# mitsuba-renderer/mitsuba2

Hardware: AMD Instinct MI355X
Metric: Msamples/sec (whole node), 1080p/512spp path integrator (higher is better)
Workload: dtype f32

## Files before the change

### mitsuba2_amd/csrc/device/resident_kernel.h

```cpp
#ifndef MIW_KERNEL
#define MIW_KERNEL __global__
#endif
MIW_KERNEL __launch_bounds__(MIW_BLOCK) void k_init_pixels(RenderParams P, U4 *st_out, uint32_t *pixel_out, InitArgs A) {
    uint32_t lane = blockIdx.x * blockDim.x + threadIdx.x;
    if (lane >= P.n_lanes) return;
    uint32_t tile = lane >> A.bs2_log2, i = lane & ((1u << A.bs2_log2) - 1u);
    uint32_t b = A.tile_list ? A.tile_list[tile] : tile;
    uint32_t bx = b % A.blocks_x, by = b / A.blocks_x;
    uint32_t x, y;
    morton_decode2(i, x, y);
    int32_t bw = P.film.crop_w - (int32_t) (bx * A.bs), bh = P.film.crop_h - (int32_t) (by * A.bs);
    if (bw > (int32_t) A.bs) bw = (int32_t) A.bs;
    if (bh > (int32_t) A.bs) bh = (int32_t) A.bs;
    if ((int32_t) x >= bw || (int32_t) y >= bh) {
        U4 st; st.x = st.y = 0; st.z = LF_DONE; st.w = 0;
        st_out[lane] = st; pixel_out[lane] = 0;
        return;
    }
    uint32_t px = (uint32_t) P.film.crop_x + bx * A.bs + x, py = (uint32_t) P.film.crop_y + by * A.bs + y;
    pixel_out[lane] = px | (py << 16);
    st_out[lane] = lane_seed_state(A.base_seed + (uint64_t) A.block_ids[b] * (uint64_t) (A.bs * A.bs) + i);
}

struct TileArgs {
// ... 21 lines not shown
            if (nq > 1u) { const uint32_t id = Q->simd_ids[1u + key]; q = id < nq ? id : key % nq; }
            else if ((threadIdx.x & 63u) == 0u) Q->simd_ids[1u + key] = 1u;
        }
    }
    uint32_t ticks, quarter, tail_prio, sample_end_; uint32_t *prog;
    __device__ __forceinline__ void tick(uint32_t sample_idx, bool has_pixel) {
        if (!tail_prio) { ++ticks; return; }
        if ((uint32_t) __builtin_amdgcn_readfirstlane((int) ++ticks) & 15u) return;
        if (has_pixel) atomicMin(prog, sample_idx);
        const uint32_t v = *prog;
        *prog = 0xffffffffu;
        const uint32_t v4 = 4u * v, se = sample_end_;
        uint32_t qtr = v == 0xffffffffu ? 3u : (v4 >= se ? 1u : 0u) + (v4 >= 2u * se ? 1u : 0u) + (v4 >= 3u * se ? 1u : 0u);
        qtr = (uint32_t) __builtin_amdgcn_readfirstlane((int) qtr);
        if (qtr == quarter) return;
        quarter = qtr;
        if (qtr == 0u) __builtin_amdgcn_s_setprio(3); else if (qtr == 1u) __builtin_amdgcn_s_setprio(2);
        else if (qtr == 2u) __builtin_amdgcn_s_setprio(1); else __builtin_amdgcn_s_setprio(0);
    }
    __device__ __forceinline__ void enable_tail_prio(uint32_t sample_end, uint32_t *wave_word) {
        tail_prio = 1u; sample_end_ = sample_end; quarter = 0; prog = wave_word; *prog = 0xffffffffu; __builtin_amdgcn_s_setprio(3);
    }
    typedef uint32_t U4v __attribute__((ext_vector_type(4)));
    __device__ __forceinline__ static uint32_t &job_pend() { __shared__ uint32_t s_job_pend[MIW_BLOCK]; return s_job_pend[threadIdx.x & (MIW_BLOCK - 1)]; }
    __device__ __forceinline__ bool exhausted() const { return !Jobs || !Q->job_chunk || job_pend() == 0xffffffffu; }
    __device__ __forceinline__ uint32_t job_end(uint32_t sample_idx, uint32_t sample_end) const {
        const uint32_t r = spp - sample_idx;
        return Jobs && (r & (r - 1u)) == 0u && r >= Q->job_min ? sample_idx : sample_end;
    }
    __device__ __forceinline__ bool fetch_job(uint32_t &pixel, U4 &st) {
        for (;;) {
            const uint32_t parked = job_pend();
            if (parked == 0xffffffffu) return false;
            uint32_t id = parked - 1u;
            const bool fresh = parked == 0u;
            const unsigned long long b = __ballot(fresh);
            if (fresh) {
                const uint32_t me = threadIdx.x & 63u, leader = (uint32_t) __ffsll((long long) b) - 1u;
                uint32_t base = 0;
                if (me == leader) base = atomicAdd(next_pixel, (uint32_t) __popcll(b));
                base = (uint32_t) __shfl((int) base, (int) leader, 64);
                id = base + __builtin_amdgcn_mbcnt_hi((uint32_t) (b >> 32), __builtin_amdgcn_mbcnt_lo((uint32_t) b, 0u));
                if (id >= Q->job_total) { job_pend() = 0xffffffffu; return false; }
            }
            const uint32_t j = id / n_lanes, slot = id - j * n_lanes;
            const uint32_t px = Q->pixel[slot];
            U4v w;
#if defined(__HIP_DEVICE_COMPILE__)
            asm volatile("global_load_dwordx4 %0, %1, off sc1\n\ts_waitcnt vmcnt(0)" : "=&v"(w) : "v"(Q->st + slot) : "memory");
#endif
            if (w.z & LF_DONE) { job_pend() = 0u; continue; }
            if (w.w != (j ? spp - (Q->job_pow >> (j - 1u)) : 0u)) { job_pend() = id + 1u; return false; }
            job_pend() = 0u;
            lane = slot; pixel = px;
            st.x = w.x; st.y = w.y; st.z = w.z; st.w = w.w;
            return true;
        }
    }
    __device__ __forceinline__ bool fetch(uint32_t &pixel, U4 &st) {
        if (Jobs && Q->job_chunk) return fetch_job(pixel, st);
        for (;;) {
            if (!Placed) {
                const unsigned long long b = __ballot(1);
                const uint32_t me = threadIdx.x & 63u, leader = (uint32_t) __ffsll((long long) b) - 1u;
                uint32_t base = 0;
                if (me == leader) base = atomicAdd(next_pixel, (uint32_t) __popcll(b));
                base = (uint32_t) __shfl((int) base, (int) leader, 64);
                const uint32_t l = base + __builtin_amdgcn_mbcnt_hi((uint32_t) (b >> 32), __builtin_amdgcn_mbcnt_lo((uint32_t) b, 0u));
                if (l >= n_lanes) return false;
                lane = l;
                st = Q->st[lane];
                if (st.z & LF_DONE) continue;
                pixel = Q->pixel[lane];
                return true;
            }
            if (dry >= nq) {
                if (nq > 1u) Q->simd_ids[0] = 1u;
                return false;
            }
            if (nq > 1u && __hip_atomic_load(Q->simd_ids, __ATOMIC_RELAXED, __HIP_MEMORY_SCOPE_AGENT)) { dry = nq; return false; }
            const unsigned long long all = __ballot(1);
            const uint32_t me = threadIdx.x & 63u, leader = (uint32_t) __ffsll((long long) all) - 1u;
            const uint32_t q_lead = (uint32_t) __shfl((int) q, (int) leader, 64);
            const bool mine = q == q_lead;
            const unsigned long long b = __ballot(mine);
            if (!mine) continue;
            uint32_t base = 0;
            if (me == leader) base = atomicAdd(next_pixel + q, (uint32_t) __popcll(b));
            base = (uint32_t) __shfl((int) base, (int) leader, 64);
            const uint32_t idx = base + __builtin_amdgcn_mbcnt_hi((uint32_t) (b >> 32), __builtin_amdgcn_mbcnt_lo((uint32_t) b, 0u));
            uint32_t l = idx;
            if (nq > 1u) {
                const uint32_t piece = idx < per ? Q->piece_list[q * MIW_PLACE_PIECES + (idx >> 6)] : 0xffffffffu;
                if (piece == 0xffffffffu) { q = q + 1u == nq ? 0u : q + 1u; ++dry; continue; }
                l = Q->lane_sorted[piece * Q->piece_a + (idx & 63u) * Q->piece_b];
                if (l >= n_lanes) continue;
            } else if (l >= n_lanes) { ++dry; continue; }
            lane = l;
            st = Q->st[lane];
            if (st.z & LF_DONE) continue;
            pixel = Q->pixel[lane];
            if (Placed) t_fetch = cost_clock();
            return true;
        }
    }
    __device__ __forceinline__ uint32_t cost_clock() const {
        return Clock ? (uint32_t) (__builtin_amdgcn_s_memtime() >> 8) : ticks;
    }
    __device__ __forceinline__ void store(U4 st) {
        if (Jobs && Q->job_chunk) {
            unsigned long long *words = reinterpret_cast<unsigned long long *>(Q->st + lane);
            __hip_atomic_store(words, (unsigned long long) st.x | ((unsigned long long) st.y << 32), __ATOMIC_RELAXED, __HIP_MEMORY_SCOPE_AGENT);
            asm volatile("s_waitcnt vmcnt(0)" ::: "memory");
            __hip_atomic_store(words + 1, (unsigned long long) st.z | ((unsigned long long) st.w << 32), __ATOMIC_RELAXED, __HIP_MEMORY_SCOPE_AGENT);
            return;
        }
        Q->st[lane] = st;
        if (Placed && Q->lane_cost) Q->lane_cost[lane] = cost_clock() - t_fetch + 1u;
        if (Groups && Q->group_done && (st.z & LF_DONE)) {
            __threadfence();
            const uint32_t g = lane >> Q->group_shift;
            if (atomicAdd(Q->group_done + g, 1u) + 1u == Q->group_expected[g]) {
                __threadfence_system();
                __hip_atomic_store(Q->group_flag + g, 1u, __ATOMIC_RELEASE, __HIP_MEMORY_SCOPE_SYSTEM);
            }
        }
    }
    __device__ __forceinline__ void put(uint32_t pixel, uint32_t sample_idx, V2 pos, const float *aovs) {
        if (Q->log_rec) {
            LogSink16<const float *> sink{ Q->log_rec, thr, film, lane, spp, Q->log_rej & 255u, Q->log_rej >> 8 };
            sink(pixel, sample_idx, pos, aovs);
        } else {
            LogSink sink; sink.log_pos = Q->log_pos; sink.log_val = Q->log_val; sink.lane = lane; sink.spp = spp; sink.warn_negative = warn_negative;
            sink(0u, sample_idx, pos, aovs);
        }
    }
};

#ifndef MIW_DIRECT_WAVES
#define MIW_DIRECT_WAVES 3
#endif
#ifndef MIW_PACKET_WAVES_ALL
#define MIW_PACKET_WAVES_ALL 4
#endif
#ifndef MIW_PACKET_WAVES
#define MIW_PACKET_WAVES 5
#endif
template <bool UseLog, int Tiny, int Mats = MATS_ALL, bool Analytic = (Tiny == 0), uint32_t Integ = INTEG_PATH, bool Groups = false, int Waves = 0>
__global__ __launch_bounds__(MIW_BLOCK, Waves ? Waves : Integ == INTEG_DIRECT ? MIW_DIRECT_WAVES : Tiny ? ((Mats == MATS_DIFFUSE && !MIW_SPECTRAL) ? (Tiny == 2 ? MIW_PACKET_WAVES : 4) : MIW_PACKET_WAVES_ALL) : MIW_TREE_WAVES) void k_path_resident(RenderParams P, SceneView sc, LaneQueues Q, double *accum, Counters *cnt,
                                                               TraceLds cfg, uint32_t sample_end, TileArgs T, uint32_t *next_pixel) {
    extern __shared__ uint4 smem[];
    stage_to_lds(sc, cfg, smem);
    const float *thr = stage_thresholds(smem, cfg, UseLog && Q.log_rec ? Q.log_thr : nullptr);
#if MIW_LDS_TABLES
    if constexpr (UseLog && Tiny != 0) stage_tables<true, mats_lights(Mats)>(sc, cfg, smem);
#endif
#if defined(MIW_SECTION_PROFILE) && defined(__HIP_DEVICE_COMPILE__)
    if ((threadIdx.x & 63u) == 0) { unsigned long long *b_ = miw_sec_buf(); for (int i = 0; i < 15; ++i) b_[i] = 0; b_[15] = __builtin_amdgcn_s_memtime(); }
#endif
    const uint32_t lane = blockIdx.x * blockDim.x + threadIdx.x;
    double *tile = reinterpret_cast<double *>(smem + T.geom16);
    int tile_x0 = 0, tile_y0 = 0;
    if (!UseLog && T.side) {
        const uint32_t lane0 = blockIdx.x * blockDim.x, t = lane0 >> T.bs2_log2, q0 = lane0 & ((1u << T.bs2_log2) - 1u);
        const uint32_t b = T.tile_list ? T.tile_list[t] : t;
        uint32_t qx, qy;
        morton_decode2(q0, qx, qy);
        const int margin = (int) (T.side - 16u) / 2;
        tile_x0 = (int) ((b % T.blocks_x) * T.bs + qx) - margin;
        tile_y0 = (int) ((b / T.blocks_x) * T.bs + qy) - margin;
        for (uint32_t i = threadIdx.x; i < T.side * T.side * MIW_FILM_CHANNELS; i += blockDim.x) tile[i] = 0.0;
        __syncthreads();
    }
    LaneCounters local; local.segments = local.samples = local.shadow_rays = 0;
    auto tr2 = [&](V3 o, float mint, V3 dE, float maxtE, bool hasE, V3 dS, float maxtS, bool hasS, F4 &hE, bool &occS) {
        trace2<Tiny, Analytic>(sc, cfg, smem, o, mint, dE, maxtE, hasE, dS, maxtS, hasS, hE, occS);
    };
    if (UseLog) {
        QueueWork<Tiny != 0, false, Groups> work; work.Q = &Q; work.next_pixel = next_pixel; work.n_lanes = P.n_lanes; work.spp = P.spp; work.lane = 0; work.warn_negative = P.film.warn_negative;
        work.film = &P.film; work.thr = thr; work.init_queues(cfg.queues ? cfg.queues : 1u);
        __shared__ uint32_t s_prog[MIW_BLOCK / 64];
        if (cfg.tail_prio) work.enable_tail_prio(sample_end, &s_prog[threadIdx.x >> 6]);
        if constexpr (Integ == INTEG_DIRECT) pixel_stream_render_direct<Mats, Analytic>(P, sc, sample_end, work, tr2, &local);
        else pixel_stream_render<Mats, Analytic>(P, sc, sample_end, work, tr2, &local);
    } else if (lane < P.n_lanes) {
        U4 st = Q.st[lane];
        if (!(st.z & LF_DONE)) {
            const uint32_t pixel = Q.pixel[lane];
            if (T.side) {
                TileAdd add; add.tile = tile; add.x0 = tile_x0; add.y0 = tile_y0; add.side = (int) T.side;
                SplatXYSink<TileAdd> sink; sink.film = &P.film; sink.add = add;
                st = pixel_render<Integ, mats_nested(Mats) ? Mats : MATS_ALL>(P, sc, pixel, st, sample_end, tr2, sink, &local);
            } else {
                FilmAdd add; add.accum = accum;
                SplatSink<FilmAdd> sink; sink.film = &P.film; sink.add = add;
                st = pixel_render<Integ, mats_nested(Mats) ? Mats : MATS_ALL>(P, sc, pixel, st, sample_end, tr2, sink, &local);
            }
            Q.st[lane] = st;
        }
    }
    if (!UseLog && T.side) {
        __syncthreads();
        const int n = (int) (T.side * T.side);
        for (int i = (int) threadIdx.x; i < n * MIW_FILM_CHANNELS; i += (int) blockDim.x) {
            const double v = tile[i];
            if (v == 0.0) continue;
            const int texel = i / MIW_FILM_CHANNELS, k = i - texel * MIW_FILM_CHANNELS;
            const int fx = tile_x0 + texel % (int) T.side, fy = tile_y0 + texel / (int) T.side;
            unsafeAtomicAdd(accum + ((size_t) fy * P.film.crop_w + fx) * MIW_FILM_CHANNELS + k, v);
        }
    }
    unsigned long long a = wave_sum(local.segments), b = wave_sum(local.samples), c = wave_sum(local.shadow_rays);
    if ((threadIdx.x & 63) == 0) {
        Counters *shard = cnt + ((blockIdx.x * (MIW_BLOCK / 64) + (threadIdx.x >> 6)) & (MIW_CNT_SHARDS - 1));
        if (a) atomicAdd(&shard->segments, a);
        if (b) atomicAdd(&shard->samples, b);
        if (c) atomicAdd(&shard->shadow_rays, c);
#if defined(MIW_SECTION_PROFILE) && defined(__HIP_DEVICE_COMPILE__)
        { unsigned long long *b_ = miw_sec_buf(); for (int i = 0; i < 15; ++i) if (b_[i]) atomicAdd(&g_sections[i], b_[i]); }
#endif
    }
}
```

### mitsuba2_amd/csrc/device/trace.h

```cpp

struct TraceLds {
    uint32_t nodes_staged;
    uint32_t tris_staged;
    uint32_t brute;
    uint32_t leaves;
    uint32_t stack;
    uint32_t stack16;
    uint32_t shade_num, shade_den;
    uint32_t node_exit, tri_exit;
    uint32_t queues;
    uint32_t tail_prio;
    uint32_t thr16;
    uint32_t tab16;
    uint32_t tab_words[10];
    uint32_t env_top_count, env_top_base, env_top_words;
    uint32_t pool_claim_min;
    uint32_t pool16, stat16;
    uint32_t light_words;
};

struct alignas(16) LeafBox { float p[6]; uint32_t mask_lo, mask_hi; };
static_assert(sizeof(LeafBox) == 32, "LeafBox must be 32 bytes");

struct alignas(16) TriPacket { float p0[3], e1[3], e2[3]; uint32_t prim; uint32_t pad[2]; };
static_assert(sizeof(TriPacket) == 48, "TriPacket must be 48 bytes");

#ifndef MIW_LDS_TABLES
#define MIW_LDS_TABLES 1
#endif
#ifndef MIW_OCTANT_BOXES
#define MIW_OCTANT_BOXES 1
#endif
#define MIW_LEAF_BOX_COPIES (MIW_OCTANT_BOXES ? 8u : 1u)
__device__ __forceinline__ void stage_to_lds(const SceneView &sc, TraceLds cfg, uint4 *smem) {
    if (cfg.brute) {
        TriPacket *dst = reinterpret_cast<TriPacket *>(smem);
        for (uint32_t i = threadIdx.x; i < sc.tri_count; i += blockDim.x) {
            const Tri &t = sc.tris[i];
            V3 p0 = ld3(t.p0), e1 = ld3(t.p1) - p0, e2 = ld3(t.p2) - p0;
            TriPacket k;
            k.p0[0] = p0.x; k.p0[1] = p0.y; k.p0[2] = p0.z; k.e1[0] = e1.x; k.e1[1] = e1.y; k.e1[2] = e1.z;
            k.e2[0] = e2.x; k.e2[1] = e2.y; k.e2[2] = e2.z; k.prim = t.prim; k.pad[0] = k.pad[1] = 0;
            dst[i] = k;
        }
        uint4 *dst_b = smem + sc.tri_count * (sizeof(TriPacket) / 16);
        const uint4 *src_b = reinterpret_cast<const uint4 *>(sc.leaf_boxes);
#if MIW_OCTANT_BOXES
        for (uint32_t i = threadIdx.x; i < cfg.leaves * 8u; i += blockDim.x) {
            const LeafBox b = reinterpret_cast<const LeafBox *>(sc.leaf_boxes)[i >> 3];
            const uint32_t o = i & 7u;
            LeafBox k;
            for (int a = 0; a < 3; ++a) { const bool neg = (o >> a) & 1u; k.p[2 * a] = b.p[2 * a + (neg ? 1 : 0)]; k.p[2 * a + 1] = b.p[2 * a + (neg ? 0 : 1)]; }
            k.mask_lo = b.mask_lo; k.mask_hi = b.mask_hi;
            reinterpret_cast<LeafBox *>(dst_b)[i] = k;
        }
        (void) src_b;
#else
        for (uint32_t i = threadIdx.x; i < cfg.leaves * (sizeof(LeafBox) / 16); i += blockDim.x) dst_b[i] = src_b[i];
#endif
        float *dst_t = reinterpret_cast<float *>(dst_b + cfg.leaves * MIW_LEAF_BOX_COPIES * (sizeof(LeafBox) / 16));
        const float *src_t = reinterpret_cast<const float *>(sc.tri_bounds);
        for (uint32_t i = threadIdx.x; i < sc.tri_count * 6u; i += blockDim.x) dst_t[i] = src_t[i];
        __syncthreads();
        return;
    }
    const uint4 *src_n = reinterpret_cast<const uint4 *>(sc.nodes);
    uint32_t n16 = cfg.nodes_staged * (sizeof(BvhNode) / 16);
    for (uint32_t i = threadIdx.x; i < n16; i += blockDim.x) smem[i] = src_n[i];
    const uint4 *src_t = reinterpret_cast<const uint4 *>(sc.tris);
    uint32_t t16 = cfg.tris_staged * (sizeof(Tri) / 16);
    uint4 *dst_t = smem + n16;
    for (uint32_t i = threadIdx.x; i < t16; i += blockDim.x) dst_t[i] = src_t[i];
    __syncthreads();
}

__device__ __forceinline__ const float *stage_thresholds(uint4 *smem, TraceLds cfg, const float *thr_global) {
    float *t = reinterpret_cast<float *>(smem + cfg.thr16);
    if (thr_global) {
        for (uint32_t i = threadIdx.x; i < MIW_FC_TABLE; i += blockDim.x) t[i] = thr_global[i];
        __syncthreads();
    }
    return t;
}

template <bool WithTris, bool Lights = false>
__device__ __forceinline__ void stage_tables(SceneView &sc, const TraceLds &cfg, uint4 *smem) {
    constexpr int N = WithTris ? 10 : 7;
    uint32_t *dst = reinterpret_cast<uint32_t *>(smem + cfg.tab16);
    const uint32_t *src[10] = { reinterpret_cast<const uint32_t *>(sc.shapes), reinterpret_cast<const uint32_t *>(sc.bsdfs), reinterpret_cast<const uint32_t *>(sc.emitters),
                                reinterpret_cast<const uint32_t *>(sc.emit_tri), reinterpret_cast<const uint32_t *>(sc.emit_vnorm),
                                reinterpret_cast<const uint32_t *>(sc.emit_pmf), reinterpret_cast<const uint32_t *>(sc.emit_cdf),
                                reinterpret_cast<const uint32_t *>(sc.tris), reinterpret_cast<const uint32_t *>(sc.tri_vn), reinterpret_cast<const uint32_t *>(sc.tri_uv) };
    uint32_t *at[10];
    uint32_t off = 0;
#pragma unroll
    for (int k = 0; k < N; ++k) {
        const uint32_t n = cfg.tab_words[k];
        at[k] = dst + off;
        for (uint32_t i = threadIdx.x; i < n; i += blockDim.x) dst[off + i] = src[k][i];
        off += (n + 3u) & ~3u;
    }
    uint32_t *lights_at = dst + off;
    if constexpr (Lights) {
        const uint32_t *lsrc = reinterpret_cast<const uint32_t *>(sc.lights);
        for (uint32_t i = threadIdx.x; i < cfg.light_words; i += blockDim.x) lights_at[i] = lsrc[i];
        off += (cfg.light_words + 3u) & ~3u;
    }
    uint32_t *env_at = dst + off;
    if (cfg.env_top_words) {
        const uint32_t *lv = reinterpret_cast<const uint32_t *>(sc.env->levels) + cfg.env_top_base;
        for (uint32_t i = threadIdx.x; i < cfg.env_top_words; i += blockDim.x) env_at[i] = lv[i];
    }
    sc.env_top = reinterpret_cast<const float *>(env_at); sc.env_top_count = cfg.env_top_count; sc.env_top_base = cfg.env_top_base;
    __syncthreads();
    sc.shapes = reinterpret_cast<const ShapeRec *>(at[0]); sc.bsdfs = reinterpret_cast<const BsdfRec *>(at[1]); sc.emitters = reinterpret_cast<const EmitterRec *>(at[2]);
    sc.emit_tri = reinterpret_cast<const float *>(at[3]);
    sc.emit_vnorm = reinterpret_cast<const float *>(at[4]);
    sc.emit_pmf = reinterpret_cast<const float *>(at[5]); sc.emit_cdf = reinterpret_cast<const float *>(at[6]);
    if constexpr (Lights) {
        if (cfg.light_words) {
            const LightRec *staged = reinterpret_cast<const LightRec *>(lights_at);
            if (sc.constant) sc.constant = staged + (sc.constant - sc.lights);
            sc.lights = staged;
        }
    }
    if (WithTris) {
        sc.tris = reinterpret_cast<const Tri *>(at[7]); sc.tri_vn = reinterpret_cast<const float *>(at[8]); sc.tri_uv = reinterpret_cast<const float *>(at[9]);
    }
}

struct FastRay { V3 inv_d, neg_o_inv_d; float mint; };
__device__ __forceinline__ FastRay fast_ray(V3 o, V3 d, float mint) {
    FastRay r;
    float dx = abs_(d.x) < 1e-30f ? mulsign(1e-30f, d.x) : d.x,
          dy = abs_(d.y) < 1e-30f ? mulsign(1e-30f, d.y) : d.y,
          dz = abs_(d.z) < 1e-30f ? mulsign(1e-30f, d.z) : d.z;
    r.inv_d = v3(__builtin_amdgcn_rcpf(dx), __builtin_amdgcn_rcpf(dy), __builtin_amdgcn_rcpf(dz));
    r.neg_o_inv_d = v3(-(o.x * r.inv_d.x), -(o.y * r.inv_d.y), -(o.z * r.inv_d.z));
    r.mint = mint;
    return r;
}
__device__ __forceinline__ bool box_test_fast(const float *lo, const float *hi, const FastRay &r, float tmax_wide, float &tn_out) {
    float t0x = __builtin_fmaf(lo[0], r.inv_d.x, r.neg_o_inv_d.x), t1x = __builtin_fmaf(hi[0], r.inv_d.x, r.neg_o_inv_d.x),
          t0y = __builtin_fmaf(lo[1], r.inv_d.y, r.neg_o_inv_d.y), t1y = __builtin_fmaf(hi[1], r.inv_d.y, r.neg_o_inv_d.y),
          t0z = __builtin_fmaf(lo[2], r.inv_d.z, r.neg_o_inv_d.z), t1z = __builtin_fmaf(hi[2], r.inv_d.z, r.neg_o_inv_d.z);
    float tn = __builtin_fmaxf(__builtin_fmaxf(__builtin_fminf(t0x, t1x), __builtin_fminf(t0y, t1y)),
                               __builtin_fmaxf(__builtin_fminf(t0z, t1z), r.mint));
    float tf = __builtin_fminf(__builtin_fminf(__builtin_fmaxf(t0x, t1x), __builtin_fmaxf(t0y, t1y)), __builtin_fmaxf(t0z, t1z));
    tf = __builtin_fmaf(abs_(tf), 2e-6f, tf);
    tn_out = tn;
    return tn <= tf && tn <= tmax_wide;
}
typedef float miw_f2 __attribute__((ext_vector_type(2)));
__device__ __forceinline__ bool leaf_box_test(const LeafBox &b, const FastRay &r, float tmax_wide) {
    const miw_f2 px = { b.p[0], b.p[1] }, py = { b.p[2], b.p[3] }, pz = { b.p[4], b.p[5] };
    const miw_f2 tx = __builtin_elementwise_fma(px, (miw_f2) { r.inv_d.x, r.inv_d.x }, (miw_f2) { r.neg_o_inv_d.x, r.neg_o_inv_d.x }),
                 ty = __builtin_elementwise_fma(py, (miw_f2) { r.inv_d.y, r.inv_d.y }, (miw_f2) { r.neg_o_inv_d.y, r.neg_o_inv_d.y }),
                 tz = __builtin_elementwise_fma(pz, (miw_f2) { r.inv_d.z, r.inv_d.z }, (miw_f2) { r.neg_o_inv_d.z, r.neg_o_inv_d.z });
    const float tn = __builtin_fmaxf(__builtin_fmaxf(__builtin_fminf(tx.x, tx.y), __builtin_fminf(ty.x, ty.y)),
                                     __builtin_fmaxf(__builtin_fminf(tz.x, tz.y), r.mint));
    float tf = __builtin_fminf(__builtin_fminf(__builtin_fmaxf(tx.x, tx.y), __builtin_fmaxf(ty.x, ty.y)), __builtin_fmaxf(tz.x, tz.y));
    tf = __builtin_fmaf(abs_(tf), 2e-6f, tf);
    return tn <= tf && tn <= tmax_wide;
}
__device__ __forceinline__ bool leaf_box_test_octant(const LeafBox &b, const FastRay &r, float tmax_wide) {
    const miw_f2 px = { b.p[0], b.p[1] }, py = { b.p[2], b.p[3] }, pz = { b.p[4], b.p[5] };
    const miw_f2 tx = __builtin_elementwise_fma(px, (miw_f2) { r.inv_d.x, r.inv_d.x }, (miw_f2) { r.neg_o_inv_d.x, r.neg_o_inv_d.x }),
                 ty = __builtin_elementwise_fma(py, (miw_f2) { r.inv_d.y, r.inv_d.y }, (miw_f2) { r.neg_o_inv_d.y, r.neg_o_inv_d.y }),
                 tz = __builtin_elementwise_fma(pz, (miw_f2) { r.inv_d.z, r.inv_d.z }, (miw_f2) { r.neg_o_inv_d.z, r.neg_o_inv_d.z });
    const float tn = __builtin_fmaxf(__builtin_fmaxf(tx.x, ty.x), __builtin_fmaxf(tz.x, r.mint));
    float tf = __builtin_fminf(__builtin_fminf(tx.y, ty.y), tz.y);
    tf = __builtin_fmaf(abs_(tf), 2e-6f, tf);
    return tn <= tf && tn <= tmax_wide;
}
__device__ __forceinline__ uint32_t ray_octant(const FastRay &r) {
    return (r.inv_d.x < 0.f ? 1u : 0u) | (r.inv_d.y < 0.f ? 2u : 0u) | (r.inv_d.z < 0.f ? 4u : 0u);
}
__device__ __forceinline__ float widen(float t) { return __builtin_fmaf(abs_(t), 2e-6f, t); }

#ifndef MIW_STACK_ENTRIES
#define MIW_STACK_ENTRIES 32
#endif
#ifndef MIW_WALK
#define MIW_WALK 1
#endif
#ifndef MIW_LDS_TOP
#define MIW_LDS_TOP 0
#endif
#ifndef MIW_TREE_WAVES
#define MIW_TREE_WAVES 3
#endif
template <bool AnyHit, bool Analytic, typename NodeAt, typename TriAt>
__device__ __forceinline__ bool bvh_intersect_stack(NodeAt node_at, TriAt tri_at, int32_t *stack ,
                                                    V3 o, V3 d, float mint, float maxt, Hit &best, PrimCtx ctx) {
    best.t = MIW_INFINITY; best.u = best.v = 0.f; best.tri = MIW_MISS; best.prim = 0xffffffffu;
    const FastRay r = fast_ray(o, d, mint);
    float tmax = maxt;
    int32_t cur = 0, sp = 0;
    for (;;) {
        if (cur >= 0) {
            const BvhNode &n = node_at(cur);
            float tn0, tn1;
            const float wide = widen(tmax);
            const bool h0 = box_test_fast(n.lo0, n.hi0, r, wide, tn0), h1 = box_test_fast(n.lo1, n.hi1, r, wide, tn1);
            const int32_t c0 = n.child0, c1 = n.child1;
            if (h0 && h1) {
                const bool second_first = tn1 < tn0;
                stack[sp * MIW_BLOCK] = second_first ? c0 : c1; ++sp;
                cur = second_first ? c1 : c0;
                continue;
            }
            if (h0 || h1) { cur = h0 ? c0 : c1; continue; }
        } else {
            const uint32_t code = (uint32_t) ~cur, first = code >> 4, count = (code & 15u) + 1u;
            for (uint32_t i = 0; i < count; ++i) {
                const Tri &tr = tri_at(first + i);
                float t, u, v;
                if (prim_intersect<Analytic>(tr, ctx, o, d, mint, maxt, t, u, v)) {
                    if (AnyHit) { best.t = 0.f; best.tri = first + i; best.prim = tr.prim; return true; }
                    if (t < best.t || (t == best.t && tr.prim < best.prim)) {
                        best.t = t; best.u = u; best.v = v; best.tri = first + i; best.prim = tr.prim;
                        tmax = t;
                    }
                }
            }
        }
        if (sp == 0) return best.tri != MIW_MISS;
        --sp; cur = stack[sp * MIW_BLOCK];
    }
}

#if defined(MIW_WALK_STATS)
#define MIW_WALK_STATS_DECL unsigned long long ws_lane_[2] = { 0, 0 }; float ws_wave_[2] = { 0.f, 0.f }
#define MIW_WALK_STATS_STEP(k) do { ws_lane_[k]++; ws_wave_[k] += 1.f / (float) __popcll(__ballot(1)); } while (0)
#define MIW_WALK_STATS_FLUSH(base) do { atomicAdd(&g_walk_stats[(base)], ws_lane_[0]); atomicAdd(&g_walk_stats[(base) + 1], ws_lane_[1]); \
        atomicAdd(&g_walk_statsf[(base)], ws_wave_[0]); atomicAdd(&g_walk_statsf[(base) + 1], ws_wave_[1]); \
        atomicAdd(&g_walk_stats[(base) + 2], 1ull); } while (0)
#else
#define MIW_WALK_STATS_DECL do { } while (0)
#define MIW_WALK_STATS_STEP(k) do { } while (0)
#define MIW_WALK_STATS_FLUSH(base) do { } while (0)
#endif
#define MIW_WALK_DONE ((int32_t) 0x80000000)
template <bool AnyHit, bool Analytic, int Postpone, typename NodeAt, typename TriAt>
__device__ __forceinline__ bool bvh_intersect_ww(NodeAt node_at, TriAt tri_at, int32_t *stack ,
                                                 V3 o, V3 d, float mint, float maxt, Hit &best, PrimCtx ctx) {
    best.t = MIW_INFINITY; best.u = best.v = 0.f; best.tri = MIW_MISS; best.prim = 0xffffffffu;
    const FastRay r = fast_ray(o, d, mint);
    float tmax = maxt;
    int32_t cur = 0, sp = 0, parked = MIW_WALK_DONE;
    MIW_WALK_STATS_DECL;
    for (;;) {
        if (Postpone && cur < 0 && cur != MIW_WALK_DONE && parked == MIW_WALK_DONE) {
            parked = cur;
            if (sp == 0) cur = MIW_WALK_DONE; else { --sp; cur = stack[sp * MIW_BLOCK]; }
        }
        while (cur >= 0) {
            MIW_WALK_STATS_STEP(0);
            const BvhNode &n = node_at(cur);
            float tn0, tn1;
            const float wide = widen(tmax);
            const bool h0 = box_test_fast(n.lo0, n.hi0, r, wide, tn0), h1 = box_test_fast(n.lo1, n.hi1, r, wide, tn1);
            const int32_t c0 = n.child0, c1 = n.child1;
            const bool second_first = tn1 < tn0;
            int32_t next = h0 ? c0 : c1;
            if (h0 && h1) {
                stack[sp * MIW_BLOCK] = second_first ? c0 : c1; ++sp;
                next = second_first ? c1 : c0;
            } else if (!(h0 || h1)) {
                if (sp == 0) next = MIW_WALK_DONE; else { --sp; next = stack[sp * MIW_BLOCK]; }
            }
            if (Postpone && next < 0 && next != MIW_WALK_DONE && parked == MIW_WALK_DONE) {
                parked = next;
                if (sp == 0) next = MIW_WALK_DONE; else { --sp; next = stack[sp * MIW_BLOCK]; }
            }
            cur = next;
        }
        int32_t leaf;
        if (Postpone) {
            if (parked == MIW_WALK_DONE) break;
// ... 180 lines not shown
```

### mitsuba2_amd/csrc/miw/path.h

```cpp
#pragma once
#include "base.h"
#include "rng.h"
#include "scene.h"
#include "film.h"

namespace miw {

enum : uint32_t {
    LF_DEPTH_MASK  = 0x0fffu,
    LF_VALID_RAY   = 1u << 12,
    LF_PREV_DELTA  = 1u << 13,
    LF_HAS_SHADOW  = 1u << 14,
    LF_RAY_ACTIVE  = 1u << 15,
    LF_DONE        = 1u << 16,
    LF_DEAD_PENDING= 1u << 17,
};

struct LaneQueues {
    F4 *tp;
    F4 *res;
    U4 *st;
    F2 *pos;
    const uint32_t *pixel;
    F4 *ray_o;
// ... 58 lines not shown

MIW_HD void lane_begin_sample(const RenderParams &P, uint32_t pixel, LaneRegs &L, uint32_t sample_end) {
    if (L.sample_idx >= sample_end) {
        L.flags = LF_DONE;
        L.ray.o = L.ray.d = v3(0.f); L.ray.mint = 0.f; L.ray.maxt = -1.f;
        return;
    }
    float px = (float) (pixel & 0xffffu), py = (float) (pixel >> 16);
    V2 j = next_2d(L.rng);
    L.pos = v2(px + j.x, py + j.y);
    const float wavelength_sample = next_1d(L.rng);
#if MIW_SPECTRAL
    sample_wavelengths(wavelength_sample, L.wl, L.ray_weight);
#else
    (void) wavelength_sample; L.ray_weight = spec(1.f);
#endif
    V2 adj = v2((L.pos.x - P.crop_f[0]) / P.crop_f[2],
                (L.pos.y - P.crop_f[1]) / P.crop_f[3]);
    L.ray = sensor_sample_ray(P.sensor, adj, v3(P.cam_o[0], P.cam_o[1], P.cam_o[2]));
    L.tp = spec(1.f); L.res = spec(0.f); L.eta = 1.f; L.prev_pdf = 0.f;
    L.flags = 1u | LF_RAY_ACTIVE;
}

template <typename Sink>
MIW_HD void lane_finish_sample(const RenderParams &P, uint32_t pixel, LaneRegs &L, Sink sink) {
#if MIW_SPECTRAL
    V3 xyz = spectrum_to_xyz(L.ray_weight * L.res, L.wl);
#else
    V3 xyz = srgb_to_xyz(L.res);
#endif
    float aovs[5] = { xyz.x, xyz.y, xyz.z, (L.flags & LF_VALID_RAY) ? 1.f : 0.f, 1.f };
    if (P.moment_pass) {
        const float sq[3] = { sqr(xyz.x), sqr(xyz.y), sqr(xyz.z) };
        bool ok = true;
        for (int k = 0; k < 3; ++k) ok = ok && isfinite_(aovs[k]) && isfinite_(sq[k]);
        if (P.moment_pass == 2u) { aovs[0] = sq[0]; aovs[1] = sq[1]; aovs[2] = sq[2]; }
        if (!ok) aovs[0] = __builtin_nanf("");
    }
    sink(pixel, L.sample_idx, L.pos, aovs);
    L.sample_idx++;
}

template <typename Add> struct SplatSink {
    const FilmRec *film; Add add;
    MIW_HD void operator()(uint32_t pixel, uint32_t, V2 pos, const float *aovs) const {
        film_splat(*film, (int) (pixel & 0xffffu), (int) (pixel >> 16), pos, aovs, add);
    }
};
template <typename AddXY> struct SplatXYSink {
    const FilmRec *film; AddXY add;
    MIW_HD void operator()(uint32_t pixel, uint32_t, V2 pos, const float *aovs) const {
        film_splat_xy(*film, (int) (pixel & 0xffffu), (int) (pixel >> 16), pos, aovs, add);
    }
};
struct LogSink {
    F2 *log_pos; F4 *log_val; uint32_t lane, spp;
    uint32_t warn_negative;
    MIW_HD void operator()(uint32_t, uint32_t sample_idx, V2 pos, const float *aovs) const {
        size_t i = (size_t) lane * spp + sample_idx;
        F2 p; p.x = sample_is_valid(aovs, warn_negative != 0) ? pos.x : __builtin_nanf(""); p.y = pos.y;
        F4 v; v.x = aovs[0]; v.y = aovs[1]; v.z = aovs[2]; v.w = aovs[3];
        log_pos[i] = p; log_val[i] = v;
    }
};

#ifndef MIW_LOG_NT
#define MIW_LOG_NT 1
#endif
template <typename Thr>
struct LogSink16 {
    U4 *log_rec; Thr thr; const FilmRec *film; uint32_t lane, spp, rej, il;
    MIW_HD void operator()(uint32_t pixel, uint32_t sample_idx, V2 pos, const float *aovs) const {
        const size_t i = log_index(il, lane, spp, sample_idx);
        U4 r; r.x = r.y = r.z = 0u; r.w = film_pack_meta(rej, rej, false);
        if (sample_is_valid(aovs, film->warn_negative != 0)) {
            const uint32_t cx = film_class_of(thr, film_phase(*film, pos.x, (int) (pixel & 0xffffu), film->crop_x)),
                           cy = film_class_of(thr, film_phase(*film, pos.y, (int) (pixel >> 16), film->crop_y));
            r.x = f2u(aovs[0]); r.y = f2u(aovs[1]); r.z = f2u(aovs[2]); r.w = film_pack_meta(cx, cy, aovs[3] != 0.f);
        }
#if defined(__HIP_DEVICE_COMPILE__) && MIW_LOG_NT
        typedef uint32_t u4v_ __attribute__((ext_vector_type(4)));
        u4v_ v_; v_.x = r.x; v_.y = r.y; v_.z = r.z; v_.w = r.w;
        __builtin_nontemporal_store(v_, reinterpret_cast<u4v_ *>(log_rec + i));
#else
        log_rec[i] = r;
#endif
    }
};

MIW_HD void lane_load(const LaneQueues &Q, uint32_t lane, LaneRegs &L) {
    U4 st = Q.st[lane];
    L.rng.state = (uint64_t) st.x | ((uint64_t) st.y << 32);
    L.rng.inc = MIW_PCG32_SCALAR_INC;
    L.flags = st.z; L.sample_idx = st.w;
}
#if !MIW_SPECTRAL
MIW_HD void lane_load_path(const LaneQueues &Q, uint32_t lane, LaneRegs &L) {
    F4 a = Q.tp[lane], b = Q.res[lane];
    L.tp = v3(a.x, a.y, a.z); L.eta = a.w;
    L.res = v3(b.x, b.y, b.z); L.prev_pdf = b.w;
    L.pos = v2(0.f, 0.f);
}
MIW_HD void lane_store(const LaneQueues &Q, uint32_t lane, const LaneRegs &L, bool store_pos) {
    U4 st; st.x = (uint32_t) L.rng.state; st.y = (uint32_t) (L.rng.state >> 32);
    st.z = L.flags; st.w = L.sample_idx;
    Q.st[lane] = st;
    F4 a; a.x = L.tp.x; a.y = L.tp.y; a.z = L.tp.z; a.w = L.eta; Q.tp[lane] = a;
    F4 b; b.x = L.res.x; b.y = L.res.y; b.z = L.res.z; b.w = L.prev_pdf; Q.res[lane] = b;
    if (store_pos) { F2 p; p.x = L.pos.x; p.y = L.pos.y; Q.pos[lane] = p; }
    F4 o; o.x = L.ray.o.x; o.y = L.ray.o.y; o.z = L.ray.o.z; o.w = L.ray.mint; Q.ray_o[lane] = o;
    F4 d; d.x = L.ray.d.x; d.y = L.ray.d.y; d.z = L.ray.d.z; d.w = L.ray.maxt; Q.ray_d[lane] = d;
}
MIW_HD void lane_clear_shadow(const LaneQueues &Q, uint32_t lane) {
    F4 dead; dead.x = dead.y = dead.z = 0.f; dead.w = -1.f;
    Q.sh_d[lane] = dead;
}

MIW_HD void lane_init(const RenderParams &P, const LaneQueues &Q, uint32_t lane, uint32_t pixel, uint64_t seed) {
    LaneRegs L;
    pcg32_seed(L.rng, seed, MIW_PCG32_DEFAULT_STREAM);
    L.sample_idx = 0; L.flags = 0;
    L.tp = v3(1.f); L.res = v3(0.f); L.eta = 1.f; L.prev_pdf = 0.f; L.pos = v2(0.f, 0.f);
    L.ray.o = L.ray.d = v3(0.f); L.ray.mint = 0.f; L.ray.maxt = -1.f;
    lane_begin_sample(P, pixel, L, P.spp);
    lane_store(Q, lane, L, true);
    lane_clear_shadow(Q, lane);
    Q.sh_vis[lane] = 0;
}
MIW_HD void lane_init_unused(const LaneQueues &Q, uint32_t lane) {
    LaneRegs L;
    L.rng.state = 0; L.rng.inc = MIW_PCG32_SCALAR_INC; L.sample_idx = 0; L.flags = LF_DONE;
    L.tp = v3(0.f); L.res = v3(0.f); L.eta = 0.f; L.prev_pdf = 0.f; L.pos = v2(0.f, 0.f);
    L.ray.o = L.ray.d = v3(0.f); L.ray.mint = 0.f; L.ray.maxt = -1.f;
    lane_store(Q, lane, L, true);
    lane_clear_shadow(Q, lane);
    Q.sh_vis[lane] = 0;
}
#endif

#ifndef MIW_SECTION
#define MIW_SECTION(i) do { } while (0)
#endif

struct ShadowOut { bool has; V3 d; float maxt; Spec c; };

enum { STEP_CONTINUE = 0,
       STEP_FINISHED = 1,
       STEP_DEAD_PENDING = 2 };

enum { MATS_ALL = 0, MATS_DIFFUSE = 1, MATS_PLAIN = 2, MATS_TRIO = 3, MATS_NESTED = 4, MATS_LIGHTS = 5 };
MIW_HD constexpr bool mats_full(int mats) { return mats == MATS_ALL || mats == MATS_NESTED || mats == MATS_LIGHTS; }
MIW_HD constexpr bool mats_nested(int mats) { return mats == MATS_NESTED || mats == MATS_LIGHTS; }
MIW_HD constexpr bool mats_lights(int mats) { return mats == MATS_LIGHTS; }
template <int Mats = MATS_ALL, bool Analytic = true, typename PrevO, typename Cnt>
MIW_HD int path_step(const RenderParams &P, const SceneView &sc, LaneRegs &L, F4 h, PrevO prev_o,
                     ShadowOut &sh, Cnt *cnt_local) {
    sh.has = false;
    const uint32_t depth = L.flags & LF_DEPTH_MASK;
    const uint32_t tri_idx = f2u(h.w);
    const bool valid = tri_idx != MIW_MISS;
    const V3 ray_d = L.ray.d;

    SurfaceInteraction si;
    uint32_t bsdf_index = 0;
    int32_t emitter = -1;
    if (valid) hit_surface_interaction<Analytic, mats_full(Mats)>(sc, tri_idx, h.x, h.y, h.z, prev_o, ray_d, si, bsdf_index, emitter);
    else emitter = miss_emitter<mats_lights(Mats)>(sc);
    if (depth == 1 && valid) L.flags |= LF_VALID_RAY;
    MIW_SECTION(7);

    if (emitter >= 0) {
        float emission_weight = 1.f;
        if (depth > 1) {
            float emitter_pdf = 0.f;
            if (!(L.flags & LF_PREV_DELTA)) {
                V3 d = ray_d; float dist = 0.f; V3 n = v3(0.f), ref_p = v3(0.f);
                if (valid) {
                    ref_p = prev_o();
                    d = si.p - ref_p;
                    dist = norm(d);
                    d = d / dist;
                    n = si.sh.n;
                }
                emitter_pdf = pdf_emitter_direction<Analytic, mats_lights(Mats)>(sc, (uint32_t) emitter, d, dist, n, ref_p);
            }
            emission_weight = mis_weight(L.prev_pdf, emitter_pdf);
        }
        Spec radiance = valid ? emitter_eval(sc.emitters[emitter], si.wi, L.wl) : miss_eval<mats_lights(Mats)>(sc, ray_d, L.wl);
        L.res = L.res + emission_weight * L.tp * radiance;
    }

    MIW_SECTION(8);
    bool active = valid;

    if ((int32_t) depth > P.rr_depth) {
        float q = min_(hmax(L.tp) * sqr(L.eta), .95f);
        active = (next_1d(L.rng) < q) && active;
        L.tp = L.tp * rcp(q);
    }

    if (depth >= (uint32_t) P.max_depth || !active) return STEP_FINISHED;

    if (cnt_local) cnt_local->segments++;
    BsdfSide bsdf;
    if (Mats == MATS_DIFFUSE) { bsdf.b = sc.bsdfs + bsdf_index; bsdf.flip = bsdf.none = false; bsdf.flags = BSDF_DiffuseReflection; }
    else bsdf = bsdf_side<mats_nested(Mats)>(sc.bsdfs, bsdf_index, si.wi);
    const uint32_t bflags = bsdf.flags;
    L.ray.o = si.p; L.ray.mint = spawn_mint(si.p);
    L.ray.d = v3(0.f); L.ray.maxt = -1.f;

    const TexCtx tc(L.wl, si.uv, mats_full(Mats) ? sc.bitmaps : nullptr, mats_full(Mats) ? sc.bsdf_tables : nullptr);
    constexpr bool Ext = mats_full(Mats);
    constexpr bool Trio = Mats == MATS_TRIO;
    constexpr bool Nested = mats_nested(Mats);

    if (bflags & BSDF_Smooth) {
        DirectionSample ds;
        Spec emitter_val = sample_emitter_direction<Analytic, mats_lights(Mats)>(sc, si.p, next_2d(L.rng), ds, L.wl);
        if (ds.pdf != 0.f) {
            V3 wo = to_local(si.sh, ds.d);
            Spec bsdf_val = Mats == MATS_DIFFUSE ? diffuse_eval(*bsdf.b, si.wi, wo, tc) : bsdf_side_eval<Ext, Trio, Nested>(bsdf, si.wi, wo, tc);
            float bpdf = Mats == MATS_DIFFUSE ? diffuse_pdf(si.wi, wo) : bsdf_side_pdf<Ext, Trio, Nested>(bsdf, si.wi, wo, tc);
            float mis = (mats_lights(Mats) && ds.delta) ? 1.f : mis_weight(ds.pdf, bpdf);
            Spec c = mis * L.tp * bsdf_val * emitter_val;
            if (!all_zero(c)) {
                sh.has = true; sh.d = ds.d; sh.maxt = ds.dist * (1.f - MIW_SHADOW_EPSILON); sh.c = c;
                if (cnt_local) cnt_local->shadow_rays++;
            }
        }
    }

    MIW_SECTION(9);
    float s1 = next_1d(L.rng);
    V2 s2 = next_2d(L.rng);
    BSDFSample bs;
    Spec bsdf_val = Mats == MATS_DIFFUSE ? diffuse_sample(*bsdf.b, si.wi, s2, bs, tc) : bsdf_side_sample<Ext, Trio, Nested>(bsdf, si.wi, s1, s2, bs, tc);
    L.tp = L.tp * bsdf_val;
    if (all_zero(L.tp))
        return sh.has ? STEP_DEAD_PENDING : STEP_FINISHED;
    L.eta *= bs.eta;
    L.ray.d = to_world(si.sh, bs.wo);
    L.ray.maxt = MIW_INFINITY;
    L.prev_pdf = bs.pdf;
    L.flags = (L.flags & ~(LF_DEPTH_MASK | LF_PREV_DELTA)) | ((depth + 1) & LF_DEPTH_MASK)
            | ((bs.sampled_type & BSDF_Delta) ? LF_PREV_DELTA : 0u) | LF_RAY_ACTIVE;
    MIW_SECTION(10);
    return STEP_CONTINUE;
}

#if !MIW_SPECTRAL
template <int Mats = MATS_NESTED, typename Sink, typename Cnt>
MIW_HD uint32_t lane_shade(const RenderParams &P, const SceneView &sc, const LaneQueues &Q,
                           uint32_t lane, Cnt *cnt_local, Sink sink) {
    LaneRegs L;
    lane_load(Q, lane, L);
    if (L.flags & LF_DONE) return LF_DONE;
    lane_load_path(Q, lane, L);
    const bool had_shadow = (L.flags & LF_HAS_SHADOW) != 0;

    if (had_shadow) {
        if (Q.sh_vis[lane]) { F4 c = Q.sh_c[lane]; L.res = L.res + v3(c.x, c.y, c.z); }
        L.flags &= ~LF_HAS_SHADOW;
    }

    bool finished = false;

    if (L.flags & LF_DEAD_PENDING) {
        finished = true;
    } else {
        F4 rd = Q.ray_d[lane];
        L.ray.d = v3(rd.x, rd.y, rd.z);
        ShadowOut sh;
        const int r = path_step<Mats>(P, sc, L, Q.hit[lane],
                                [&]() { F4 ro = Q.ray_o[lane]; return v3(ro.x, ro.y, ro.z); }, sh, cnt_local);
        if (sh.has) {
            F4 sd; sd.x = sh.d.x; sd.y = sh.d.y; sd.z = sh.d.z; sd.w = sh.maxt;
            Q.sh_d[lane] = sd;
            F4 sc4; sc4.x = sh.c.x; sc4.y = sh.c.y; sc4.z = sh.c.z; sc4.w = 0.f;
            Q.sh_c[lane] = sc4;
            L.flags |= LF_HAS_SHADOW;
        }
        if (r == STEP_FINISHED) finished = true;
        else if (r == STEP_DEAD_PENDING)
            L.flags = (L.flags & ~LF_RAY_ACTIVE) | LF_DEAD_PENDING;
    }

    bool store_pos = false;
    if (finished) {
        const uint32_t pixel = Q.pixel[lane];
        F2 ps = Q.pos[lane]; L.pos = v2(ps.x, ps.y);
        lane_finish_sample(P, pixel, L, sink);
        if (cnt_local) cnt_local->samples++;
        L.flags = 0;
        lane_begin_sample(P, pixel, L, P.spp);
        store_pos = true;
    }
    lane_store(Q, lane, L, store_pos);
    if (had_shadow && !(L.flags & LF_HAS_SHADOW)) lane_clear_shadow(Q, lane);
    return L.flags;
}
#endif

template <int Mats = MATS_ALL, bool Analytic = true, typename Work, typename Trace2, typename Cnt>
MIW_HD void pixel_stream_render(const RenderParams &P, const SceneView &sc, uint32_t sample_end, Work &work,
                                Trace2 trace2, Cnt *cnt_local) {
    LaneRegs L;
    L.flags = LF_DONE; L.sample_idx = 0; L.rng.state = 0; L.rng.inc = MIW_PCG32_SCALAR_INC;
    uint32_t pixel = 0;
    bool have = false, dead_pending = false;
    ShadowOut sh; sh.has = false; sh.d = v3(0.f); sh.maxt = -1.f; sh.c = spec(0.f);
    auto sink = [&work](uint32_t px, uint32_t sample_idx, V2 pos, const float *aovs) { work.put(px, sample_idx, pos, aovs); };
    for (;;) {
        if (L.flags & LF_DONE) {
            if (have) {
                U4 st; st.x = (uint32_t) L.rng.state; st.y = (uint32_t) (L.rng.state >> 32);
                st.z = L.sample_idx >= P.spp ? (uint32_t) LF_DONE : 0u; st.w = L.sample_idx;
                work.store(st);
            }
            U4 st;
            have = work.fetch(pixel, st);
            if (!have) { if (work.exhausted()) break; continue; }
            L.rng.state = (uint64_t) st.x | ((uint64_t) st.y << 32);
            L.sample_idx = st.w; L.flags = 0;
            lane_begin_sample(P, pixel, L, sample_end);
            MIW_SECTION(0);
            continue;
        }
        work.tick(L.sample_idx, true);
        MIW_SECTION(0);
        const V3 o = L.ray.o;
        F4 h; bool occluded = false;
        trace2(o, L.ray.mint, L.ray.d, L.ray.maxt, !dead_pending, sh.d, sh.maxt, sh.has, h, occluded);
        if (sh.has && !occluded) L.res = L.res + sh.c;
        sh.has = false;
        int r = STEP_FINISHED;
        if (!dead_pending) {
            r = path_step<Mats, Analytic>(P, sc, L, h, [o]() { return o; }, sh, cnt_local);
            MIW_SECTION(4);
            if (r == STEP_DEAD_PENDING) { dead_pending = true; continue; }
            if (r == STEP_CONTINUE) continue;
        }
        dead_pending = false;
        lane_finish_sample(P, pixel, L, sink);
        if (cnt_local) cnt_local->samples++;
        L.flags = 0;
        lane_begin_sample(P, pixel, L, work.job_end(L.sample_idx, sample_end));
        MIW_SECTION(5);
    }
}

MIW_HD void lane_begin_path(LaneRegs &L) {
    L.tp = spec(1.f); L.res = spec(0.f); L.eta = 1.f; L.prev_pdf = 0.f;
    L.flags = 1u | LF_RAY_ACTIVE;
    L.sample_idx = 0; L.pos = v2(0.f, 0.f); L.ray_weight = spec(1.f);
}
template <int Mats = MATS_ALL, bool Analytic = true, typename Feed, typename Trace2, typename Cnt>
MIW_HD void ray_stream_sample(const RenderParams &P, const SceneView &sc, Feed &feed, Trace2 trace2, Cnt *cnt_local) {
    LaneRegs L;
    L.flags = LF_DONE; L.rng.state = 0; L.rng.inc = MIW_PCG32_SCALAR_INC;
    bool dead_pending = false;
    ShadowOut sh; sh.has = false; sh.d = v3(0.f); sh.maxt = -1.f; sh.c = spec(0.f);
    for (;;) {
        if (L.flags & LF_DONE) {
            if (!feed.fetch(L)) break;
            lane_begin_path(L);
            continue;
        }
        const V3 o = L.ray.o;
        F4 h; bool occluded = false;
        trace2(o, L.ray.mint, L.ray.d, L.ray.maxt, !dead_pending, sh.d, sh.maxt, sh.has, h, occluded);
        if (sh.has && !occluded) L.res = L.res + sh.c;
        sh.has = false;
        if (!dead_pending) {
            const int r = path_step<Mats, Analytic>(P, sc, L, h, [o]() { return o; }, sh, cnt_local);
            if (r == STEP_DEAD_PENDING) { dead_pending = true; continue; }
            if (r == STEP_CONTINUE) continue;
        }
        dead_pending = false;
        feed.store(L);
        if (cnt_local) cnt_local->samples++;
        L.flags = LF_DONE;
    }
}

template <int Mats, bool Analytic, typename Feed, typename Trace2, typename Cnt>
MIW_HD void ray_stream_sample_direct(const RenderParams &P, const SceneView &sc, Feed &feed, Trace2 trace2, Cnt *cnt_local);

template <int Mats, bool Analytic, typename Work, typename Trace2, typename Cnt>
MIW_HD void pixel_stream_render_direct(const RenderParams &P, const SceneView &sc, uint32_t sample_end, Work &work,
                                       Trace2 trace2, Cnt *cnt_local);

template <uint32_t Integ = INTEG_PATH, int Mats = MATS_NESTED, typename Trace2, typename Sink, typename Cnt>
MIW_HD U4 pixel_render(const RenderParams &P, const SceneView &sc, uint32_t pixel, U4 st, uint32_t sample_end,
                       Trace2 trace2, Sink sink, Cnt *cnt_local) {
    struct OnePixel {
        uint32_t pixel; U4 st; bool taken; Sink sink;
        MIW_HD bool fetch(uint32_t &px, U4 &s) { if (taken) return false; taken = true; px = pixel; s = st; return true; }
        MIW_HD void store(U4 s) { st = s; }
        MIW_HD bool exhausted() const { return true; }
        MIW_HD uint32_t job_end(uint32_t, uint32_t sample_end) const { return sample_end; }
        MIW_HD void tick(uint32_t, bool) { }
        MIW_HD void put(uint32_t px, uint32_t sample_idx, V2 pos, const float *aovs) { sink(px, sample_idx, pos, aovs); }
    } work{ pixel, st, false, sink };
    if constexpr (Integ == INTEG_DIRECT) pixel_stream_render_direct<Mats, true>(P, sc, sample_end, work, trace2, cnt_local);
    else pixel_stream_render<Mats>(P, sc, sample_end, work, trace2, cnt_local);
    return work.st;
}

MIW_HD U4 lane_seed_state(uint64_t seed) {
    PCG32 r; pcg32_seed(r, seed, MIW_PCG32_DEFAULT_STREAM);
    U4 st; st.x = (uint32_t) r.state; st.y = (uint32_t) (r.state >> 32); st.z = 0; st.w = 0;
    return st;
}

}
```

### mitsuba2_amd/csrc/miw/scene.h

```cpp
#pragma once
#include "base.h"
#include "shape.h"
#include "bsdf.h"
#include "envmap.h"
#include "light.h"

namespace miw {

#define MIW_MISS 0xffffffffu

struct BvhNode {
    float lo0[3], hi0[3];
    float lo1[3], hi1[3];
    int32_t child0, child1;
    int32_t parent;
    int32_t pad;
};

struct ShapeRec {
    uint32_t bsdf;
    int32_t  emitter;
    uint32_t flags;
    uint32_t pad;
};

struct EmitterRec {
    TexRec radiance;
    uint32_t shape;
    uint32_t tri_first;
    uint32_t tri_count;
    uint32_t valid_lo, valid_hi;
    float sum, normalization;
    uint32_t flags;
    uint32_t type;
};
enum : uint32_t { SHAPE_HAS_NORMALS = 1u, SHAPE_HAS_TEXCOORDS = 8u };

struct SceneView {
    const BvhNode *nodes;   uint32_t node_count;
    const Tri     *tris;    uint32_t tri_count;
    const float   *tri_vn;
    const float   *tri_uv;
    const ShapeRec *shapes; uint32_t shape_count;
    const BsdfRec  *bsdfs;  uint32_t bsdf_count;
    const EmitterRec *emitters; uint32_t emitter_count;
    float emitter_count_f, emitter_count_inv;
    const float *emit_tri;
    const float *emit_vnorm;
    const float *emit_pmf, *emit_cdf;
    const EnvmapRec *env;
    const AnalyticRec *rects;   uint32_t rect_count;
    const BitmapRec *bitmaps;
    const float *bsdf_tables;
    float accept_pad;
    const void *tri_bounds;
    const void *leaf_boxes;
    const struct Bvh4Node *nodes4;
    const struct Bvh8Node *nodes8;
    const float *env_top; uint32_t env_top_count, env_top_base;
    const LightRec *lights;
    const LightRec *constant;
};
MIW_HD EnvTop env_top(const SceneView &sc) { EnvTop t; t.p = sc.env_top; t.count = sc.env_top_count; t.base = sc.env_top_base; return t; }
MIW_HD void scene_view_prepare(SceneView &v) {
    v.emitter_count_f = (float) v.emitter_count;
    v.emitter_count_inv = v.emitter_count ? 1.f / (float) v.emitter_count : 0.f;
}

MIW_HD PrimCtx prim_ctx(const SceneView &sc) { PrimCtx c; c.rects = sc.rects; c.accept_pad = sc.accept_pad; return c; }

template <bool Analytic, bool Texcoords, typename RayO>
MIW_HD void hit_surface_interaction(const SceneView &sc, uint32_t tri_idx, float t, float u, float v, RayO ray_o, V3 ray_d,
                                    SurfaceInteraction &si, uint32_t &bsdf_index, int32_t &emitter) {
    const Tri &tr = sc.tris[tri_idx];
    const ShapeRec &shape = sc.shapes[tr.shape];
    if (Analytic && tr.pad) {
        const AnalyticRec &a = sc.rects[tr.pad - 1u];
        if (a.kind == ANALYTIC_SPHERE) compute_surface_interaction_sphere(a, t, ray_o(), ray_d, si);
        else compute_surface_interaction_rect(a, t, u, v, ray_o(), ray_d, si);
    } else {
        const float *vn = (shape.flags & 1u) ? sc.tri_vn + 9 * (size_t) tri_idx : nullptr;
        const float *tc = (Texcoords && (shape.flags & SHAPE_HAS_TEXCOORDS)) ? sc.tri_uv + 6 * (size_t) tr.prim : nullptr;
        compute_surface_interaction(ld3(tr.p0), ld3(tr.p1), ld3(tr.p2), vn, tc, t, u, v, ray_d, si);
    }
    si.shape = tr.shape; si.prim = tr.prim;
    emitter = shape.emitter; bsdf_index = shape.bsdf;
}

struct DirectionSample { V3 p, n, d; float dist, pdf; uint32_t emitter; bool delta; };

template <bool Lights = false>
MIW_HD int32_t miss_emitter(const SceneView &sc) {
    if (sc.env) return (int32_t) sc.env->emitter_index;
    if (Lights && sc.constant) return (int32_t) sc.constant->emitter_index;
    return -1;
}

MIW_HD MeshSampler emitter_mesh(const SceneView &sc, const EmitterRec &e) {
    MeshSampler m;
    m.tri = sc.emit_tri + 9 * (size_t) e.tri_first;
    m.vnorm = (e.flags & 1u) ? sc.emit_vnorm + 9 * (size_t) e.tri_first : nullptr;
    m.pmf = sc.emit_pmf + e.tri_first;
    m.cdf = sc.emit_cdf + e.tri_first;
    m.count = e.tri_count;
    m.valid_lo = e.valid_lo; m.valid_hi = e.valid_hi;
    m.sum = e.sum; m.normalization = e.normalization;
    return m;
}

MIW_HD void sphere_sample_direction(const AnalyticRec &r, V3 ref_p, V2 sample, DirectionSample &ds) {
    const V3 center = ld3(r.n);
    const float radius = r.radius;
    V3 dc_v = center - ref_p;
    float dc_2 = squared_norm(dc_v);
    float radius_adj = radius * (r.flip ? (1.f + MIW_RAY_EPSILON) : (1.f - MIW_RAY_EPSILON));
    if (dc_2 > sqr(radius_adj)) {
        float inv_dc = rsqrt(dc_2),
              sin_theta_max = radius * inv_dc,
              sin_theta_max_2 = sqr(sin_theta_max),
              inv_sin_theta_max = rcp(sin_theta_max),
              cos_theta_max = safe_sqrt(1.f - sin_theta_max_2);
        float sin_theta_2 = sin_theta_max_2 > 0.00068523f ? 1.f - sqr(fmadd(cos_theta_max - 1.f, sample.x, 1.f))
                                                          : sin_theta_max_2 * sample.x,
              cos_theta = safe_sqrt(1.f - sin_theta_2);
        float cos_alpha = sin_theta_2 * inv_sin_theta_max + cos_theta * safe_sqrt(fnmadd(sin_theta_2, sqr(inv_sin_theta_max), 1.f)),
              sin_alpha = safe_sqrt(fnmadd(cos_alpha, cos_alpha, 1.f));
        float sin_phi, cos_phi;
        sincos_(sample.y * (2.f * MIW_PI), sin_phi, cos_phi);
        Frame f; f.n = dc_v * -inv_dc;
        coordinate_system(f.n, f.s, f.t);
        V3 d = to_world(f, v3(cos_phi * sin_alpha, sin_phi * sin_alpha, cos_alpha));
        ds.p = v3(fmadd(d.x, radius, center.x), fmadd(d.y, radius, center.y), fmadd(d.z, radius, center.z));
        ds.n = d;
        ds.d = ds.p - ref_p;
        float dist2 = squared_norm(ds.d);
        ds.dist = __builtin_sqrtf(dist2);
        ds.d = ds.d / ds.dist;
        ds.pdf = (.5f * MIW_INV_PI) / (1.f - cos_theta_max);
        if (ds.dist == 0.f) ds.pdf = 0.f;
    } else {
        V3 d = square_to_uniform_sphere(sample);
        ds.p = v3(fmadd(d.x, radius, center.x), fmadd(d.y, radius, center.y), fmadd(d.z, radius, center.z));
        ds.n = d;
        ds.d = ds.p - ref_p;
        float dist2 = squared_norm(ds.d);
        ds.dist = __builtin_sqrtf(dist2);
        ds.d = ds.d / ds.dist;
        ds.pdf = r.inv_area * dist2 / abs_dot(ds.d, ds.n);
    }
    if (r.flip) ds.n = -ds.n;
}
MIW_HD float sphere_pdf_direction(const AnalyticRec &r, V3 ref_p, V3 ds_d, float ds_dist, V3 ds_n) {
    float sin_alpha = r.radius * rcp(norm(ld3(r.n) - ref_p)),
          cos_alpha = safe_sqrt(1.f - sin_alpha * sin_alpha);
    return sin_alpha < (1.f - MIW_EPSILON) ? (.5f * MIW_INV_PI) / (1.f - cos_alpha)
                                           : r.inv_area * sqr(ds_dist) / abs_dot(ds_d, ds_n);
}

#if MIW_SPECTRAL
MIW_HD Spec env_eval_uv_spec(const EnvmapRec &e, V2 uv, const Wavelengths &wl) {
    uv.x *= (float) (e.width - 1u); uv.y *= (float) (e.height - 1u);
    uint32_t px = (uint32_t) uv.x, py = (uint32_t) uv.y;
    if (px > e.width - 2u) px = e.width - 2u;
    if (py > e.height - 2u) py = e.height - 2u;
    const float w1x = uv.x - (float) px, w1y = uv.y - (float) py, w0x = 1.f - w1x, w0y = 1.f - w1y;
    const float *p = e.data + 4 * ((size_t) px + (size_t) py * e.width);
    const float *q = p + 4 * (size_t) e.width;
    const float f0 = fmadd(w0x, p[3], w1x * p[7]), f1 = fmadd(w0x, q[3], w1x * q[7]);
    const float f = fmadd(w0y, f0, w1y * f1);
    Spec r;
    for (int i = 0; i < MIW_SPEC_N; ++i) {
        const float l = wl.l[i];
        const float s00 = srgb_model_eval(p, l), s10 = srgb_model_eval(p + 4, l),
                    s01 = srgb_model_eval(q, l), s11 = srgb_model_eval(q + 4, l);
        const float s0 = fmadd(w0x, s00, w1x * s10), s1 = fmadd(w0x, s01, w1x * s11);
        const float sv = fmadd(w0y, s0, w1y * s1);
        const float wp = d65_eval(1.f * (1.f / 10568.f), l);
        r.c[i] = sv * wp * f * e.scale;
    }
    return r;
}
MIW_HD Spec env_eval_spec(const EnvmapRec &e, V3 d_world, const Wavelengths &wl) {
    return env_eval_uv_spec(e, env_dir_to_uv(xf_vector(e.to_local, d_world)), wl);
}
MIW_HD Spec env_sample_direction_spec(const EnvmapRec &e, V3 ref_p, V2 sample, V3 &d_out, float &dist_out, float &pdf_out,
                                      V3 &p_out, V3 &n_out, const Wavelengths &wl, EnvTop top = env_top_none()) {
    float pdf;
    V2 uv = hier2d_sample(e, sample, pdf, top);
    float theta = uv.y * MIW_PI, phi = uv.x * (2.f * MIW_PI);
    float st, ct, sp, cp;
    sincos_(theta, st, ct); sincos_(phi, sp, cp);
    V3 d = v3(cp * st, sp * st, ct);
    d = v3(d.y, d.z, -d.x);
    float dist = 2.f * e.radius;
    float inv_sin_theta = env_inv_sin_theta(d);
    d = xf_vector(e.to_world, d);
    p_out = ref_p + d * dist;
    n_out = -d;
    float ds_pdf = pdf > 0.f ? pdf * inv_sin_theta * (1.f / (2.f * sqr(MIW_PI))) : 0.f;
    d_out = d; dist_out = dist; pdf_out = ds_pdf;
    return env_eval_uv_spec(e, uv, wl) / ds_pdf;
}
#else
MIW_HD Spec env_sample_direction_spec(const EnvmapRec &e, V3 ref_p, V2 sample, V3 &d, float &dist, float &pdf, V3 &p, V3 &n, const Wavelengths &,
                                      EnvTop top = env_top_none()) {
    return env_sample_direction(e, ref_p, sample, d, dist, pdf, p, n, top);
}
MIW_HD Spec env_eval_spec(const EnvmapRec &e, V3 d, const Wavelengths &) { return env_eval(e, d); }
#endif

template <bool Analytic = true, bool Lights = false>
MIW_HD Spec emitter_sample_direction(const SceneView &sc, uint32_t index, V3 ref_p, V2 sample, DirectionSample &ds, const Wavelengths &wl) {
    const EmitterRec &e = sc.emitters[index];
    Spec value;
    ds.emitter = index;
    if (Lights) ds.delta = false;
    if (Lights && e.type >= EMITTER_POINT) {
        LightSample ls;
        value = light_sample_direction(sc.lights[e.tri_first], ref_p, sample, ls, wl);
        ds.p = ls.p; ds.n = ls.n; ds.d = ls.d; ds.dist = ls.dist; ds.pdf = ls.pdf; ds.delta = ls.delta;
    } else if (e.type == EMITTER_ENVMAP) {
        value = env_sample_direction_spec(*sc.env, ref_p, sample, ds.d, ds.dist, ds.pdf, ds.p, ds.n, wl, env_top(sc));
    } else {
        if (Analytic && (e.flags & 2u) && sc.rects[e.tri_first].kind == ANALYTIC_SPHERE) {
            sphere_sample_direction(sc.rects[e.tri_first], ref_p, sample, ds);
        } else {
            PositionSample ps = (Analytic && (e.flags & 2u)) ? rect_sample_position(sc.rects[e.tri_first], sample)
                                                             : mesh_sample_position(emitter_mesh(sc, e), sample);
            ds.p = ps.p; ds.n = ps.n; ds.pdf = ps.pdf;
            ds.d = ds.p - ref_p;
            float dist_squared = squared_norm(ds.d);
            ds.dist = __builtin_sqrtf(dist_squared);
            ds.d = ds.d / ds.dist;
            float dp = abs_dot(ds.d, ds.n);
            ds.pdf *= (dp != 0.f) ? dist_squared / dp : 0.f;
        }
        bool active = dot(ds.d, ds.n) < 0.f && ds.pdf != 0.f;
        value = tex_eval(e.radiance, wl) / ds.pdf;
        if (!active) value = spec(0.f);
    }
    return value;
}

template <bool Analytic = true, bool Lights = false>
MIW_HD Spec sample_emitter_direction(const SceneView &sc, V3 ref_p, V2 sample, DirectionSample &ds, const Wavelengths &wl) {
    if (sc.emitter_count == 0) {
        ds.p = ds.n = ds.d = v3(0.f); ds.dist = 0.f; ds.pdf = 0.f; ds.emitter = 0;
        if (Lights) ds.delta = false;
        return spec(0.f);
    }
    uint32_t index = 0;
    float emitter_pdf = 1.f;
    if (sc.emitter_count > 1) {
        float n = sc.emitter_count_f;
        emitter_pdf = sc.emitter_count_inv;
        uint32_t i = (uint32_t) (sample.x * n);
        index = i < sc.emitter_count - 1 ? i : sc.emitter_count - 1;
        sample.x = (sample.x - (float) index * emitter_pdf) * n;
    }
    Spec value = emitter_sample_direction<Analytic, Lights>(sc, index, ref_p, sample, ds, wl);
    if (sc.emitter_count > 1) {
        ds.pdf *= emitter_pdf;
        value = value * rcp(emitter_pdf);
    }
    return value;
}

template <bool Analytic = true, bool Lights = false>
MIW_HD float emitter_pdf_direction(const SceneView &sc, uint32_t emitter, V3 ds_d, float ds_dist, V3 ds_n, V3 ref_p) {
    const EmitterRec &e = sc.emitters[emitter];
    if (Lights && e.type >= EMITTER_POINT) return light_pdf_direction(sc.lights[e.tri_first]);
    if (e.type == EMITTER_ENVMAP) return env_pdf_direction(*sc.env, ds_d);
    float dp = dot(ds_d, ds_n);
    bool active = dp < 0.f;
    float pdf;
    if (Analytic && (e.flags & 2u) && sc.rects[e.tri_first].kind == ANALYTIC_SPHERE) {
        pdf = sphere_pdf_direction(sc.rects[e.tri_first], ref_p, ds_d, ds_dist, ds_n);
    } else {
        pdf = e.normalization;
        float adp = abs_dot(ds_d, ds_n);
        pdf *= (adp != 0.f) ? (ds_dist * ds_dist) / adp : 0.f;
    }
    return active ? pdf : 0.f;
}
template <bool Analytic = true, bool Lights = false>
MIW_HD float pdf_emitter_direction(const SceneView &sc, uint32_t emitter, V3 ds_d, float ds_dist, V3 ds_n, V3 ref_p) {
    float value = emitter_pdf_direction<Analytic, Lights>(sc, emitter, ds_d, ds_dist, ds_n, ref_p);
    if (sc.emitter_count > 1) value = value * sc.emitter_count_inv;
    return value;
}

MIW_HD Spec emitter_eval(const EmitterRec &e, V3 wi, const Wavelengths &wl) {
    return wi.z > 0.f ? tex_eval(e.radiance, wl) : spec(0.f);
}
template <bool Lights = false>
MIW_HD Spec miss_eval(const SceneView &sc, V3 ray_d, const Wavelengths &wl) {
    if (Lights && !sc.env) return light_eval(*sc.constant, wl);
    return env_eval_spec(*sc.env, ray_d, wl);
}


MIW_HD float mis_weight(float pdf_a, float pdf_b) {
    pdf_a *= pdf_a; pdf_b *= pdf_b;
    return pdf_a > 0.f ? pdf_a / (pdf_a + pdf_b) : 0.f;
}

struct SensorRec {
    float sample_to_camera[16];
    float to_world[16];
    float near_clip, far_clip;
    float pp_offset[2];
};

MIW_HD V3 sensor_origin(const SensorRec &s) { return xf_point_affine(s.to_world, v3(0.f)); }
MIW_HD Ray sensor_sample_ray(const SensorRec &s, V2 position_sample, V3 origin) {
    V3 near_p = xf_point_persp(s.sample_to_camera,
                               v3(position_sample.x + s.pp_offset[0],
                                  position_sample.y + s.pp_offset[1], 0.f));
    V3 d = normalize(near_p);
    float inv_z = rcp(d.z);
    Ray r;
    r.mint = s.near_clip * inv_z;
    r.maxt = s.far_clip * inv_z;
    r.o = origin;
    r.d = xf_vector(s.to_world, d);
    return r;
}
MIW_HD Ray sensor_sample_ray(const SensorRec &s, V2 position_sample) { return sensor_sample_ray(s, position_sample, sensor_origin(s)); }

}
```

### mitsuba2_amd/csrc/miw/shape.h

```cpp
#pragma once
#include "base.h"
#include "warp.h"
#include "special.h"

namespace miw {

struct Ray { V3 o, d; float mint, maxt; };

struct Tri {
    float p0[3], p1[3], p2[3];
    uint32_t shape;
    uint32_t prim;
    uint32_t pad;
};

enum : uint32_t { ANALYTIC_RECTANGLE = 0, ANALYTIC_SPHERE = 1 };
struct AnalyticRec {
    float to_world[16], to_object[16];
    float n[3], inv_area;
    float dp_du[3]; uint32_t shape;
    float dp_dv[3]; uint32_t prim;
    uint32_t kind; float radius;
    uint32_t flip;
    uint32_t pad_;
};

MIW_HD V3 ld3(const float *p) { return v3(p[0], p[1], p[2]); }

MIW_HD bool ray_intersect_triangle_edges(V3 p0, V3 e1, V3 e2, V3 o, V3 d, float mint, float maxt,
                                         float &t_out, float &u_out, float &v_out) {
    V3 pvec = cross(d, e2);
    float inv_det = rcp_loop(dot(e1, pvec));
    V3 tvec = o - p0;
    float u = dot(tvec, pvec) * inv_det;
    bool active = u >= 0.f && u <= 1.f;
    V3 qvec = cross(tvec, e1);
    float v = dot(d, qvec) * inv_det;
    active = active && v >= 0.f && u + v <= 1.f;
    float t = dot(e2, qvec) * inv_det;
    active = active && t >= mint && t <= maxt;
    t_out = t; u_out = u; v_out = v;
    return active;
}

MIW_HD bool ray_intersect_triangle(V3 p0, V3 p1, V3 p2, V3 o, V3 d, float mint, float maxt,
                                   float &t_out, float &u_out, float &v_out) {
    V3 e1 = p1 - p0, e2 = p2 - p0;
    V3 pvec = cross(d, e2);
    float inv_det = rcp(dot(e1, pvec));
    V3 tvec = o - p0;
    float u = dot(tvec, pvec) * inv_det;
    bool active = u >= 0.f && u <= 1.f;
    V3 qvec = cross(tvec, e1);
    float v = dot(d, qvec) * inv_det;
    active = active && v >= 0.f && u + v <= 1.f;
    float t = dot(e2, qvec) * inv_det;
    active = active && t >= mint && t <= maxt;
    t_out = t; u_out = u; v_out = v;
    return active;
}

MIW_HD bool ray_intersect_rectangle(const AnalyticRec &r, V3 o, V3 d, float mint, float maxt,
                                    float &t_out, float &u_out, float &v_out) {
    V3 ol = xf_point_affine(r.to_object, o), dl = xf_vector(r.to_object, d);
    float t = -ol.z * rcp(dl.z);
    V3 local = v3(fmadd(dl.x, t, ol.x), fmadd(dl.y, t, ol.y), fmadd(dl.z, t, ol.z));
    t_out = t; u_out = local.x; v_out = local.y;
    return t >= mint && t <= maxt && abs_(local.x) <= 1.f && abs_(local.y) <= 1.f;
}
struct PrimCtx { const AnalyticRec *rects; float accept_pad; };
struct TriBounds { float lo[3], hi[3]; };
MIW_HD TriBounds tri_bounds(V3 p0, V3 p1, V3 p2, float pad) {
    TriBounds b;
    b.lo[0] = min_(p0.x, min_(p1.x, p2.x)) - pad; b.hi[0] = max_(p0.x, max_(p1.x, p2.x)) + pad;
    b.lo[1] = min_(p0.y, min_(p1.y, p2.y)) - pad; b.hi[1] = max_(p0.y, max_(p1.y, p2.y)) + pad;
    b.lo[2] = min_(p0.z, min_(p1.z, p2.z)) - pad; b.hi[2] = max_(p0.z, max_(p1.z, p2.z)) + pad;
    return b;
}
#ifndef MIW_ACCEPT_RULE
#define MIW_ACCEPT_RULE 1
#endif
MIW_HD bool hit_in_bounds(const TriBounds &b, V3 o, V3 d, float t) {
#if !MIW_ACCEPT_RULE
    (void) b; (void) o; (void) d; (void) t;
    return true;
#endif
    const float px = fmadd(d.x, t, o.x), py = fmadd(d.y, t, o.y), pz = fmadd(d.z, t, o.z);
    return px >= b.lo[0] && px <= b.hi[0] && py >= b.lo[1] && py <= b.hi[1] && pz >= b.lo[2] && pz <= b.hi[2];
}
MIW_HD bool solve_quadratic_d(double a, double b, double c, double &x0, double &x1) {
    const bool linear_case = a == 0.0, valid_linear = linear_case && b != 0.0;
    x0 = x1 = -c / b;
    const double discrim = __builtin_fma(b, b, -(4.0 * a * c));
    const bool valid_quadratic = !linear_case && discrim >= 0.0;
    if (valid_quadratic) {
        const double sqrt_discrim = __builtin_sqrt(discrim);
        const double temp = -0.5 * (b + __builtin_copysign(sqrt_discrim, b));
        const double x0p = temp / a, x1p = c / temp;
        x0 = x1p < x0p ? x1p : x0p;
        x1 = x0p < x1p ? x1p : x0p;
    }
    return valid_linear || valid_quadratic;
}
MIW_HD bool ray_intersect_sphere(const AnalyticRec &r, V3 o_, V3 d_, float mint_, float maxt_,
                                 float &t_out, float &u_out, float &v_out) {
    const double mint = (double) mint_, maxt = (double) maxt_;
    const double ox = (double) o_.x - (double) r.n[0], oy = (double) o_.y - (double) r.n[1], oz = (double) o_.z - (double) r.n[2];
    const double dx = d_.x, dy = d_.y, dz = d_.z;
    const double A = __builtin_fma(dz, dz, __builtin_fma(dy, dy, dx * dx));
    const double B = 2.0 * __builtin_fma(oz, dz, __builtin_fma(oy, dy, ox * dx));
    const double rad = (double) r.radius;
    const double C = __builtin_fma(oz, oz, __builtin_fma(oy, oy, ox * ox)) - rad * rad;
    double near_t, far_t;
    const bool found = solve_quadratic_d(A, B, C, near_t, far_t);
    const bool out_bounds = !(near_t <= maxt && far_t >= mint);
    const bool in_bounds = near_t < mint && far_t > maxt;
    t_out = near_t < mint ? (float) far_t : (float) near_t;
    u_out = v_out = 0.f;
    return found && !out_bounds && !in_bounds;
}

template <bool Analytic = true>
MIW_HD bool prim_intersect(const Tri &tr, PrimCtx ctx, V3 o, V3 d, float mint, float maxt,
                           float &t, float &u, float &v) {
    if (Analytic && tr.pad) {
        const AnalyticRec &a = ctx.rects[tr.pad - 1u];
        return a.kind == ANALYTIC_SPHERE ? ray_intersect_sphere(a, o, d, mint, maxt, t, u, v)
                                         : ray_intersect_rectangle(a, o, d, mint, maxt, t, u, v);
    }
    const V3 p0 = ld3(tr.p0), p1 = ld3(tr.p1), p2 = ld3(tr.p2);
    return ray_intersect_triangle(p0, p1, p2, o, d, mint, maxt, t, u, v) &&
           hit_in_bounds(tri_bounds(p0, p1, p2, ctx.accept_pad), o, d, t);
}

struct SurfaceInteraction {
    float t;
    V3 p, n;
    Frame sh;
    V3 wi;
    V2 uv;
    uint32_t shape, prim;
};

MIW_HD void compute_surface_interaction(V3 p0, V3 p1, V3 p2, const float *vn, const float *tc,
                                        float t, float b1, float b2, V3 ray_d,
                                        SurfaceInteraction &si) {
    float b0 = 1.f - b1 - b2;
    V3 dp0 = p1 - p0, dp1 = p2 - p0;
    si.t = t;
    si.p = p0 * b0 + p1 * b1 + p2 * b2;
    si.n = normalize(cross(dp0, dp1));
    si.uv = v2(b1, b2);
    V3 dp_du, dp_dv;
    coordinate_system(si.n, dp_du, dp_dv);
    if (tc) {
        const V2 uv0 = v2(tc[0], tc[1]), uv1 = v2(tc[2], tc[3]), uv2 = v2(tc[4], tc[5]);
        si.uv = v2(uv0.x * b0 + uv1.x * b1 + uv2.x * b2, uv0.y * b0 + uv1.y * b1 + uv2.y * b2);
        const V2 duv0 = v2(uv1.x - uv0.x, uv1.y - uv0.y), duv1 = v2(uv2.x - uv0.x, uv2.y - uv0.y);
        const float det = fmsub(duv0.x, duv1.y, duv0.y * duv1.x), inv_det = rcp(det);
        if (det != 0.f) {
            dp_du = fmsub3(dp0, duv1.y, dp1 * duv0.y) * inv_det;
            dp_dv = fnmadd3(dp0, duv1.x, dp1 * duv0.x) * inv_det;
        }
    }
    if (vn) {
        V3 n0 = ld3(vn), n1 = ld3(vn + 3), n2 = ld3(vn + 6);
        si.sh.n = normalize(n0 * b0 + n1 * b1 + n2 * b2);
    } else {
        si.sh.n = si.n;
    }
    si.sh.s = normalize(fnmadd3(si.sh.n, dot(si.sh.n, dp_du), dp_du));
    si.sh.t = cross(si.sh.n, si.sh.s);
    si.wi = to_local(si.sh, -ray_d);
}
MIW_HD void compute_surface_interaction(V3 p0, V3 p1, V3 p2, const float *vn, float t, float b1, float b2, V3 ray_d,
                                        SurfaceInteraction &si) {
    compute_surface_interaction(p0, p1, p2, vn, nullptr, t, b1, b2, ray_d, si);
}

MIW_HD void compute_surface_interaction_rect(const AnalyticRec &r, float t, float u, float v, V3 ray_o, V3 ray_d,
                                             SurfaceInteraction &si) {
    si.t = t;
    si.p = v3(fmadd(ray_d.x, t, ray_o.x), fmadd(ray_d.y, t, ray_o.y), fmadd(ray_d.z, t, ray_o.z));
    si.n = ld3(r.n); si.sh.n = si.n;
    V3 dp_du = ld3(r.dp_du);
    si.uv = v2(fmadd(u, .5f, .5f), fmadd(v, .5f, .5f));
    si.sh.s = normalize(fnmadd3(si.sh.n, dot(si.sh.n, dp_du), dp_du));
    si.sh.t = cross(si.sh.n, si.sh.s);
    si.wi = to_local(si.sh, -ray_d);
}

MIW_HD float unit_angle_z(V3 v) {
    float temp = 2.f * asin_(.5f * __builtin_sqrtf(sqr(v.x) + sqr(v.y) + sqr(v.z - mulsign(1.f, v.z))));
    return v.z >= 0.f ? temp : MIW_PI - temp;
}
MIW_HD void compute_surface_interaction_sphere(const AnalyticRec &r, float t, V3 ray_o, V3 ray_d, SurfaceInteraction &si) {
    const V3 center = ld3(r.n);
    si.t = t;
    V3 n = normalize(v3(fmadd(ray_d.x, t, ray_o.x), fmadd(ray_d.y, t, ray_o.y), fmadd(ray_d.z, t, ray_o.z)) - center);
    si.p = v3(fmadd(n.x, r.radius, center.x), fmadd(n.y, r.radius, center.y), fmadd(n.z, r.radius, center.z));
    V3 local = xf_point_affine(r.to_object, si.p);
    float phi = atan2_(local.y, local.x);
    if (phi < 0.f) phi += 2.f * MIW_PI;
    si.uv = v2(phi * (.5f * MIW_INV_PI), unit_angle_z(local) * MIW_INV_PI);
    V3 dp_du = xf_vector(r.to_world, v3(-local.y, local.x, 0.f)) * (2.f * MIW_PI);
    if (r.flip) n = -n;
    si.sh.n = n; si.n = n;
    si.sh.s = normalize(fnmadd3(si.sh.n, dot(si.sh.n, dp_du), dp_du));
    si.sh.t = cross(si.sh.n, si.sh.s);
    si.wi = to_local(si.sh, -ray_d);
}

MIW_HD float spawn_mint(V3 p) { return (1.f + hmax(abs3(p))) * MIW_RAY_EPSILON; }

struct MeshSampler {
    const float *tri;
    const float *vnorm;
    const float *pmf;
    const float *cdf;
    uint32_t count;
    uint32_t valid_lo, valid_hi;
    float sum, normalization;
};

MIW_HD uint32_t distr_sample(const MeshSampler &m, float value) {
    value *= m.sum;
    uint32_t lo = m.valid_lo, hi = m.valid_hi;
    while (lo < hi) {
        uint32_t mid = (lo + hi) >> 1;
        if (m.cdf[mid] < value) lo = mid + 1; else hi = mid;
    }
    return lo;
}

struct PositionSample { V3 p, n; V2 uv; float pdf; };

MIW_HD PositionSample rect_sample_position(const AnalyticRec &r, V2 sample) {
    PositionSample ps;
    ps.p = xf_point_affine(r.to_world, v3(sample.x * 2.f - 1.f, sample.y * 2.f - 1.f, 0.f));
    ps.n = ld3(r.n); ps.pdf = r.inv_area; ps.uv = sample;
    return ps;
}

MIW_HD PositionSample mesh_sample_position(const MeshSampler &m, V2 sample) {
    uint32_t idx = distr_sample(m, sample.y);
    float pmf = m.pmf[idx] * m.normalization,
          cdf = idx > 0 ? m.cdf[idx - 1] * m.normalization : 0.f;
    sample.y = (sample.y - cdf) / pmf;

    const float *f = m.tri + 9 * (size_t) idx;
    V3 p0 = ld3(f), p1 = ld3(f + 3), p2 = ld3(f + 6);
    V3 e0 = p1 - p0, e1 = p2 - p0;
    V2 b = square_to_uniform_triangle(sample);

    PositionSample ps;
    ps.p = p0 + e0 * b.x + e1 * b.y;
    ps.pdf = m.normalization;
    ps.uv = b;
    if (m.vnorm) {
        const float *vn = m.vnorm + 9 * (size_t) idx;
        V3 n0 = ld3(vn), n1 = ld3(vn + 3), n2 = ld3(vn + 6);
        ps.n = normalize(n0 * (1.f - b.x - b.y) + n1 * b.x + n2 * b.y);
    } else {
        ps.n = normalize(cross(e0, e1));
    }
    return ps;
}

MIW_HD float face_area(V3 p0, V3 p1, V3 p2) { return 0.5f * norm(cross(p1 - p0, p2 - p0)); }

}
```

### mitsuba2_amd/csrc/miwave.hip

```cpp
#include <hip/hip_runtime.h>
#include <stdio.h>
#include <stdlib.h>
#include <string.h>
#include <stdarg.h>
#include <string>
#include <vector>
#include <chrono>
#include <atomic>
#include <cmath>
#include <map>
#include <string>
#include <algorithm>

#include "../../include/miwave.h"
#if defined(MIW_NESTED_PART) || defined(MIW_LIGHTS_PART)
#define MIW_KERNELS_ONLY 1
#endif
#if defined(MIW_SECTION_PROFILE)
__device__ unsigned long long g_sections[16];
#endif
#if defined(MIW_PHASE_STATS)
__device__ unsigned long long g_phase_stats[15];
#endif
#if defined(MIW_WALK_STATS)
// ... 488 lines not shown
            uint32_t vi = s->faces[3 * f + k];
            if (vi >= s->vertex_count) return fail(c, MI_ERR_INVALID, "face %u: vertex index out of range", f);
            float *dst = k == 0 ? t.p0 : (k == 1 ? t.p1 : t.p2);
            memcpy(dst, s->vertex_positions + 3 * (size_t) vi, 12);
            if (any_normals && (c->shapes[face_shape[f]].flags & 1u))
                memcpy(&c->tri_vn_in[(size_t) f * 9 + 3 * k], s->vertex_normals + 3 * (size_t) vi, 12);
        }
        t.shape = face_shape[f]; t.prim = f; t.pad = 0;
    }
    c->bsdfs.resize(s->bsdf_count);
    for (uint32_t i = 0; i < s->bsdf_count; ++i) {
        const mi_bsdf &b = s->bsdfs[i];
        BsdfRec r; int slot = 0;
        if (s->bsdf_table_floats && !s->bsdf_tables) return fail(c, MI_ERR_INVALID, "scene: bsdf_table_floats without bsdf_tables");
        if (const char *why = bsdf_record_from_abi(b, s->bitmap_count, s->bsdf_table_floats, r, &slot))
            return slot < 0 ? fail(c, MI_ERR_INVALID, "bsdf %u: %s", i, why) : fail(c, MI_ERR_INVALID, "bsdf %u: texture %d: %s", i, slot, why);
        if (!(b.flags & MI_BSDF_FLAG_TWOSIDED) && b.type != BSDF_TYPE_MASK && b.type != BSDF_TYPE_BLEND) r.back = 0;
        c->bsdfs[i] = r;
    }
    for (uint32_t i = 0; i < s->bsdf_count; ++i)
        if (const char *why = bsdf_chain_check(c->bsdfs, i, s->bitmaps)) return fail(c, MI_ERR_INVALID, "bsdf %u: %s", i, why);
    c->diffuse_only = true;
    for (const BsdfRec &r : c->bsdfs) if (r.type != BSDF_TYPE_DIFFUSE || (r.flags & BSDF_REC_TWOSIDED)) c->diffuse_only = false;
    if (!c->tri_uv_in.empty()) c->diffuse_only = false;
    for (const BsdfRec &r : c->bsdfs) if (bsdf_uses_bitmap(r)) c->diffuse_only = false;
    {
        std::vector<BitmapRec> recs; uint32_t bad = 0;
        if (const char *why = build_bitmap_table(s, recs, &bad)) return fail(c, MI_ERR_INVALID, "bitmap %u: %s", bad, why);
        std::vector<size_t> first(recs.size() + 1, 0);
        for (size_t i = 0; i < recs.size(); ++i) first[i + 1] = first[i] + (size_t) recs[i].width * recs[i].height * recs[i].channels;
        HIP_TRY(c, c->d_bitmap_data.resize(std::max<size_t>(first.back(), 1)));
        for (size_t i = 0; i < recs.size(); ++i) {
            HIP_TRY(c, hipMemcpyAsync(c->d_bitmap_data.p + first[i], recs[i].data, (first[i + 1] - first[i]) * sizeof(float), hipMemcpyHostToDevice, c->stream));
            recs[i].data = c->d_bitmap_data.p + first[i];
        }
        HIP_TRY(c, hipStreamSynchronize(c->stream));
        HIP_TRY(c, c->d_bitmaps.upload(recs, c->stream));
        c->bitmap_count = (uint32_t) recs.size();
    }
    c->trio = true;
    for (const BsdfRec &r : c->bsdfs) if (r.type != BSDF_TYPE_DIFFUSE && r.type != BSDF_TYPE_DIELECTRIC && r.type != BSDF_TYPE_ROUGHCONDUCTOR) c->trio = false;
    c->textured = !c->tri_uv_in.empty();
    for (const BsdfRec &r : c->bsdfs) if (bsdf_uses_bitmap(r) || bsdf_is_extended(r)) c->textured = true;
    c->nested = false;
    for (const BsdfRec &r : c->bsdfs) if (bsdf_is_nested(r)) c->nested = c->textured = true;
    c->bsdf_tables.assign(s->bsdf_tables, s->bsdf_tables + s->bsdf_table_floats);
    HIP_TRY(c, c->d_bsdf_tables.upload(c->bsdf_tables, c->stream));
    HIP_TRY(c, hipStreamSynchronize(c->stream));
    c->emitters.clear(); c->emit_tri.clear(); c->emit_vnorm.clear(); c->emit_pmf.clear(); c->emit_cdf.clear();
    bool any_emit_normals = false;
    auto push_env = [&]() { EmitterRec r; memset(&r, 0, sizeof r); r.type = EMITTER_ENVMAP; r.shape = 0xffffffffu; c->emitters.push_back(r); };
    c->lights.clear(); c->constant_light = -1; c->lights_on = s->light_count != 0;
    auto push_light = [&](uint32_t k) {
        const mi_light &l = s->lights[k];
        LightRec q; memset(&q, 0, sizeof q);
#if MIW_SPECTRAL
        memcpy(&q.value, &l.value_tex, sizeof(TexRec));
#else
        q.value.type = TEX_RGB; memcpy(q.value.v, l.value, 12);
#endif
        q.type = EMITTER_POINT + l.type; q.emitter_index = (uint32_t) c->emitters.size();
        memcpy(q.position, l.position, 12); memcpy(q.direction, l.direction, 12); memcpy(q.to_object, l.to_object, 64);
        q.cutoff_angle = l.cutoff_angle; q.cos_cutoff_angle = l.cos_cutoff_angle; q.cos_beam_width = l.cos_beam_width; q.inv_transition_width = l.inv_transition_width;
        q.dist = 2.f * light_bsphere_radius(l.bsphere_radius);
        EmitterRec r; memset(&r, 0, sizeof r); r.type = q.type; r.shape = 0xffffffffu; r.tri_first = (uint32_t) c->lights.size();
        if (l.type == MI_LIGHT_CONSTANT) c->constant_light = (int32_t) c->lights.size();
        c->lights.push_back(q); c->emitters.push_back(r);
    };
    auto push_specials = [&]() { while (c->emitters.size() < emitter_total && slot_light[c->emitters.size()] != -1) { const int32_t k = slot_light[c->emitters.size()]; if (k == -2) push_env(); else push_light((uint32_t) k); } };
    for (uint32_t i = 0; i < s->emitter_count; ++i) {
        if (s->light_count) push_specials();
        else if (s->envmap && s->envmap->emitter_index == i) push_env();
        const mi_emitter &e = s->emitters[i];
        if (e.shape >= s->shape_count) return fail(c, MI_ERR_INVALID, "emitter %u: shape index out of range", i);
        const mi_shape &sh = s->shapes[e.shape];
        if (sh.emitter != (int32_t) i) return fail(c, MI_ERR_INVALID, "emitter %u: shape %u does not point back to it", i, e.shape);
        if (sh.face_count == 0) return fail(c, MI_ERR_INVALID, "emitter %u: cannot create sampling table for an empty mesh", i);
        EmitterRec r; memset(&r, 0, sizeof r);
#if MIW_SPECTRAL
        if (e.radiance_tex.type != MI_TEX_D65 && e.radiance_tex.type != MI_TEX_SRGB_D65 && e.radiance_tex.type != MI_TEX_UNIFORM)
            return fail(c, MI_ERR_INVALID, "emitter %u: the scalar_spectral library needs a spectral radiance record", i);
        memcpy(&r.radiance, &e.radiance_tex, sizeof(TexRec));
#else
        r.radiance.type = TEX_RGB; memcpy(r.radiance.v, e.radiance, 12);
#endif
        if (shape_rect[e.shape] >= 0) {
            const AnalyticRec &q = c->rects[shape_rect[e.shape]];
            r.shape = e.shape; r.tri_first = (uint32_t) shape_rect[e.shape]; r.tri_count = 0; r.flags = 2u;
            r.valid_lo = r.valid_hi = 0; r.normalization = q.inv_area; r.sum = rcp(q.inv_area);
            c->emitters.push_back(r);
            continue;
        }
        r.shape = e.shape; r.tri_first = (uint32_t) c->emit_pmf.size(); r.tri_count = sh.face_count;
        r.flags = (sh.flags & MI_SHAPE_HAS_NORMALS) ? 1u : 0u;
        any_emit_normals = any_emit_normals || r.flags;
        double sum = 0.0; uint32_t vlo = 0xffffffffu, vhi = 0;
        for (uint32_t k = 0; k < sh.face_count; ++k) {
            const Tri &t = c->tris_in[sh.first_face + k];
            float area = face_area(ld3(t.p0), ld3(t.p1), ld3(t.p2));
            if (area < 0.f) return fail(c, MI_ERR_INVALID, "emitter %u: negative face area", i);
            c->emit_pmf.push_back(area);
            sum += (double) area;
            c->emit_cdf.push_back((float) sum);
            if (area > 0.f) { if (vlo == 0xffffffffu) vlo = k; vhi = k; }
            for (int q = 0; q < 3; ++q) c->emit_tri.push_back(t.p0[q]);
            for (int q = 0; q < 3; ++q) c->emit_tri.push_back(t.p1[q]);
            for (int q = 0; q < 3; ++q) c->emit_tri.push_back(t.p2[q]);
            for (int q = 0; q < 9; ++q)
                c->emit_vnorm.push_back(r.flags ? c->tri_vn_in[(size_t) (sh.first_face + k) * 9 + q] : 0.f);
        }
        if (vlo == 0xffffffffu) return fail(c, MI_ERR_INVALID, "emitter %u: no probability mass found", i);
        r.valid_lo = vlo; r.valid_hi = vhi;
        r.sum = (float) sum; r.normalization = (float) (1.0 / sum);
        c->emitters.push_back(r);
    }
    if (!any_emit_normals) c->emit_vnorm.clear();
    if (s->light_count) push_specials();
    else if (s->envmap && s->envmap->emitter_index >= s->emitter_count) push_env();
    if (c->lights_on) { c->nested = c->textured = true; c->diffuse_only = c->trio = false; }

    HIP_TRY(c, hipSetDevice(c->device));
    c->have_env = false;
#if MIW_SPECTRAL
    if (s->envmap && !s->envmap->density)
        return fail(c, MI_ERR_INVALID, "envmap: the scalar_spectral library needs mi_envmap::density (its texels are model coefficients, include/miwave.h)");
#endif
    if (s->envmap) {
        EnvmapTables t = envmap_build(*s->envmap);
        if (!t.ok) return fail(c, MI_ERR_INVALID, "envmap: needs >= 2x2 texels, a non-zero luminance sum and an invertible to_world");
        HIP_TRY(c, c->d_env_data.upload(t.data, c->stream));
        HIP_TRY(c, c->d_env_levels.upload(t.levels, c->stream));
        t.rec.data = c->d_env_data.p; t.rec.levels = c->d_env_levels.p;
        c->env_host = t.rec; c->env_levels_total = t.levels.size();
        std::vector<EnvmapRec> one(1, t.rec);
        HIP_TRY(c, c->d_env.upload(one, c->stream));
        HIP_TRY(c, hipStreamSynchronize(c->stream));
        c->have_env = true;
    }
    HIP_TRY(c, c->d_shapes.upload(c->shapes, c->stream));
    HIP_TRY(c, c->d_tri_uv.upload(c->tri_uv_in, c->stream));
    HIP_TRY(c, c->d_rects.upload(c->rects, c->stream));
    HIP_TRY(c, c->d_bsdfs.upload(c->bsdfs, c->stream));
    HIP_TRY(c, c->d_emitters.upload(c->emitters, c->stream));
    HIP_TRY(c, c->d_lights.upload(c->lights, c->stream));
    HIP_TRY(c, c->d_emit_tri.upload(c->emit_tri, c->stream));
    HIP_TRY(c, c->d_emit_vnorm.upload(c->emit_vnorm, c->stream));
    HIP_TRY(c, c->d_emit_pmf.upload(c->emit_pmf, c->stream));
    HIP_TRY(c, c->d_emit_cdf.upload(c->emit_cdf, c->stream));
    HIP_TRY(c, hipStreamSynchronize(c->stream));
    c->have_scene = true;
    return MI_OK;
}

#define MIW_LDS_PER_WORKGROUP (40u * 1024u)
#define MIW_LDS_STATIC 1024u
#define MIW_LDS_GRANULE 512u
static size_t lds_table_bytes(const mi_ctx *c, uint32_t words[10], bool with_tris) {
    words[0] = (uint32_t) (c->shapes.size() * sizeof(ShapeRec) / 4); words[1] = (uint32_t) (c->bsdfs.size() * sizeof(BsdfRec) / 4);
    words[2] = (uint32_t) (c->emitters.size() * sizeof(EmitterRec) / 4);
    words[3] = (uint32_t) c->emit_tri.size(); words[4] = (uint32_t) c->emit_vnorm.size(); words[5] = (uint32_t) c->emit_pmf.size(); words[6] = (uint32_t) c->emit_cdf.size();
    words[7] = with_tris ? (uint32_t) (c->tris_in.size() * sizeof(Tri) / 4) : 0u;
    words[8] = with_tris ? (uint32_t) c->tri_vn_in.size() : 0u; words[9] = with_tris ? (uint32_t) c->tri_uv_in.size() : 0u;
    size_t total = 0;
    for (int k = 0; k < 10; ++k) total += ((size_t) words[k] + 3u) / 4u * 16u;
    total += c->lights.size() * sizeof(LightRec);
    return total;
}

mi_status mi_bvh_build(mi_ctx *c, int32_t quality) {
    if (!c) return MI_ERR_INVALID;
    if (!c->have_scene) return fail(c, MI_ERR_STATE, "mi_bvh_build: no scene uploaded");
    const bool force_tree = (quality & MI_BVH_FORCE_TREE) != 0;
    const int32_t quality_flags = quality;
    quality &= ~(MI_BVH_FORCE_TREE | MI_BVH_NO_LEAF_FILTER | MI_BVH_RADIX_TREE);
    if (quality != 1 && quality != 0) return fail(c, MI_ERR_INVALID, "mi_bvh_build: quality must be 0 or 1");
    auto t0 = std::chrono::steady_clock::now();
    HIP_TRY(c, hipSetDevice(c->device));
    const float pad_unit = scene_pad_unit(c->tris_in);
    BvhBuildResult r;
    uint32_t node_count = 0, tri_count = (uint32_t) c->tris_in.size(), depth = 0;
    bool built_on_device = false;
    bool wide_on_device = false; uint32_t dev4_nodes = 0, dev4_stack = 0;
    const bool wide_on = !(c->opt.get("MIW_BVH4") && atoi(c->opt.get("MIW_BVH4")) == 0);
    const bool wide8_on = wide_on && !(c->opt.get("MIW_BVH8") && atoi(c->opt.get("MIW_BVH8")) == 0) && !c->opt.get("MIW_BVH4_FAN");
    uint32_t dev8_nodes = 0, dev8_depth = 0; double ms_bvh8 = 0.0;
    std::vector<uint32_t> sah_level_start;
    int max_fan = 4;
    if (const char *e = c->opt.get("MIW_BVH4_FAN")) max_fan = std::min(4, std::max(2, atoi(e)));
    double ms_bvh4 = 0.0;
    uint32_t tab_words_[10];
    const bool tiny = c->tris_in.size() <= MIW_BRUTE_MAX_TRIS && !force_tree && c->rects.empty() &&
                      (!MIW_LDS_TABLES || lds_table_bytes(c, tab_words_, true) <= 24u * 1024u);
    if (quality == 0 && !tiny && tri_count >= 2) {
        hipStream_t s = c->stream;
        const int n = (int) tri_count;
        TmpBuf<Tri> d_in; TmpBuf<float> d_vn_in; TmpBuf<uint64_t> d_keys, d_keys_sorted; TmpBuf<uint32_t> d_bounds, d_arrivals, d_height, d_span, d_first;
        uint32_t lbvh_leaf = 2u;
        if (const char *e = c->opt.get("MIW_LBVH_LEAF")) lbvh_leaf = (uint32_t) std::min(16, std::max(1, atoi(e)));
        if ((uint32_t) n <= lbvh_leaf) lbvh_leaf = 1u;
        TmpBuf<LbvhBox> d_boxes; TmpBuf<LbvhLinks> d_inner; TmpBuf<int32_t> d_leaf_parent; TmpBuf<unsigned char> d_tmp;
        auto free_tmp = [&]() { d_in.release(); d_vn_in.release(); d_keys.release(); d_keys_sorted.release(); d_bounds.release();
                                d_arrivals.release(); d_height.release(); d_boxes.release(); d_inner.release(); d_leaf_parent.release(); d_tmp.release();
                                d_span.release(); d_first.release(); };
        auto lap_t = std::chrono::steady_clock::now();
        auto lap = [&](const char *what) {
            if (!c->opt.get("MIW_DEBUG_ALLOC")) return;
            (void) hipStreamSynchronize(s);
            const auto now = std::chrono::steady_clock::now();
            fprintf(stderr, "[miwave]   build set-up: %-28s %8.2f ms\n", what, std::chrono::duration<double, std::milli>(now - lap_t).count());
            lap_t = now;
        };
        HIP_TRY(c, d_in.upload(c->tris_in, s));
        lap("triangle upload");
        if (!c->tri_vn_in.empty()) HIP_TRY(c, d_vn_in.upload(c->tri_vn_in, s));
        lap("vertex-normal upload");
        HIP_TRY(c, c->d_nodes.resize(n)); HIP_TRY(c, c->d_tris.resize(n)); HIP_TRY(c, d_height.resize(n));
        if (!c->tri_vn_in.empty()) HIP_TRY(c, c->d_tri_vn.resize((size_t) n * 9));
        lap("node / triangle buffers");
        const dim3 blk(256), grd((unsigned) ((n + 255) / 256));
        enum { DEV_SAH = 0, DEV_LBVH = 1 } dev_builder = (quality_flags & MI_BVH_RADIX_TREE) ? DEV_LBVH : DEV_SAH;
        if (const char *e = c->opt.get("MIW_DEVICE_BUILDER")) {
            if (!strcmp(e, "lbvh")) dev_builder = DEV_LBVH; else if (!strcmp(e, "sah")) dev_builder = DEV_SAH;
        }
        bool sah_need_host = false;
        if (dev_builder == DEV_SAH) {
            uint32_t max_leaf = 4u;
            if (const char *e = c->opt.get("MIW_MAX_LEAF")) max_leaf = (uint32_t) std::min(16, std::max(1, atoi(e)));
            const uint32_t un = (uint32_t) n;
            const float pad = 2.f * pad_unit;
            TmpBuf<SahPrim> d_prim; TmpBuf<uint32_t> d_ia, d_ib, d_flags, d_rank; TmpBuf<SahCand> d_ca, d_cb; TmpBuf<SahDecision> d_dec; TmpBuf<SahState> d_state;
            TmpBuf<unsigned char> d_scan_tmp; TmpBuf<SahHuge> d_huge;
            HIP_TRY(c, d_huge.resize(MIW_SAH_HUGE_CANDS));
            HIP_TRY(c, d_prim.resize(un)); HIP_TRY(c, d_ia.resize(un)); HIP_TRY(c, d_ib.resize(un)); HIP_TRY(c, d_flags.resize(un)); HIP_TRY(c, d_rank.resize(un));
            HIP_TRY(c, d_ca.resize(un)); HIP_TRY(c, d_cb.resize(un)); HIP_TRY(c, d_dec.resize(un)); HIP_TRY(c, d_state.resize(1));
            size_t scan_bytes = 0;
            HIP_TRY(c, rocprim::exclusive_scan(nullptr, scan_bytes, d_flags.p, d_rank.p, 0u, (size_t) n, rocprim::plus<uint32_t>(), s));
            HIP_TRY(c, d_scan_tmp.resize(scan_bytes + 16));
            lap("builder temporaries");
            HIP_TRY(c, hipStreamSynchronize(s));
            const auto t_setup = std::chrono::steady_clock::now();
            hipLaunchKernelGGL(k_sah_prims, grd, blk, 0, s, d_in.p, un, pad, d_prim.p, d_ia.p);
            const SahCand root = { 0u, un, -1, 0u };
            HIP_TRY(c, hipMemcpyAsync(d_ca.p, &root, sizeof root, hipMemcpyHostToDevice, s));
            HIP_TRY(c, hipMemsetAsync(d_state.p, 0, sizeof(SahState), s));
            std::vector<uint32_t> level_start{ 0u };
            uint32_t n_cand = 1u, base = 0u, level = 0u;
            bool big_left = true;
            uint32_t level_max = un;
            const bool huge_on = !(c->opt.get("MIW_SAH_HUGE") && atoi(c->opt.get("MIW_SAH_HUGE")) == 0);
            while (n_cand > 0u && !sah_need_host) {
                const SahCand *cur = (level & 1u) ? d_cb.p : d_ca.p; SahCand *nxt = (level & 1u) ? d_ca.p : d_cb.p;
                const uint32_t *ic = (level & 1u) ? d_ib.p : d_ia.p; uint32_t *in = (level & 1u) ? d_ia.p : d_ib.p;
                const bool all_big = n_cand <= 512u;
                const uint32_t none = 0u, all = 0xffffffffu;
                const bool huge = huge_on && level_max > MIW_SAH_HUGE && n_cand <= MIW_SAH_HUGE_CANDS;
                if (huge) {
                    const dim3 hgrid(n_cand, (level_max + MIW_SAH_SLICE - 1u) / MIW_SAH_SLICE);
                    const uint32_t words = n_cand * (uint32_t) (sizeof(SahHuge) / 4u);
                    hipLaunchKernelGGL(k_sah_huge_init, dim3((words + 255u) / 256u), dim3(256), 0, s, d_huge.p, n_cand);
                    hipLaunchKernelGGL(k_sah_huge_box, hgrid, dim3(1024), 0, s, cur, n_cand, ic, d_prim.p, d_huge.p);
                    hipLaunchKernelGGL(k_sah_huge_bins, hgrid, dim3(1024), 0, s, cur, n_cand, ic, d_prim.p, level, d_huge.p);
                    hipLaunchKernelGGL(k_sah_huge_finish, dim3(n_cand), dim3(64), 0, s, cur, n_cand, level, max_leaf, d_huge.p, d_dec.p, d_flags.p, d_state.p);
                }
                if (all_big || big_left) hipLaunchKernelGGL(k_sah_decide<1024>, dim3(n_cand), dim3(1024), 0, s, cur, n_cand, ic, d_prim.p, level, max_leaf, d_dec.p, d_flags.p, d_state.p, all_big ? none : MIW_SAH_BIG, huge ? MIW_SAH_HUGE : all);
                if (!all_big) hipLaunchKernelGGL(k_sah_decide<64>, dim3(n_cand), dim3(64), 0, s, cur, n_cand, ic, d_prim.p, level, max_leaf, d_dec.p, d_flags.p, d_state.p, none, big_left ? MIW_SAH_BIG : all);
                HIP_TRY(c, rocprim::exclusive_scan(d_scan_tmp.p, scan_bytes, d_flags.p, d_rank.p, 0u, (size_t) n_cand, rocprim::plus<uint32_t>(), s));
                hipLaunchKernelGGL(k_sah_totals, dim3(1), dim3(1), 0, s, d_flags.p, d_rank.p, n_cand, d_state.p);
                if (all_big || big_left) hipLaunchKernelGGL(k_sah_apply<1024>, dim3(n_cand), dim3(1024), 0, s, cur, n_cand, ic, in, d_prim.p, d_dec.p, d_rank.p, base, c->d_nodes.p, nxt, d_state.p, all_big ? none : MIW_SAH_BIG, all, un);
                if (!all_big) hipLaunchKernelGGL(k_sah_apply<64>, dim3(n_cand), dim3(64), 0, s, cur, n_cand, ic, in, d_prim.p, d_dec.p, d_rank.p, base, c->d_nodes.p, nxt, d_state.p, none, big_left ? MIW_SAH_BIG : all, un);
                SahState h;
                HIP_TRY(c, hipMemcpyAsync(&h, d_state.p, sizeof h, hipMemcpyDeviceToHost, s));
                HIP_TRY(c, hipStreamSynchronize(s));
                HIP_TRY(c, hipGetLastError());
                sah_need_host = h.need_host != 0u || level >= 62u || (uint64_t) base + h.n_inner > (uint64_t) un - 1u;
                big_left = h.max_count > MIW_SAH_BIG; level_max = h.max_count;
                if (big_left) HIP_TRY(c, hipMemsetAsync(&d_state.p->max_count, 0, sizeof(uint32_t), s));
                depth = level;
                base += h.n_inner; level_start.push_back(base);
                n_cand = 2u * h.n_inner; ++level;
            }
            const auto t_levels = std::chrono::steady_clock::now();
            if (!sah_need_host) {
                for (size_t L = level_start.size() - 1; L-- > 0;) {
                    const uint32_t cnt = level_start[L + 1] - level_start[L];
                    if (cnt) hipLaunchKernelGGL(k_sah_heights, dim3((cnt + 255u) / 256u), blk, 0, s, c->d_nodes.p, level_start[L], level_start[L + 1], d_height.p);
                }
                const uint32_t *idx_final = (level & 1u) ? d_ib.p : d_ia.p;
                hipLaunchKernelGGL(k_sah_gather, grd, blk, 0, s, d_in.p, c->tri_vn_in.empty() ? (const float *) nullptr : d_vn_in.p, idx_final, un,
                                   c->d_tris.p, c->tri_vn_in.empty() ? (float *) nullptr : c->d_tri_vn.p);
                HIP_TRY(c, hipGetLastError());
                HIP_TRY(c, hipStreamSynchronize(s));
                node_count = base;
                built_on_device = true;
                sah_level_start = level_start;
                c->counters.bvh_builder = 3u;
                if (c->opt.get("MIW_DEBUG")) {
                    auto ms = [](std::chrono::steady_clock::time_point a, std::chrono::steady_clock::time_point b) { return std::chrono::duration<double, std::milli>(b - a).count(); };
                    fprintf(stderr, "[miwave] device builder: binned SAH by levels, %u triangles, %u inner nodes, depth %u; upload + allocations %.2f ms, %u levels %.2f ms, heights + gather %.2f ms\n",
                            un, node_count, depth, ms(t0, t_setup), level, ms(t_setup, t_levels), ms(t_levels, std::chrono::steady_clock::now()));
                }
            }
        } else {
            HIP_TRY(c, d_keys.resize(n)); HIP_TRY(c, d_keys_sorted.resize(n)); HIP_TRY(c, d_bounds.resize(6));
            HIP_TRY(c, d_arrivals.resize(n)); HIP_TRY(c, d_boxes.resize((size_t) 2 * n));
            HIP_TRY(c, d_inner.resize(n)); HIP_TRY(c, d_leaf_parent.resize(n)); HIP_TRY(c, d_span.resize(n)); HIP_TRY(c, d_first.resize(n));
            const uint32_t init_bounds[6] = { 0xffffffffu, 0xffffffffu, 0xffffffffu, 0u, 0u, 0u };
            HIP_TRY(c, hipMemcpyAsync(d_bounds.p, init_bounds, sizeof init_bounds, hipMemcpyHostToDevice, s));
            HIP_TRY(c, hipMemsetAsync(d_arrivals.p, 0, (size_t) n * sizeof(uint32_t), s));
            HIP_TRY(c, hipMemsetAsync(d_height.p, 0, (size_t) n * sizeof(uint32_t), s));
            hipLaunchKernelGGL(k_lbvh_bounds, dim3(std::min<unsigned>(grd.x, 1024u)), blk, 0, s, d_in.p, (uint32_t) n, d_bounds.p);
            hipLaunchKernelGGL(k_lbvh_morton, grd, blk, 0, s, d_in.p, (uint32_t) n, d_bounds.p, d_keys.p);
            size_t tmp_bytes = 0;
            HIP_TRY(c, rocprim::radix_sort_keys(nullptr, tmp_bytes, d_keys.p, d_keys_sorted.p, (size_t) n, 0u, 64u, s));
            HIP_TRY(c, d_tmp.resize(tmp_bytes + 16));
            HIP_TRY(c, rocprim::radix_sort_keys(d_tmp.p, tmp_bytes, d_keys.p, d_keys_sorted.p, (size_t) n, 0u, 64u, s));
            uint32_t hb[6];
            HIP_TRY(c, hipMemcpyAsync(hb, d_bounds.p, sizeof hb, hipMemcpyDeviceToHost, s));
            HIP_TRY(c, hipStreamSynchronize(s));
            float m = 0.f;
            for (int k = 0; k < 6; ++k) { uint32_t o = hb[k]; float f = u2f((o & 0x80000000u) ? (o & 0x7fffffffu) : ~o); m = std::max(m, std::fabs(f)); }
            const float pad = 2.f * std::max(1e-5f * m, 1e-30f);
            HIP_TRY(c, hipMemsetAsync(d_height.p, 0, (size_t) n * sizeof(uint32_t), s));
            hipLaunchKernelGGL(k_lbvh_leaves, grd, blk, 0, s, d_in.p, c->tri_vn_in.empty() ? (const float *) nullptr : d_vn_in.p, d_keys_sorted.p,
                               (uint32_t) n, pad, c->d_tris.p, c->tri_vn_in.empty() ? (float *) nullptr : c->d_tri_vn.p, d_boxes.p);
            hipLaunchKernelGGL(k_lbvh_tree, grd, blk, 0, s, d_keys_sorted.p, n, d_inner.p, d_leaf_parent.p, d_span.p, d_first.p);
            hipLaunchKernelGGL(k_lbvh_fit, grd, blk, 0, s, d_inner.p, d_leaf_parent.p, n, d_boxes.p, d_arrivals.p, d_height.p, d_span.p, lbvh_leaf);
            hipLaunchKernelGGL(k_lbvh_emit, grd, blk, 0, s, d_inner.p, d_boxes.p, n, c->d_nodes.p, d_span.p, d_first.p, lbvh_leaf);
            HIP_TRY(c, hipGetLastError());
            HIP_TRY(c, hipMemcpyAsync(&depth, d_height.p, sizeof depth, hipMemcpyDeviceToHost, s));
            HIP_TRY(c, hipStreamSynchronize(s));
            c->counters.bvh_builder = 1u;
            if (c->opt.get("MIW_DEBUG")) fprintf(stderr, "[miwave] device builder: LBVH, %u triangles, height %u\n", (uint32_t) n, depth);
        node_count = (uint32_t) (n - 1);
        built_on_device = depth <= MIW_BVH_MAX_DEPTH;
        }
        const uint32_t budget4 = MIW_STACK_ENTRIES - 1;
        if (built_on_device && wide_on && depth <= budget4 && !c->opt.get("MIW_NO_STACK") && !c->opt.get("MIW_BVH4_HOST")) {
            auto t4 = std::chrono::steady_clock::now();
            TmpBuf<Bvh4Item> fa, fb; TmpBuf<Bvh4Levels> lv;
            HIP_TRY(c, fa.resize(n)); HIP_TRY(c, fb.resize(n)); HIP_TRY(c, lv.resize(1)); HIP_TRY(c, c->d_nodes4.resize(n));
            Bvh4Levels h; memset(&h, 0, sizeof h); h.count[0] = 1;
            const Bvh4Item root = { 0, budget4 };
            HIP_TRY(c, hipMemcpyAsync(lv.p, &h, sizeof h, hipMemcpyHostToDevice, s));
            HIP_TRY(c, hipMemcpyAsync(fa.p, &root, sizeof root, hipMemcpyHostToDevice, s));
            const uint32_t levels = std::min<uint32_t>(depth + 1u, 62u);
            for (uint32_t L = 0; L < levels; ++L)
                hipLaunchKernelGGL(k_bvh4_level, grd, blk, 0, s, c->d_nodes.p, d_height.p, (L & 1u) ? fb.p : fa.p, (L & 1u) ? fa.p : fb.p, lv.p,
                                   c->d_nodes4.p, L, budget4, max_fan);
            HIP_TRY(c, hipGetLastError());
            HIP_TRY(c, hipMemcpyAsync(&h, lv.p, sizeof h, hipMemcpyDeviceToHost, s));
            HIP_TRY(c, hipStreamSynchronize(s));
            for (uint32_t L = 0; L < levels; ++L) dev4_nodes += h.count[L];
            dev4_stack = h.stack_bound;
            wide_on_device = !h.failed && h.count[levels] == 0 && dev4_stack <= budget4 && dev4_nodes <= (uint32_t) n;
            ms_bvh4 = std::chrono::duration<double, std::milli>(std::chrono::steady_clock::now() - t4).count();
        }
        if (built_on_device && dev_builder == DEV_SAH && wide8_on && !c->opt.get("MIW_NO_STACK")) {
            auto t8 = std::chrono::steady_clock::now();
            TmpBuf<Bvh8Dp> d_dp; TmpBuf<int32_t> ga, gb; TmpBuf<Bvh8Levels> lv8; TmpBuf<uint32_t> d_perm;
            HIP_TRY(c, d_dp.resize(node_count)); HIP_TRY(c, ga.resize(n)); HIP_TRY(c, gb.resize(n)); HIP_TRY(c, lv8.resize(1)); HIP_TRY(c, d_perm.resize(n));
            HIP_TRY(c, c->d_nodes8.resize(n)); HIP_TRY(c, c->d_tris8.resize(n));
            if (!c->tri_vn_in.empty()) HIP_TRY(c, c->d_tri_vn8.resize((size_t) n * 9));
            for (size_t L = sah_level_start.size() - 1; L-- > 0;) {
                const uint32_t cnt = sah_level_start[L + 1] - sah_level_start[L];
                if (cnt) hipLaunchKernelGGL(k_bvh8_dp, dim3((cnt + 255u) / 256u), blk, 0, s, c->d_nodes.p, d_dp.p, sah_level_start[L], sah_level_start[L + 1]);
            }
            Bvh8Levels h8; memset(&h8, 0, sizeof h8); h8.count[0] = 1;
            const int32_t root8 = 0;
            HIP_TRY(c, hipMemcpyAsync(lv8.p, &h8, sizeof h8, hipMemcpyHostToDevice, s));
            HIP_TRY(c, hipMemcpyAsync(ga.p, &root8, sizeof root8, hipMemcpyHostToDevice, s));
            const uint32_t levels8 = std::min<uint32_t>(depth + 1u, 62u);
            for (uint32_t L = 0; L < levels8; ++L)
                hipLaunchKernelGGL(k_bvh8_level, grd, blk, 0, s, c->d_nodes.p, d_dp.p, (L & 1u) ? gb.p : ga.p, (L & 1u) ? ga.p : gb.p, lv8.p,
                                   c->d_nodes8.p, d_perm.p, L, (uint32_t) n, (uint32_t) n);
            hipLaunchKernelGGL(k_bvh8_gather, grd, blk, 0, s, c->d_tris.p, c->tri_vn_in.empty() ? (const float *) nullptr : c->d_tri_vn.p, d_perm.p, (uint32_t) n,
                               c->d_tris8.p, c->tri_vn_in.empty() ? (float *) nullptr : c->d_tri_vn8.p);
            HIP_TRY(c, hipGetLastError());
            HIP_TRY(c, hipMemcpyAsync(&h8, lv8.p, sizeof h8, hipMemcpyDeviceToHost, s));
            HIP_TRY(c, hipStreamSynchronize(s));
            uint32_t nn = 0, dd = 0;
            for (uint32_t L = 0; L < levels8; ++L) { nn += h8.count[L]; dd += h8.count[L] ? 1u : 0u; }
            if (!h8.failed && h8.count[levels8] == 0 && h8.tri_next == (uint32_t) n && dd <= MIW_BVH8_STACK && nn <= (uint32_t) n) { dev8_nodes = nn; dev8_depth = dd; }
            ms_bvh8 = std::chrono::duration<double, std::milli>(std::chrono::steady_clock::now() - t8).count();
        }
        free_tmp();
    }
    std::vector<float> vn;
    if (!built_on_device) {
        uint32_t max_leaf = tiny ? MIW_BRUTE_MAX_LEAF : 4u;
        if (const char *e = c->opt.get("MIW_MAX_LEAF")) max_leaf = (uint32_t) atoi(e);
        r = bvh_build_sah(c->tris_in, -1.f, max_leaf);
        if (r.depth > MIW_BVH_MAX_DEPTH) return fail(c, MI_ERR_INVALID, "BVH depth %u exceeds the traversal trail", r.depth);
        if (!c->tri_vn_in.empty()) {
            vn.resize(c->tri_vn_in.size());
            for (size_t i = 0; i < r.order.size(); ++i)
                memcpy(&vn[i * 9], &c->tri_vn_in[(size_t) r.order[i] * 9], 36);
        }
        HIP_TRY(c, c->d_nodes.upload(r.nodes, c->stream));
        HIP_TRY(c, c->d_tris.upload(r.tris, c->stream));
        HIP_TRY(c, c->d_tri_vn.upload(vn, c->stream));
        HIP_TRY(c, hipStreamSynchronize(c->stream));
        node_count = (uint32_t) r.nodes.size(); tri_count = (uint32_t) r.tris.size(); depth = r.depth;
    }
    c->counters.bvh_on_device = built_on_device ? 1u : 0u;
    if (!built_on_device) c->counters.bvh_builder = 0u;

    SceneView &v = c->view;
    v.accept_pad = pad_unit;
    v.tri_bounds = nullptr;
    v.nodes = c->d_nodes.p; v.node_count = node_count;
    v.tris = c->d_tris.p; v.tri_count = tri_count;
    v.tri_vn = c->tri_vn_in.empty() ? nullptr : c->d_tri_vn.p;
    v.tri_uv = c->tri_uv_in.empty() ? nullptr : c->d_tri_uv.p;
    v.bitmaps = c->bitmap_count ? c->d_bitmaps.p : nullptr;
    v.bsdf_tables = c->bsdf_tables.empty() ? nullptr : c->d_bsdf_tables.p;
    v.shapes = c->d_shapes.p; v.shape_count = (uint32_t) c->shapes.size();
    v.bsdfs = c->d_bsdfs.p; v.bsdf_count = (uint32_t) c->bsdfs.size();
    v.emitters = c->d_emitters.p; v.emitter_count = (uint32_t) c->emitters.size();
    scene_view_prepare(v);
    v.emit_tri = c->d_emit_tri.p; v.emit_vnorm = c->emit_vnorm.empty() ? nullptr : c->d_emit_vnorm.p;
    v.emit_pmf = c->d_emit_pmf.p; v.emit_cdf = c->d_emit_cdf.p;
    v.env = c->have_env ? c->d_env.p : nullptr;
    v.lights = c->lights.empty() ? nullptr : c->d_lights.p;
    v.constant = c->constant_light >= 0 ? c->d_lights.p + c->constant_light : nullptr;
    v.env_top = nullptr; v.env_top_count = v.env_top_base = 0;
    v.rects = c->rects.empty() ? nullptr : c->d_rects.p; v.rect_count = (uint32_t) c->rects.size();

    size_t all = (size_t) node_count * sizeof(BvhNode) + (size_t) tri_count * sizeof(Tri);
    c->lds_cfg.brute = 0; c->lds_cfg.leaves = 0; c->lds_cfg.stack = 0; c->lds_cfg.stack16 = 0; v.leaf_boxes = nullptr; v.nodes4 = nullptr; c->nodes4_count = c->nodes4_stack = 0;
    v.nodes8 = nullptr; c->nodes8_count = c->nodes8_depth = 0; bool wide8_on_device = false;
    if (tiny && v.tri_count > 0) {
        c->lds_cfg.brute = 1; c->lds_cfg.nodes_staged = 0; c->lds_cfg.tris_staged = v.tri_count;
        std::vector<LeafBox> leaves;
        auto add_leaf = [&](const float *lo, const float *hi, int32_t child) {
            if (child >= 0 || !(lo[0] <= hi[0])) return;
            const uint32_t code = (uint32_t) ~child;
            const uint32_t first = code >> 4, count = (code & 15u) + 1u;
            const unsigned long long bits = (count >= 64u ? ~0ull : ((1ull << count) - 1ull)) << first;
            LeafBox b; for (int a = 0; a < 3; ++a) { b.p[2 * a] = lo[a]; b.p[2 * a + 1] = hi[a]; } b.mask_lo = (uint32_t) bits; b.mask_hi = (uint32_t) (bits >> 32);
            leaves.push_back(b);
        };
        for (const BvhNode &n : r.nodes) { add_leaf(n.lo0, n.hi0, n.child0); add_leaf(n.lo1, n.hi1, n.child1); }
        HIP_TRY(c, c->d_leaf_boxes.upload(leaves, c->stream));
        HIP_TRY(c, hipStreamSynchronize(c->stream));
        v.leaf_boxes = c->d_leaf_boxes.p;
        c->lds_cfg.leaves = (quality_flags & MI_BVH_NO_LEAF_FILTER) ? 0u : (uint32_t) leaves.size();
        std::vector<TriBounds> bounds(v.tri_count);
        for (uint32_t i = 0; i < v.tri_count; ++i)
            bounds[i] = tri_bounds(ld3(r.tris[i].p0), ld3(r.tris[i].p1), ld3(r.tris[i].p2), v.accept_pad);
        HIP_TRY(c, c->d_tri_bounds.upload(bounds, c->stream));
        HIP_TRY(c, hipStreamSynchronize(c->stream));
        v.tri_bounds = c->d_tri_bounds.p;
        c->lds_bytes = v.tri_count * sizeof(TriPacket) + leaves.size() * MIW_LEAF_BOX_COPIES * sizeof(LeafBox) + v.tri_count * sizeof(TriBounds);
    } else {
        const bool stack_ok = depth <= MIW_STACK_ENTRIES && !c->opt.get("MIW_NO_STACK");
        const bool resident_tree = all <= 16 * 1024 && (!stack_ok || v.tri_count <= MIW_BRUTE_MAX_TRIS);
        if (resident_tree) { c->lds_cfg.nodes_staged = v.node_count; c->lds_cfg.tris_staged = v.tri_count; }
        else { c->lds_cfg.nodes_staged = MIW_LDS_TOP ? std::min<uint32_t>(v.node_count, 255) : 0u; c->lds_cfg.tris_staged = 0; }
        c->lds_bytes = c->lds_cfg.nodes_staged * sizeof(BvhNode) + c->lds_cfg.tris_staged * sizeof(Tri);
        c->lds_cfg.stack = 0; c->lds_cfg.stack16 = 0;
        if (!resident_tree && stack_ok) {
            c->lds_cfg.stack = 1; c->lds_cfg.stack16 = (uint32_t) (c->lds_bytes / 16);
            c->lds_bytes += (size_t) MIW_STACK_ENTRIES * MIW_BLOCK * sizeof(int32_t);
        }
        if (c->lds_cfg.stack && wide_on && wide_on_device) {
            v.nodes4 = c->d_nodes4.p; c->nodes4_count = dev4_nodes; c->nodes4_stack = dev4_stack;
            if (c->opt.get("MIW_DEBUG")) fprintf(stderr, "[miwave] bvh4 (device): %u nodes (bvh2 %u), stack bound %u, %.2f ms\n", dev4_nodes, node_count, dev4_stack, ms_bvh4);
        } else if (c->lds_cfg.stack && wide_on) {
            auto t4 = std::chrono::steady_clock::now();
            if (built_on_device) {
                r.nodes.resize(node_count);
                HIP_TRY(c, hipMemcpy(r.nodes.data(), c->d_nodes.p, (size_t) node_count * sizeof(BvhNode), hipMemcpyDeviceToHost));
            }
            const Bvh4BuildResult b4 = bvh4_collapse(r.nodes, MIW_STACK_ENTRIES - 1, max_fan);
            if (b4.ok) {
                HIP_TRY(c, c->d_nodes4.upload(b4.nodes, c->stream));
                HIP_TRY(c, hipStreamSynchronize(c->stream));
                v.nodes4 = c->d_nodes4.p; c->nodes4_count = (uint32_t) b4.nodes.size(); c->nodes4_stack = b4.stack_bound;
            }
            ms_bvh4 = std::chrono::duration<double, std::milli>(std::chrono::steady_clock::now() - t4).count();
            if (c->opt.get("MIW_DEBUG")) fprintf(stderr, "[miwave] bvh4: %zu nodes (bvh2 %u), depth %u, stack bound %u, ok %d\n", b4.nodes.size(), node_count, b4.depth, b4.stack_bound, (int) b4.ok);
        }
        if (c->lds_cfg.stack && v.nodes4 && dev8_nodes) {
            c->nodes8_count = dev8_nodes; c->nodes8_depth = dev8_depth; wide8_on_device = true;
            if (c->opt.get("MIW_DEBUG")) fprintf(stderr, "[miwave] bvh8 (device): %u nodes (bvh2 %u, bvh4 %u), depth %u, %.2f ms\n", dev8_nodes, node_count, c->nodes4_count, dev8_depth, ms_bvh8);
        } else if (c->lds_cfg.stack && v.nodes4 && wide8_on && !built_on_device) {
            auto t8 = std::chrono::steady_clock::now();
            const Bvh8BuildResult b8 = bvh8_collapse(r.nodes, tri_count);
            if (b8.ok) {
                std::vector<Tri> t8v(b8.perm.size()); std::vector<float> vn8;
                for (size_t i = 0; i < t8v.size(); ++i) t8v[i] = r.tris[b8.perm[i]];
                if (!vn.empty()) { vn8.resize(vn.size()); for (size_t i = 0; i < t8v.size(); ++i) memcpy(&vn8[i * 9], &vn[(size_t) b8.perm[i] * 9], 36); }
                HIP_TRY(c, c->d_nodes8.upload(b8.nodes, c->stream)); HIP_TRY(c, c->d_tris8.upload(t8v, c->stream)); HIP_TRY(c, c->d_tri_vn8.upload(vn8, c->stream));
                HIP_TRY(c, hipStreamSynchronize(c->stream));
                c->nodes8_count = (uint32_t) b8.nodes.size(); c->nodes8_depth = b8.depth;
            }
            ms_bvh8 = std::chrono::duration<double, std::milli>(std::chrono::steady_clock::now() - t8).count();
            if (c->opt.get("MIW_DEBUG")) fprintf(stderr, "[miwave] bvh8: %zu nodes (bvh2 %u), depth %u, ok %d, %.2f ms\n", b8.nodes.size(), node_count, b8.depth, (int) b8.ok, ms_bvh8);
        }
    }

    if (c->nodes8_count == 0) { c->d_nodes8.release(); c->d_tris8.release(); c->d_tri_vn8.release(); }
    else if (c->d_nodes8.n > 2 * (size_t) c->nodes8_count) {
        DevBuf<Bvh8Node> fit;
        HIP_TRY(c, fit.resize(c->nodes8_count));
        HIP_TRY(c, hipMemcpyAsync(fit.p, c->d_nodes8.p, (size_t) c->nodes8_count * sizeof(Bvh8Node), hipMemcpyDeviceToDevice, c->stream));
        HIP_TRY(c, hipStreamSynchronize(c->stream));
        c->d_nodes8.release(); c->d_nodes8 = fit;
    }

    c->counters.ms_bvh_build = std::chrono::duration<double, std::milli>(std::chrono::steady_clock::now() - t0).count();
    c->counters.bvh_nodes = v.node_count; c->counters.bvh_tris = v.tri_count; c->counters.bvh_depth = depth;
    c->counters.bvh4_on_device = (v.nodes4 && wide_on_device) ? 1u : 0u; c->counters.ms_bvh4 = ms_bvh4;
    c->counters.bvh8_nodes = c->nodes8_count; c->counters.bvh8_depth = c->nodes8_depth; c->counters.bvh8_on_device = wide8_on_device ? 1u : 0u; c->counters.ms_bvh8 = ms_bvh8;
    c->have_bvh = true;
    return MI_OK;
}

mi_status mi_trace(mi_ctx *c, const mi_rays_soa *rays, const mi_hits_soa *hits, uint64_t n, int32_t any_hit) {
    if (!c || !rays || !hits) return MI_ERR_INVALID;
    if (!c->have_bvh) return fail(c, MI_ERR_STATE, "mi_trace: call mi_scene_upload and mi_bvh_build first");
    if (n == 0) return MI_OK;
    if (!hits->t) return fail(c, MI_ERR_INVALID, "mi_trace: hits->t is required");
    HIP_TRY(c, hipSetDevice(c->device));
    TmpBuf<float> in, out; TmpBuf<uint32_t> outu;
    HIP_TRY(c, in.resize(8 * n)); HIP_TRY(c, out.resize(3 * n)); HIP_TRY(c, outu.resize(2 * n));
    const float *src[8] = { rays->ox, rays->oy, rays->oz, rays->dx, rays->dy, rays->dz, rays->mint, rays->maxt };
    for (int k = 0; k < 8; ++k) {
        if (!src[k]) return fail(c, MI_ERR_INVALID, "mi_trace: null ray array");
        HIP_TRY(c, hipMemcpyAsync(in.p + k * n, src[k], n * sizeof(float), hipMemcpyHostToDevice, c->stream));
    }
    SoaRays R = { in.p, in.p + n, in.p + 2 * n, in.p + 3 * n, in.p + 4 * n, in.p + 5 * n, in.p + 6 * n, in.p + 7 * n };
    SoaHits H = { out.p, out.p + n, out.p + 2 * n, outu.p, outu.p + n };
    dim3 grid((unsigned) ((n + MIW_BLOCK - 1) / MIW_BLOCK)), block(MIW_BLOCK);
    if (any_hit) hipLaunchKernelGGL(k_trace_soa<true>, grid, block, c->lds_bytes, c->stream, c->view, R, H, n, c->lds_cfg);
    else         hipLaunchKernelGGL(k_trace_soa<false>, grid, block, c->lds_bytes, c->stream, c->view, R, H, n, c->lds_cfg);
    HIP_TRY(c, hipGetLastError());
    HIP_TRY(c, hipMemcpyAsync(hits->t, out.p, n * sizeof(float), hipMemcpyDeviceToHost, c->stream));
    if (hits->u) HIP_TRY(c, hipMemcpyAsync(hits->u, out.p + n, n * sizeof(float), hipMemcpyDeviceToHost, c->stream));
    if (hits->v) HIP_TRY(c, hipMemcpyAsync(hits->v, out.p + 2 * n, n * sizeof(float), hipMemcpyDeviceToHost, c->stream));
    if (hits->prim) HIP_TRY(c, hipMemcpyAsync(hits->prim, outu.p, n * sizeof(uint32_t), hipMemcpyDeviceToHost, c->stream));
    if (hits->shape) HIP_TRY(c, hipMemcpyAsync(hits->shape, outu.p + n, n * sizeof(uint32_t), hipMemcpyDeviceToHost, c->stream));
    HIP_TRY(c, hipStreamSynchronize(c->stream));
    return MI_OK;
}

mi_status mi_ray_intersect(mi_ctx *c, const mi_rays_soa *rays, mi_surface_interaction *si, uint64_t n) {
    if (!c || !rays || !si) return MI_ERR_INVALID;
    if (!c->have_bvh) return fail(c, MI_ERR_STATE, "mi_ray_intersect: call mi_scene_upload and mi_bvh_build first");
    if (n == 0) return MI_OK;
    HIP_TRY(c, hipSetDevice(c->device));
    TmpBuf<float> in; TmpBuf<mi_surface_interaction> out;
    HIP_TRY(c, in.resize(8 * n)); HIP_TRY(c, out.resize(n));
    const float *src[8] = { rays->ox, rays->oy, rays->oz, rays->dx, rays->dy, rays->dz, rays->mint, rays->maxt };
    for (int k = 0; k < 8; ++k) {
        if (!src[k]) return fail(c, MI_ERR_INVALID, "mi_ray_intersect: null ray array");
        HIP_TRY(c, hipMemcpyAsync(in.p + k * n, src[k], n * sizeof(float), hipMemcpyHostToDevice, c->stream));
    }
    SoaRays R = { in.p, in.p + n, in.p + 2 * n, in.p + 3 * n, in.p + 4 * n, in.p + 5 * n, in.p + 6 * n, in.p + 7 * n };
    hipLaunchKernelGGL(k_ray_intersect, dim3((unsigned) ((n + MIW_BLOCK - 1) / MIW_BLOCK)), dim3(MIW_BLOCK), c->lds_bytes, c->stream, c->view, R, out.p, n, c->lds_cfg);
    HIP_TRY(c, hipGetLastError());
    HIP_TRY(c, hipMemcpyAsync(si, out.p, n * sizeof(mi_surface_interaction), hipMemcpyDeviceToHost, c->stream));
    HIP_TRY(c, hipStreamSynchronize(c->stream));
    return MI_OK;
}

mi_status mi_sample_emitter_direction(mi_ctx *c, int32_t emitter, const float *ref_p, const float *sample, const float *wavelengths,
                                      int32_t test_visibility, mi_direction_sample *ds, float *spec_out, uint64_t n) {
    if (!c || !ref_p || !sample || !ds || !spec_out) return MI_ERR_INVALID;
    if (!c->have_bvh) return fail(c, MI_ERR_STATE, "mi_sample_emitter_direction: call mi_scene_upload and mi_bvh_build first");
    if (emitter >= (int32_t) c->emitters.size()) return fail(c, MI_ERR_INVALID, "mi_sample_emitter_direction: emitter index out of range");
    if (MIW_SPECTRAL && !wavelengths) return fail(c, MI_ERR_INVALID, "mi_sample_emitter_direction: the scalar_spectral library needs wavelengths");
    if (n == 0) return MI_OK;
    HIP_TRY(c, hipSetDevice(c->device));
    TmpBuf<float> d_ref, d_smp, d_wl, d_spec; TmpBuf<mi_direction_sample> d_ds;
    HIP_TRY(c, d_ref.resize(3 * n)); HIP_TRY(c, d_smp.resize(2 * n)); HIP_TRY(c, d_spec.resize(MIW_SPEC_N * n)); HIP_TRY(c, d_ds.resize(n));
    HIP_TRY(c, hipMemcpyAsync(d_ref.p, ref_p, 3 * n * sizeof(float), hipMemcpyHostToDevice, c->stream));
    HIP_TRY(c, hipMemcpyAsync(d_smp.p, sample, 2 * n * sizeof(float), hipMemcpyHostToDevice, c->stream));
// ... 556 lines not shown
                        const uint32_t first = queued ? queued->beside : 0u, groups_all = ((uint32_t) n_tiles + 63u) / 64u;
                        const uint32_t waves_rest = (groups_all - first) * PC.patches_x * PC.patches_y;
                        if (waves_rest == 0u) { }
                        else if (fl_nt) MIW_TIMED(4, hipLaunchKernelGGL((k_film_lanes<4, 1>), dim3(waves_rest), dim3(64), lbytes, s, P.film, A, PC, (uint32_t) n_tiles, c->d_tiles.p, first, 0u));
                        else MIW_TIMED(4, hipLaunchKernelGGL((k_film_lanes<4, 0>), dim3(waves_rest), dim3(64), lbytes, s, P.film, A, PC, (uint32_t) n_tiles, c->d_tiles.p, first, 0u));
                        if (queued) { for (int i = 0; i < 3; ++i) HIP_TRY(c, hipStreamWaitEvent(s, c->ev_join[i], 0)); }
                    } else if (quads) {
                        PatchArgs PC = PA; PC.patches_x = (side + qw - 1) / qw; PC.patches_y = (side + qh - 1) / qh;
                        const uint32_t per_wave = 64u / qw, waves = (uint32_t) (((size_t) n_tiles * PC.patches_x * PC.patches_y + per_wave - 1u) / per_wave);
                        const size_t qbytes = (size_t) (c->classes.count + 1u) * (size_t) (5u + 2u * qh) * sizeof(float);
#define MIW_FQ_LAUNCH(GW, GH, U) MIW_TIMED(4, hipLaunchKernelGGL((k_film_quads<GW, GH, U>), dim3(waves), dim3(64), qbytes, s, P.film, A, PC, (uint32_t) n_tiles, c->d_tiles.p))
                        int fq_u = 4;
                        if (const char *e = ropt.get("MIW_FQ_U")) fq_u = atoi(e);
                        if (quads == 24) { if (fq_u == 8) MIW_FQ_LAUNCH(2, 4, 8); else if (fq_u == 2) MIW_FQ_LAUNCH(2, 4, 2); else MIW_FQ_LAUNCH(2, 4, 4); }
                        else if (quads == 42) { if (fq_u == 8) MIW_FQ_LAUNCH(4, 2, 8); else MIW_FQ_LAUNCH(4, 2, 4); }
                        else if (quads == 28) MIW_FQ_LAUNCH(2, 8, 4); else MIW_FQ_LAUNCH(4, 4, 4);
#undef MIW_FQ_LAUNCH
                    } else if (columns == 42) MIW_FC_LAUNCH(4, 2); else if (columns == 44) MIW_FC_LAUNCH(4, 4); else if (columns == 82) MIW_FC_LAUNCH(8, 2);
                    else if (group == 4) MIW_FG_LAUNCH(4, 4); else if (group == 2) MIW_FG_LAUNCH(2, 2); else MIW_FG_LAUNCH(4, 2);
#undef MIW_FC_LAUNCH
#undef MIW_FG_LAUNCH
                } else if (wide)
                    MIW_TIMED(4, hipLaunchKernelGGL(k_film_blocks<true>, fgrid, dim3(64), 0, s, P.film, A, PA, c->d_tiles.p));
                else
                    MIW_TIMED(4, hipLaunchKernelGGL(k_film_blocks<false>, fgrid, dim3(64), 0, s, P.film, A, PA, c->d_tiles.p));
            }
            MIW_TIMED(5, hipLaunchKernelGGL(k_film_merge, dim3(((uint32_t) cfg->crop_w + 255u) / 256u, (uint32_t) cfg->crop_h), dim3(256), 0, s,
                                            P.film, A, c->d_tiles.p, dst32, dst64, cfg->accumulate));
            HIP_TRY(c, hipGetLastError());
            HIP_TRY(c, hipStreamSynchronize(s));
        } else {
            dim3 block(256), grid((unsigned) ((film_n + 255) / 256));
            MIW_TIMED(4, hipLaunchKernelGGL(k_film_resolve, grid, block, 0, s, c->d_accum.p, dst32, dst64, film_n, cfg->accumulate));
        }
        if (staged) HIP_TRY(c, hipMemcpyAsync(film, c->d_out.p, film_n * elem, hipMemcpyDeviceToHost, s));
        HIP_TRY(c, hipGetLastError());
        HIP_TRY(c, hipStreamSynchronize(s));
        T.drain();
#if defined(MIW_DEBUG_POISON)
        if (result == MI_OK) {
            std::vector<unsigned char> host(film_n * elem);
            HIP_TRY(c, hipMemcpy(host.data(), dst, film_n * elem, hipMemcpyDeviceToHost));
            size_t bad = 0;
            for (size_t i = 0; i < film_n; ++i) bad += cfg->film_f64 ? std::isnan(((const double *) host.data())[i]) : std::isnan(((const float *) host.data())[i]);
            if (bad) return fail(c, MI_ERR_STATE, "render (poisoned build): %zu film values are NaN - a log / queue / tile slot was read before it was written", bad);
        }
#endif
    }
#undef MIW_TIMED
    return MI_OK;
}

mi_status mi_render(mi_ctx *c, const mi_render_cfg *cfg, void *film) {
    if (!c || !cfg || !film) return MI_ERR_INVALID;
    if (!c->have_bvh) return fail(c, MI_ERR_STATE, "mi_render: call mi_scene_upload and mi_bvh_build first");
    Options ropt = c->opt;
    switch (cfg->debug_film_replay) {
        case MI_FILM_REPLAY_AUTO: break;
        case MI_FILM_REPLAY_BLOCKS: ropt.v["MIW_FILM_LEGACY"] = "1"; break;
        case MI_FILM_REPLAY_GROUPS: ropt.v.erase("MIW_FILM_LEGACY"); ropt.v["MIW_FILM_LANES"] = "0"; ropt.v["MIW_FILM_QUADS"] = "0"; ropt.v["MIW_FILM_COLUMNS"] = "0"; break;
        case MI_FILM_REPLAY_COLUMNS: ropt.v.erase("MIW_FILM_LEGACY"); ropt.v["MIW_FILM_LANES"] = "0"; ropt.v["MIW_FILM_QUADS"] = "0"; ropt.v.erase("MIW_FILM_COLUMNS"); ropt.v.erase("MIW_FILM_GROUP"); break;
        case MI_FILM_REPLAY_QUADS: ropt.v.erase("MIW_FILM_LEGACY"); ropt.v["MIW_FILM_LANES"] = "0"; ropt.v.erase("MIW_FILM_COLUMNS"); ropt.v.erase("MIW_FILM_GROUP"); if (ropt.get("MIW_FILM_QUADS") && atoi(ropt.get("MIW_FILM_QUADS")) == 0) ropt.v.erase("MIW_FILM_QUADS"); break;
        case MI_FILM_REPLAY_LANES: ropt.v.erase("MIW_FILM_LEGACY"); ropt.v["MIW_FILM_LANES"] = "1"; break;
        case MI_FILM_REPLAY_LANES_PLAIN_LOG: ropt.v.erase("MIW_FILM_LEGACY"); ropt.v["MIW_FILM_LANES"] = "2"; break;
        default: return fail(c, MI_ERR_INVALID, "render: debug_film_replay must be one of MI_FILM_REPLAY_*");
    }
    if (cfg->debug_tree_width == 4) ropt.v["MIW_BVH8"] = "0";
    else if (cfg->debug_tree_width == 8) ropt.v.erase("MIW_BVH8");
    else if (cfg->debug_tree_width != 0) return fail(c, MI_ERR_INVALID, "render: debug_tree_width must be 0, 4 or 8");
    switch (cfg->debug_path_kernel) {
        case MI_PATH_KERNEL_AUTO: break;
        case MI_PATH_KERNEL_LOCKSTEP: ropt.v["MIW_PHASED"] = "0"; break;
        case MI_PATH_KERNEL_PHASED: ropt.v.erase("MIW_PHASED"); ropt.v["MIW_POOLED"] = "0"; break;
        case MI_PATH_KERNEL_POOLED: ropt.v.erase("MIW_PHASED"); ropt.v["MIW_POOLED"] = "1"; break;
        default: return fail(c, MI_ERR_INVALID, "render: debug_path_kernel must be one of MI_PATH_KERNEL_*");
    }
    RenderParams P;
    mi_status st = fill_params(c, cfg, P);
    if (st != MI_OK) return st;
    const uint32_t bs = (uint32_t) cfg->block_size, bs2 = bs * bs;
    uint32_t bs2_log2 = 0; while ((1u << bs2_log2) < bs2) ++bs2_log2;
    const uint32_t blocks_x = (cfg->crop_w + bs - 1) / bs, blocks_y = (cfg->crop_h + bs - 1) / bs;
    if (!cfg->block_ids || cfg->block_count != blocks_x * blocks_y)
        return fail(c, MI_ERR_INVALID, "render: block_ids must hold %u entries", blocks_x * blocks_y);
    uint32_t n_tiles = cfg->tile_list ? cfg->tile_count : cfg->block_count;
    if (cfg->tile_list)
        for (uint32_t i = 0; i < n_tiles; ++i)
            if (cfg->tile_list[i] >= cfg->block_count) return fail(c, MI_ERR_INVALID, "render: tile_list entry out of range");
    uint64_t n_lanes64 = (uint64_t) n_tiles * bs2;
    if (n_lanes64 >= (1ull << 31)) return fail(c, MI_ERR_INVALID, "render: too many lanes");
    const uint32_t n_lanes = (uint32_t) n_lanes64;
    P.n_lanes = n_lanes;
    const size_t film_n = (size_t) cfg->crop_w * cfg->crop_h * MIW_FILM_CHANNELS;

    HIP_TRY(c, hipSetDevice(c->device));
    hipStream_t s = c->stream;
    auto wall0 = std::chrono::steady_clock::now();
    c->cancel.store(0);

    int plan = cfg->plan;
    if (plan < 0 || plan > 2) return fail(c, MI_ERR_INVALID, "render: plan must be 0, 1 or 2");
    const bool lds_resident = c->lds_cfg.brute || (c->lds_cfg.nodes_staged >= c->view.node_count && c->lds_cfg.tris_staged >= c->view.tri_count);
    if (plan == 0) plan = (lds_resident || c->lds_cfg.stack || c->nested) ? 2 : 1;
    if (plan == 1 && c->lights_on) return fail(c, MI_ERR_INVALID, "render: scenes with point / spot / directional / constant emitters run the resident plan only (plan 0 or 2)");
    if (plan == 1 && c->nested) return fail(c, MI_ERR_INVALID, "render: scenes with mask / blendbsdf / null / thindielectric records run the resident plan only (plan 0 or 2)");
#if MIW_SPECTRAL
    if (cfg->plan == 1) return fail(c, MI_ERR_INVALID, "render: the scalar_spectral library runs the resident plan only (plan 0 or 2)");
    plan = 2;
#endif
    const bool direct = P.integrator == INTEG_DIRECT;
    if (direct) {
        if (cfg->plan == 1) return fail(c, MI_ERR_INVALID, "render: the direct integrator runs the resident plan only (plan 0 or 2)");
        plan = 2;
    }
    c->counters.plan = (uint32_t) plan;

    size_t nl = std::max<uint32_t>(n_lanes, 1);
    HIP_TRY(c, c->q_st.resize(nl)); HIP_TRY(c, c->q_pixel.resize(nl));
    if (plan == 1) {
        HIP_TRY(c, c->q_tp.resize(nl)); HIP_TRY(c, c->q_res.resize(nl)); HIP_TRY(c, c->q_ray_o.resize(nl));
        HIP_TRY(c, c->q_ray_d.resize(nl)); HIP_TRY(c, c->q_hit.resize(nl)); HIP_TRY(c, c->q_sh_d.resize(nl));
        HIP_TRY(c, c->q_sh_c.resize(nl)); HIP_TRY(c, c->q_pos.resize(nl)); HIP_TRY(c, c->q_sh_vis.resize(nl));
    }
    HIP_TRY(c, c->d_cnt.resize(MIW_CNT_SHARDS));
    HIP_TRY(c, hipMemsetAsync(c->d_cnt.p, 0, sizeof(Counters) * MIW_CNT_SHARDS, s));

    FilmPlan FP;
    FilmReplay replay;
    { const mi_status fs = plan_film_log(c, cfg, ropt, P, s, plan, n_tiles, n_lanes, bs2, bs2_log2, film_n, FP); if (fs != MI_OK) return fs; }
    const int film_mode = FP.film_mode; const bool rec16 = FP.rec16; const int film_lanes = FP.film_lanes; const uint32_t log_il = FP.log_il;
    HIP_TRY(c, c->d_block_ids.resize(cfg->block_count));
    HIP_TRY(c, hipMemcpyAsync(c->d_block_ids.p, cfg->block_ids, cfg->block_count * sizeof(uint32_t), hipMemcpyHostToDevice, s));
    if (cfg->tile_list && n_tiles) {
        HIP_TRY(c, c->d_tile_list.resize(n_tiles));
        HIP_TRY(c, hipMemcpyAsync(c->d_tile_list.p, cfg->tile_list, n_tiles * sizeof(uint32_t), hipMemcpyHostToDevice, s));
    }

    LaneQueues Q;
    Q.tp = c->q_tp.p; Q.res = c->q_res.p; Q.st = c->q_st.p; Q.pos = c->q_pos.p; Q.pixel = c->q_pixel.p;
    Q.ray_o = c->q_ray_o.p; Q.ray_d = c->q_ray_d.p; Q.hit = c->q_hit.p;
    Q.sh_d = c->q_sh_d.p; Q.sh_c = c->q_sh_c.p; Q.sh_vis = c->q_sh_vis.p;
    Q.log_pos = film_mode == 1 && !rec16 ? c->q_log_pos.p : nullptr; Q.log_val = film_mode == 1 && !rec16 ? c->q_log_val.p : nullptr;
    Q.lane_cost = nullptr; Q.lane_sorted = nullptr; Q.piece_list = nullptr; Q.simd_ids = nullptr; Q.piece_a = 64u; Q.piece_b = 1u;
    Q.log_rec = film_mode == 1 && rec16 ? c->q_log_rec.p : nullptr; Q.log_thr = rec16 ? c->d_fc_thr.p : nullptr; Q.log_rej = rec16 ? c->classes.count | ((film_mode == 1 ? log_il : 0u) << 8) : 0u;
    struct LdsLayout { TraceLds cfg; size_t rlds, rlds_plain, table_bytes; bool tables_fit; };
    const size_t lds_budget4 = MIW_LDS_PER_WORKGROUP - MIW_LDS_STATIC - MIW_LDS_GRANULE;
    auto lay_out = [&](size_t base, size_t env_cap, size_t lds_budget) {
        LdsLayout L; L.cfg = c->lds_cfg; L.rlds = base;
        L.cfg.thr16 = (uint32_t) ((L.rlds + 15) / 16);
        if (rec16) L.rlds = (size_t) L.cfg.thr16 * 16 + (MIW_FC_TABLE + 3) / 4 * 16;
        L.cfg.tab16 = (uint32_t) ((L.rlds + 15) / 16);
        L.table_bytes = lds_table_bytes(c, L.cfg.tab_words, c->lds_cfg.brute != 0);
        L.cfg.light_words = (uint32_t) (c->lights.size() * sizeof(LightRec) / 4);
        L.tables_fit = (size_t) L.cfg.tab16 * 16 + L.table_bytes <= (c->lds_cfg.brute ? 64u * 1024u : lds_budget);
        L.cfg.env_top_count = L.cfg.env_top_base = L.cfg.env_top_words = 0;
        if (L.tables_fit && c->have_env && !(ropt.get("MIW_ENV_TOP") && atoi(ropt.get("MIW_ENV_TOP")) == 0)) {
            const EnvmapRec &e = c->env_host;
            const size_t used = (size_t) L.cfg.tab16 * 16 + L.table_bytes;
            const size_t room = used < lds_budget ? std::min<size_t>(env_cap, lds_budget - used) : 0;
            uint32_t count = 0;
            while (count + 1 < e.n_levels && ((size_t) c->env_levels_total - e.level_offset[e.n_levels - 1 - count]) * 4 <= room) ++count;
            if (count) {
                L.cfg.env_top_count = count; L.cfg.env_top_base = e.level_offset[e.n_levels - count];
                L.cfg.env_top_words = (uint32_t) (c->env_levels_total - L.cfg.env_top_base);
                L.table_bytes += ((size_t) L.cfg.env_top_words + 3) / 4 * 16;
            }
        }
        L.rlds_plain = L.rlds;
        if (L.tables_fit) L.rlds = (size_t) L.cfg.tab16 * 16 + L.table_bytes;
        return L;
    };
    LdsLayout lay = lay_out(c->lds_bytes, 4096, lds_budget4);
    const bool pre8 = plan == 2 && cfg->integrator != MI_INTEGRATOR_DIRECT && !c->lds_cfg.brute && c->lds_cfg.stack && c->view.nodes4 && c->nodes8_count != 0u &&
                      !(ropt.get("MIW_BVH8") && atoi(ropt.get("MIW_BVH8")) == 0) && !(ropt.get("MIW_PHASED") && atoi(ropt.get("MIW_PHASED")) == 0) &&
                      !(ropt.get("MIW_PHASED_WAVES") && atoi(ropt.get("MIW_PHASED_WAVES")) != 4) && film_mode == 1;
    bool stack8_sized = false;
    if (pre8 && !(ropt.get("MIW_STACK8_FULL") && atoi(ropt.get("MIW_STACK8_FULL")) != 0)) {
        const size_t base8 = (size_t) c->lds_cfg.stack16 * 16 + (size_t) std::max<uint32_t>(c->nodes8_depth, 2u) * MIW_BLOCK * sizeof(U2);
        const LdsLayout lay8 = lay_out(base8, 12288, lds_budget4);
        if (lay8.tables_fit && base8 <= c->lds_bytes) { lay = lay8; stack8_sized = true; }
    }
    LdsLayout layp{}; bool pooled_fits = false;
    int pool_nw = 12, pool_pp = 1;
    if (const char *e = ropt.get("MIW_POOL_SHAPE")) { int a = 0, b = 0; if (sscanf(e, "%dx%d", &a, &b) == 2 && ((a == 12 && b == 1) || (a == 8 && b == 2))) { pool_nw = a; pool_pp = b; } }
    if (!(c->trio && !(ropt.get("MIW_TRIO") && atoi(ropt.get("MIW_TRIO")) == 0) && c->rects.empty() && !c->textured)) { pool_nw = 12; pool_pp = 1; }
    if (pre8 && ropt.get("MIW_POOLED") && atoi(ropt.get("MIW_POOLED")) != 0) {
        const size_t NJ = (size_t) pool_nw * pool_pp * 64u;
        size_t base = (size_t) std::max<uint32_t>(c->nodes8_depth, 2u) * NJ * sizeof(U2);
        const uint32_t pool16 = (uint32_t) (base / 16); base += 5u * NJ * 16u;
        const uint32_t stat16 = (uint32_t) (base / 16); base += NJ;
        layp = lay_out(base, 32768, (size_t) 160u * 1024u - 1024u);
        layp.cfg.stack16 = 0u; layp.cfg.pool16 = pool16; layp.cfg.stat16 = stat16; layp.cfg.nodes_staged = layp.cfg.tris_staged = 0u;
        pooled_fits = layp.tables_fit;
        if (ropt.get("MIW_DEBUG")) fprintf(stderr, "[miwave] pooled phase machine: %d wavefronts per workgroup x %d pixels per lane, LDS %zu bytes (stacks %zu, job records %zu, tables %zu of which environment warp levels %u), fits %d\n",
                                         pool_nw, pool_pp, layp.rlds, (size_t) pool16 * 16, 5u * NJ * 16u, layp.table_bytes, layp.cfg.env_top_words * 4u, (int) pooled_fits);
    }
    TraceLds rcfg = lay.cfg; size_t rlds = lay.rlds; const size_t rlds_plain = lay.rlds_plain, table_bytes = lay.table_bytes; const bool tables_fit = lay.tables_fit;
    if (ropt.get("MIW_DEBUG")) fprintf(stderr, "[miwave] LDS per workgroup: %zu bytes dynamic with the scene tables (%zu without), tables %zu B of which environment warp levels %u B, budget %zu%s\n",
                                     rlds, rlds_plain, table_bytes, rcfg.env_top_words * 4u, lds_budget4, stack8_sized ? "; stack sized for the 8-wide tree's depth" : "");

    mi_counters &K = c->counters;
    K.samples = K.segments = K.shadow_rays = K.iterations = 0; K.lanes = n_lanes;
    K.ms_trace_closest = K.ms_trace_any = K.ms_shade = K.ms_init = K.ms_resolve = K.ms_path = K.ms_film_blocks = K.ms_film_merge = K.ms_film_pack = 0;
    K.n_trace_closest = K.n_trace_any = K.n_shade = K.n_path = 0; K.path_kernel = 0; K.placed = 0; K.tree_width = 0; K.pooled = 0; K.pool_waves = 0; K.film_overlapped = 0; K.film_groups = 0; K.job_chunk = 0; K.job_chunks = 0; c->replay_enqueued = false; K.place_cost_max = K.place_cost_unit = K.place_max_pixel = K.place_measure_spp = 0; K.place_cost_mean = 0.0;

    LaunchTimer T{ c, K, cfg->profile != 0 };
#define MIW_TIMED(cls_, launch) do {                                                   \
        size_t e0_ = 0, e1_ = 0;                                                       \
        if (T.on) { HIP_TRY(c, T.get_event(e0_)); HIP_TRY(c, hipEventRecord(c->ev_pool[e0_], s)); } \
        launch;                                                                        \
        if (T.on) { HIP_TRY(c, T.get_event(e1_)); HIP_TRY(c, hipEventRecord(c->ev_pool[e1_], s)); \
                    T.stamps.push_back({ cls_, e0_, e1_ }); }                          \
    } while (0)

    mi_status result = MI_OK;
    auto read_counters = [&](Counters &sum) -> mi_status {
        HIP_TRY(c, hipMemcpyAsync(c->h_cnt, c->d_cnt.p, sizeof(Counters) * MIW_CNT_SHARDS, hipMemcpyDeviceToHost, s));
        HIP_TRY(c, hipStreamSynchronize(s));
        sum.segments = sum.samples = sum.shadow_rays = sum.active_lanes = 0;
        for (int i = 0; i < MIW_CNT_SHARDS; ++i) {
            sum.segments += c->h_cnt[i].segments; sum.samples += c->h_cnt[i].samples;
            sum.shadow_rays += c->h_cnt[i].shadow_rays; sum.active_lanes += c->h_cnt[i].active_lanes;
        }
        K.samples = sum.samples; K.segments = sum.segments; K.shadow_rays = sum.shadow_rays;
        return MI_OK;
    };
    auto out_of_time = [&]() {
        return cfg->timeout_s > 0.f &&
               std::chrono::duration<double>(std::chrono::steady_clock::now() - wall0).count() > cfg->timeout_s;
    };
    if (n_lanes > 0 && plan == 2) {
        dim3 grid((n_lanes + MIW_BLOCK - 1) / MIW_BLOCK), block(MIW_BLOCK);
        InitArgs A; A.block_ids = c->d_block_ids.p; A.tile_list = cfg->tile_list ? c->d_tile_list.p : nullptr;
        A.blocks_x = blocks_x; A.blocks_y = blocks_y; A.bs = bs; A.bs2_log2 = bs2_log2; A.base_seed = cfg->base_seed;
        MIW_TIMED(3, hipLaunchKernelGGL(k_init_pixels, grid, block, 0, s, P, c->q_st.p, c->q_pixel.p, A));
        HIP_TRY(c, hipGetLastError());
        const uint32_t n_simd = (uint32_t) c->cu_count * 4u;
        HIP_TRY(c, c->d_next_pixel.resize(std::max<uint32_t>(8u, n_simd)));
        const uint32_t per_launch = cfg->samples_per_launch > 0 ? (uint32_t) cfg->samples_per_launch : 128u;
        const bool tiny = c->lds_cfg.brute != 0;
        const bool phased_on = !(ropt.get("MIW_PHASED") && atoi(ropt.get("MIW_PHASED")) == 0);
        const bool trio_on = !(ropt.get("MIW_TRIO") && atoi(ropt.get("MIW_TRIO")) == 0);
        const bool trio_kernel = c->trio && trio_on && c->rects.empty() && !c->textured;
        const bool phased = phased_on && !direct && !tiny && c->lds_cfg.stack && (c->view.nodes4 != nullptr || trio_kernel) && (tables_fit || !MIW_LDS_TABLES);
        int ph_waves = 4;
        if (const char *e = ropt.get("MIW_PHASED_WAVES")) ph_waves = atoi(e) == 4 ? 4 : 3;
        const bool phased_placeable = phased && c->view.nodes4 != nullptr && ph_waves == 4;
        const bool phased8 = phased_placeable && c->nodes8_count != 0u && !(ropt.get("MIW_BVH8") && atoi(ropt.get("MIW_BVH8")) == 0);
        if (stack8_sized && !phased8) return fail(c, MI_ERR_STATE, "render: the LDS stack was sized for the 8-wide walk, which this launch does not run");
        SceneView view8 = c->view;
        if (phased8) { view8.nodes8 = c->d_nodes8.p; view8.tris = c->d_tris8.p; if (view8.tri_vn) view8.tri_vn = c->d_tri_vn8.p; }
        bool packet_shard4 = !phased && tiny && c->diffuse_only && !MIW_SPECTRAL && !direct && c->view.tri_count <= 32u && MIW_PACKET_WAVES > 4 && film_mode == 1 && n_lanes <= 64u * 4u * n_simd;
        if (const char *e = ropt.get("MIW_PACKET_SHARD4")) packet_shard4 = packet_shard4 && atoi(e) != 0;
        const uint32_t res_waves = phased ? (uint32_t) ph_waves : !tiny ? (uint32_t) MIW_TREE_WAVES : (c->diffuse_only && !MIW_SPECTRAL ? (c->view.tri_count <= 32u && !packet_shard4 ? (uint32_t) MIW_PACKET_WAVES : 4u) : (uint32_t) MIW_PACKET_WAVES_ALL);
        bool place = film_mode == 1 && !direct && (tiny || phased_placeable) && n_lanes >= 64u * n_simd / 2u && n_lanes <= 64u * res_waves * n_simd &&
                     cfg->spp >= 128u && per_launch >= cfg->spp && cfg->timeout_s <= 0.f;
        if (const char *e = ropt.get("MIW_PLACE")) place = place && atoi(e) != 0;
        uint32_t measure_div = 8u;
        if (const char *e = ropt.get("MIW_PLACE_MEASURE")) measure_div = (uint32_t) std::max(2, atoi(e));
        const uint32_t measure_end = place ? std::max<uint32_t>(16u, cfg->spp / measure_div) : 0u;
        const uint32_t n_pieces = (n_lanes + 63u) / 64u;
        size_t place_tmp_bytes = 0;
        if (place) {
            HIP_TRY(c, c->d_lane_cost.resize(n_lanes)); HIP_TRY(c, c->d_cost_sorted.resize(n_lanes)); HIP_TRY(c, c->d_lane_iota.resize(n_lanes));
            HIP_TRY(c, c->d_lane_sorted.resize((size_t) n_pieces * 64u));
            HIP_TRY(c, c->d_piece_list.resize((size_t) n_simd * MIW_PLACE_PIECES)); HIP_TRY(c, c->d_simd_ids.resize(1u + (1u << 14)));
            HIP_TRY(c, hipMemsetAsync(c->d_lane_cost.p, 0, n_lanes * sizeof(uint32_t), s));
            HIP_TRY(c, hipMemsetAsync(c->d_lane_sorted.p, 0xff, (size_t) n_pieces * 64u * sizeof(uint32_t), s));
            HIP_TRY(c, hipMemsetAsync(c->d_simd_ids.p, 0, c->d_simd_ids.n * sizeof(uint32_t), s));
            hipLaunchKernelGGL(k_iota, dim3((n_lanes + 255u) / 256u), dim3(256), 0, s, c->d_lane_iota.p, n_lanes);
            HIP_TRY(c, rocprim::radix_sort_pairs_desc(nullptr, place_tmp_bytes, c->d_lane_cost.p, c->d_cost_sorted.p, c->d_lane_iota.p, c->d_lane_sorted.p, (size_t) n_lanes, 0u, 32u, s));
            HIP_TRY(c, c->d_place_tmp.resize(place_tmp_bytes + 16));
        }
        TileArgs TA; memset(&TA, 0, sizeof TA);
        size_t tile_bytes = 0;
        if (film_mode == 2 && bs >= 16) {
            TA.tile_list = A.tile_list; TA.blocks_x = blocks_x; TA.bs = bs; TA.bs2_log2 = bs2_log2;
            TA.side = 16u + 2u * std::max<uint32_t>((uint32_t) cfg->filter_border, (uint32_t) floorf(cfg->filter_radius + .5f));
            TA.geom16 = (uint32_t) ((c->lds_bytes + 15) / 16);
            tile_bytes = (size_t) TA.geom16 * 16 - c->lds_bytes + (size_t) TA.side * TA.side * MIW_FILM_CHANNELS * sizeof(double);
            if (c->lds_bytes + tile_bytes > 64 * 1024) {
                HIP_TRY(c, hipFuncSetAttribute((const void *) k_path_resident<false, 1>, hipFuncAttributeMaxDynamicSharedMemorySize, (int) (c->lds_bytes + tile_bytes)));
                HIP_TRY(c, hipFuncSetAttribute((const void *) k_path_resident<false, 0>, hipFuncAttributeMaxDynamicSharedMemorySize, (int) (c->lds_bytes + tile_bytes)));
                HIP_TRY(c, hipFuncSetAttribute((const void *) k_path_resident<false, 1, MATS_ALL, false, INTEG_DIRECT>, hipFuncAttributeMaxDynamicSharedMemorySize, (int) (c->lds_bytes + tile_bytes)));
                HIP_TRY(c, hipFuncSetAttribute((const void *) k_path_resident<false, 0, MATS_ALL, true, INTEG_DIRECT>, hipFuncAttributeMaxDynamicSharedMemorySize, (int) (c->lds_bytes + tile_bytes)));
                HIP_TRY(c, hipFuncSetAttribute((const void *) k_path_resident<false, 1, MATS_NESTED>, hipFuncAttributeMaxDynamicSharedMemorySize, (int) (c->lds_bytes + tile_bytes)));
                HIP_TRY(c, hipFuncSetAttribute((const void *) k_path_resident<false, 1, MATS_LIGHTS>, hipFuncAttributeMaxDynamicSharedMemorySize, (int) (c->lds_bytes + tile_bytes)));
                HIP_TRY(c, hipFuncSetAttribute((const void *) k_path_resident<false, 0, MATS_NESTED>, hipFuncAttributeMaxDynamicSharedMemorySize, (int) (c->lds_bytes + tile_bytes)));
                HIP_TRY(c, hipFuncSetAttribute((const void *) k_path_resident<false, 0, MATS_LIGHTS>, hipFuncAttributeMaxDynamicSharedMemorySize, (int) (c->lds_bytes + tile_bytes)));
                HIP_TRY(c, hipFuncSetAttribute((const void *) k_path_resident<false, 1, MATS_NESTED, false, INTEG_DIRECT>, hipFuncAttributeMaxDynamicSharedMemorySize, (int) (c->lds_bytes + tile_bytes)));
                HIP_TRY(c, hipFuncSetAttribute((const void *) k_path_resident<false, 1, MATS_LIGHTS, false, INTEG_DIRECT>, hipFuncAttributeMaxDynamicSharedMemorySize, (int) (c->lds_bytes + tile_bytes)));
                HIP_TRY(c, hipFuncSetAttribute((const void *) k_path_resident<false, 0, MATS_NESTED, true, INTEG_DIRECT>, hipFuncAttributeMaxDynamicSharedMemorySize, (int) (c->lds_bytes + tile_bytes)));
                HIP_TRY(c, hipFuncSetAttribute((const void *) k_path_resident<false, 0, MATS_LIGHTS, true, INTEG_DIRECT>, hipFuncAttributeMaxDynamicSharedMemorySize, (int) (c->lds_bytes + tile_bytes)));
            }
        }
        const uint32_t sync_every = 8;
        uint32_t launches = 0;
        bool place_stats_due = false;
        int overlap_mode = 0;
        if (const char *e = ropt.get("MIW_FILM_OVERLAP")) overlap_mode = atoi(e);
        const bool overlap = overlap_mode != 0 && c->overlap_state != 0 && film_mode == 1 && FP.rec16 && FP.film_lanes != 0 && FP.log_il != 0 && !place && !phased  && tiny && c->diffuse_only && !MIW_SPECTRAL && !direct  &&
                             per_launch >= cfg->spp && cfg->timeout_s <= 0.f && n_tiles > 0;
        for (uint32_t done = 0; done < cfg->spp; ) {
            uint32_t end = cfg->spp - done < per_launch ? cfg->spp : done + per_launch;
            if (film_mode == 1) {
                HIP_TRY(c, hipMemsetAsync(c->d_next_pixel.p, 0, c->d_next_pixel.n * sizeof(uint32_t), s));
                rcfg.queues = 1u; Q.lane_cost = nullptr; Q.lane_sorted = nullptr; Q.piece_list = nullptr; Q.simd_ids = nullptr;
                if (overlap && done == 0) {
                    mi_status os = film_replay_setup(c, cfg, s, FP, n_tiles, bs, bs2_log2, blocks_x, blocks_y, replay);
                    if (os == MI_OK) os = overlap_prepare(c, cfg, s, n_tiles, bs, blocks_x, Q, bs2_log2);
                    if (os != MI_OK) return os;
                    if (Q.group_done) HIP_TRY(c, hipEventRecord(c->ev_fork, s));
                }
                Q.job_chunk = Q.job_pow = Q.job_total = 0u; Q.job_min = 0x80000000u;
                if ((tiny || (phased && MIW_PHASED_JOBS != 0)) && !pooled_fits && !place && !overlap && done == 0 && per_launch >= cfg->spp && cfg->timeout_s <= 0.f) {
                    uint32_t jmin = tiny ? 64u : 32u;
                    if (const char *e = ropt.get("MIW_JOB_CHUNK")) { const uint32_t v = (uint32_t) std::max(0, atoi(e)); jmin = (v & (v - 1u)) ? 0u : v; }
                    bool enough = (uint64_t) n_lanes * 5u >= (uint64_t) 6u * 64u * res_waves * n_simd;
                    if (const char *e = ropt.get("MIW_JOB_CHUNK_FORCE")) enough = enough || atoi(e) != 0;
                    uint32_t pow2 = 1u;
                    while (pow2 * 2u < cfg->spp) pow2 *= 2u;
                    uint64_t chunks = 1u;
                    for (uint32_t r = pow2; jmin && r >= jmin && r < cfg->spp; r >>= 1) ++chunks;
                    if (jmin && enough && chunks >= 2u && (uint64_t) n_lanes * chunks < (1ull << 31)) {
                        Q.job_chunk = jmin; Q.job_min = jmin; Q.job_pow = pow2; Q.job_total = (uint32_t) ((uint64_t) n_lanes * chunks);
                        K.job_chunk = jmin; K.job_chunks = (uint32_t) chunks;
                    }
                }
                if (place && done == 0) { end = measure_end; Q.lane_cost = c->d_lane_cost.p; Q.simd_ids = c->d_simd_ids.p; }
                else if (place) {
                    HIP_TRY(c, rocprim::radix_sort_pairs_desc(c->d_place_tmp.p, place_tmp_bytes, c->d_lane_cost.p, c->d_cost_sorted.p, c->d_lane_iota.p, c->d_lane_sorted.p, (size_t) n_lanes, 0u, 32u, s));
                    bool spread = phased && ((phased8 ? (size_t) c->nodes8_count * sizeof(Bvh8Node) : (size_t) c->nodes4_count * sizeof(Bvh4Node)) + (size_t) c->view.tri_count * sizeof(Tri)) > ((size_t) 32 << 20);
                    if (const char *e = ropt.get("MIW_PLACE_SPREAD")) spread = atoi(e) != 0;
                    Q.piece_a = spread ? 1u : 64u; Q.piece_b = spread ? n_pieces : 1u;
                    std::vector<uint32_t> &ids = c->h_simd_ids;
                    ids.resize(c->d_simd_ids.n);
                    HIP_TRY(c, hipMemcpyAsync(ids.data(), c->d_simd_ids.p, ids.size() * sizeof(uint32_t), hipMemcpyDeviceToHost, s));
                    HIP_TRY(c, hipStreamSynchronize(s));
                    place_stats_due = cfg->profile != 0;
                    uint32_t nqueues = 0;
                    for (size_t k = 1; k < ids.size(); ++k) ids[k] = ids[k] ? nqueues++ : 0xffffffffu;
                    ids[0] = 0u;
                    if (nqueues < 2u || (uint64_t) nqueues * MIW_PLACE_PIECES < n_pieces) nqueues = 0;
                    if (nqueues) {
                    std::vector<uint32_t> &list = c->h_piece_list;
                    list.assign((size_t) nqueues * MIW_PLACE_PIECES, 0xffffffffu);
                    for (uint32_t i = 0; i < n_pieces; ++i) {
                        const uint32_t round = i / nqueues, k = i % nqueues, qd = (round & 1u) ? nqueues - 1u - k : k;
                        list[(size_t) qd * MIW_PLACE_PIECES + round] = i;
                    }
                    HIP_TRY(c, c->d_piece_list.resize(list.size()));
                    HIP_TRY(c, hipMemcpyAsync(c->d_piece_list.p, list.data(), list.size() * sizeof(uint32_t), hipMemcpyHostToDevice, s));
                    HIP_TRY(c, hipMemcpyAsync(c->d_simd_ids.p, ids.data(), ids.size() * sizeof(uint32_t), hipMemcpyHostToDevice, s));
                    rcfg.queues = nqueues; Q.piece_list = c->d_piece_list.p; Q.lane_sorted = c->d_lane_sorted.p; Q.simd_ids = c->d_simd_ids.p;
                    K.placed = 1u;
                    }
                }
                unsigned wg_per_cu = std::max(4u, direct ? 4u : (unsigned) res_waves);
                if (const char *e = ropt.get("MIW_WG_PER_CU")) wg_per_cu = (unsigned) std::max(1, atoi(e));
                unsigned room = 0u;
                if (Q.group_done) { room = 32u; if (const char *e = ropt.get("MIW_FILM_OVERLAP_ROOM")) room = (unsigned) std::max(0, atoi(e)); }
                const unsigned resident = (unsigned) c->cu_count * (direct ? (unsigned) MIW_DIRECT_WAVES : (unsigned) res_waves);
                const unsigned full = room ? std::min((unsigned) c->cu_count * wg_per_cu, resident) : (unsigned) c->cu_count * wg_per_cu;
                const dim3 pgrid(std::min<unsigned>(grid.x, full > 2u * room ? full - room : full));
#define MIW_PATH_LAUNCH(T, M) MIW_TIMED(6, hipLaunchKernelGGL((k_path_resident<true, T, M, false>), pgrid, block, (T) != 0 ? rlds : rlds_plain, s, P, c->view, Q, (double *) nullptr, c->d_cnt.p, rcfg, end, TA, c->d_next_pixel.p))
                K.path_kernel = phased ? (c->view.nodes4 ? 1u : 3u) : 0u;
                const dim3 phgrid(std::min<unsigned>(grid.x, (unsigned) c->cu_count * (unsigned) ph_waves));
                rcfg.tail_prio = 1u;
                if (const char *e = ropt.get("MIW_TAIL_PRIO")) rcfg.tail_prio = atoi(e) ? 1u : 0u;
                TraceLds ph_cfg = rcfg;
                ph_cfg.shade_num = 2; ph_cfg.shade_den = c->have_env ? 4 : 3;
                if (const char *e = ropt.get("MIW_SHADE_VOTE")) { int a = 0, b = 0; if (sscanf(e, "%d:%d", &a, &b) == 2 && a > 0 && b > 0) { ph_cfg.shade_num = (uint32_t) a; ph_cfg.shade_den = (uint32_t) b; } }
                ph_cfg.node_exit = c->have_env ? 2u : 1u; ph_cfg.tri_exit = c->have_env ? 3u : 2u;
                if (const char *e = ropt.get("MIW_LOOP_EXIT")) { int a = 0, b = 0; if (sscanf(e, "%d:%d", &a, &b) == 2 && a >= 0 && b >= 0) { ph_cfg.node_exit = (uint32_t) a; ph_cfg.tri_exit = (uint32_t) b; } }
#define MIW_PHASED_LAUNCH_(M, A, WV, W, PL) MIW_TIMED(6, hipLaunchKernelGGL((k_path_phased<M, A, MIW_PHASE_SPEC != 0, WV, W, PL>), phgrid, block, rlds, s, P, (W) == 2 ? view8 : c->view, Q, c->d_cnt.p, ph_cfg, end, c->d_next_pixel.p))
#define MIW_PHASED_LAUNCH(M, A, W) do { if (ph_waves == 4) MIW_PHASED_LAUNCH_(M, A, 4, W, false); else MIW_PHASED_LAUNCH_(M, A, 3, W, false); } while (0)
                K.tree_width = phased ? (phased8 ? 8u : (c->view.nodes4 ? 4u : 2u)) : 0u;
#if MIW_SPECTRAL
                const bool pooled = false;
                if (pooled) { }
#else
                const bool pooled = phased8 && !place && pooled_fits;
                if (pooled) {
                    TraceLds pcfg = layp.cfg; pcfg.queues = 1u; pcfg.tail_prio = ph_cfg.tail_prio;
                    pcfg.shade_num = 48; pcfg.shade_den = 16; pcfg.node_exit = 40u; pcfg.tri_exit = 20u; pcfg.pool_claim_min = 8u;
                    if (const char *e = ropt.get("MIW_POOL_VOTE")) { int a = 0, b = 0, n = 0, t = 0, m = 0; if (sscanf(e, "%d:%d:%d:%d:%d", &a, &b, &n, &t, &m) == 5 && a > 0 && b >= 0) { pcfg.shade_num = (uint32_t) a; pcfg.shade_den = (uint32_t) b; pcfg.node_exit = (uint32_t) n; pcfg.tri_exit = (uint32_t) t; pcfg.pool_claim_min = (uint32_t) std::max(m, 1); } }
                    const unsigned NL = (unsigned) pool_nw * 64u;
                    const dim3 qgrid(std::min<unsigned>((n_lanes + NL - 1u) / NL, (unsigned) c->cu_count)), qblock(NL);
                    SceneView pview = view8;
#define MIW_POOLED_LAUNCH_(M, A, NW_, PP_) do { HIP_TRY(c, hipFuncSetAttribute((const void *) k_path_pooled<M, A, NW_, PP_>, hipFuncAttributeMaxDynamicSharedMemorySize, (int) layp.rlds)); \
                                     MIW_TIMED(6, hipLaunchKernelGGL((k_path_pooled<M, A, NW_, PP_>), qgrid, qblock, layp.rlds, s, P, pview, Q, c->d_cnt.p, pcfg, end, c->d_next_pixel.p)); } while (0)
#define MIW_POOLED_LAUNCH(M, A) do { if (pool_pp == 2) MIW_POOLED_LAUNCH_(M, A, 8, 2); else MIW_POOLED_LAUNCH_(M, A, 12, 1); } while (0)
                    if (c->lights_on) return fail(c, MI_ERR_INVALID, "render: the pooled kernel (MI_PATH_KERNEL_POOLED) does not serve scenes with point / spot / directional / constant emitters");
                    else if (c->nested) return fail(c, MI_ERR_INVALID, "render: the pooled kernel (MI_PATH_KERNEL_POOLED) does not serve scenes with mask / blendbsdf / null / thindielectric records");
                    else if (c->textured) MIW_POOLED_LAUNCH_(MATS_ALL, true, 12, 1);
                    else if (trio_kernel) MIW_POOLED_LAUNCH(MATS_TRIO, false);
                    else if (c->rects.empty()) MIW_POOLED_LAUNCH_(MATS_PLAIN, false, 12, 1);
                    else MIW_POOLED_LAUNCH_(MATS_PLAIN, true, 12, 1);
#undef MIW_POOLED_LAUNCH
#undef MIW_POOLED_LAUNCH_
                    K.pooled = 1u; K.pool_waves = (uint32_t) pool_nw;
                }
#endif
                else
                if (phased8 && place) {
                    if (c->lights_on) MIW_PHASED_LAUNCH_(MATS_LIGHTS, true, 4, 2, true);
                    else if (c->nested) MIW_PHASED_LAUNCH_(MATS_NESTED, true, 4, 2, true);
// ... 264 lines not shown
```

Before: 4458.

## Precompute per-triangle shading frames and emitter face normals into LDS tables

For packet (tiny) scenes on the queued path integrator, each workgroup now builds per-triangle frames (normal, dp/du, tangent basis) and per-emitter-face normals in LDS at kernel start. Hit shading and emitter position sampling then read these instead of recomputing cross products, normalizations and coordinate systems per hit. The extra LDS footprint can reduce how many workgroups fit per CU, so the host now derives the resident wave count from LDS usage and fails if the tables do not fit. The per-launch build also adds startup work to every block.

```diff
diff --git a/mitsuba2_amd/csrc/device/resident_kernel.h b/mitsuba2_amd/csrc/device/resident_kernel.h
--- a/mitsuba2_amd/csrc/device/resident_kernel.h
+++ b/mitsuba2_amd/csrc/device/resident_kernel.h
@@ -197,8 +197,9 @@
     extern __shared__ uint4 smem[];
     stage_to_lds(sc, cfg, smem);
     const float *thr = stage_thresholds(smem, cfg, UseLog && Q.log_rec ? Q.log_thr : nullptr);
+    constexpr bool Frames = MIW_LDS_TABLES && UseLog && Tiny != 0 && Integ != INTEG_DIRECT;
 #if MIW_LDS_TABLES
-    if constexpr (UseLog && Tiny != 0) stage_tables<true, mats_lights(Mats)>(sc, cfg, smem);
+    if constexpr (UseLog && Tiny != 0) stage_tables<true, mats_lights(Mats), mats_full(Mats), Frames>(sc, cfg, smem);
 #endif
 #if defined(MIW_SECTION_PROFILE) && defined(__HIP_DEVICE_COMPILE__)
     if ((threadIdx.x & 63u) == 0) { unsigned long long *b_ = miw_sec_buf(); for (int i = 0; i < 15; ++i) b_[i] = 0; b_[15] = __builtin_amdgcn_s_memtime(); }
@@ -227,7 +228,7 @@
         __shared__ uint32_t s_prog[MIW_BLOCK / 64];
         if (cfg.tail_prio) work.enable_tail_prio(sample_end, &s_prog[threadIdx.x >> 6]);
         if constexpr (Integ == INTEG_DIRECT) pixel_stream_render_direct<Mats, Analytic>(P, sc, sample_end, work, tr2, &local);
-        else pixel_stream_render<Mats, Analytic>(P, sc, sample_end, work, tr2, &local);
+        else pixel_stream_render<Mats, Analytic, Frames>(P, sc, sample_end, work, tr2, &local);
     } else if (lane < P.n_lanes) {
         U4 st = Q.st[lane];
         if (!(st.z & LF_DONE)) {
diff --git a/mitsuba2_amd/csrc/device/trace.h b/mitsuba2_amd/csrc/device/trace.h
--- a/mitsuba2_amd/csrc/device/trace.h
+++ b/mitsuba2_amd/csrc/device/trace.h
@@ -12,7 +12,7 @@
     uint32_t tail_prio;
     uint32_t thr16;
     uint32_t tab16;
-    uint32_t tab_words[10];
+    uint32_t tab_words[12];
     uint32_t env_top_count, env_top_base, env_top_words;
     uint32_t pool_claim_min;
     uint32_t pool16, stat16;
@@ -83,7 +83,7 @@
     return t;
 }
 
-template <bool WithTris, bool Lights = false>
+template <bool WithTris, bool Lights = false, bool Texcoords = false, bool BuildFrames = false>
 __device__ __forceinline__ void stage_tables(SceneView &sc, const TraceLds &cfg, uint4 *smem) {
     constexpr int N = WithTris ? 10 : 7;
     uint32_t *dst = reinterpret_cast<uint32_t *>(smem + cfg.tab16);
@@ -100,6 +100,26 @@
         for (uint32_t i = threadIdx.x; i < n; i += blockDim.x) dst[off + i] = src[k][i];
         off += (n + 3u) & ~3u;
     }
+    TriFrame *frames_at = reinterpret_cast<TriFrame *>(dst + off);
+    if constexpr (WithTris && BuildFrames) {
+        const uint32_t n_frames = cfg.tab_words[10] / (uint32_t) (sizeof(TriFrame) / 4);
+        for (uint32_t i = threadIdx.x; i < n_frames; i += blockDim.x) {
+            const Tri &tr = sc.tris[i];
+            const float *tc = (Texcoords && (sc.shapes[tr.shape].flags & SHAPE_HAS_TEXCOORDS)) ? sc.tri_uv + 6 * (size_t) tr.prim : nullptr;
+            frames_at[i] = tri_frame(ld3(tr.p0), ld3(tr.p1), ld3(tr.p2), tc);
+        }
+        off += (cfg.tab_words[10] + 3u) & ~3u;
+    }
+    float *face_n_at = reinterpret_cast<float *>(dst + off);
+    if constexpr (WithTris && BuildFrames) {
+        const uint32_t n_faces = cfg.tab_words[11] / 4u;
+        for (uint32_t f = threadIdx.x; f < n_faces; f += blockDim.x) {
+            const float *p = sc.emit_tri + 9 * (size_t) f;
+            const V3 n = face_normal(ld3(p), ld3(p + 3), ld3(p + 6));
+            face_n_at[4 * f] = n.x; face_n_at[4 * f + 1] = n.y; face_n_at[4 * f + 2] = n.z; face_n_at[4 * f + 3] = 0.f;
+        }
+        off += cfg.tab_words[11];
+    }
     uint32_t *lights_at = dst + off;
     if constexpr (Lights) {
         const uint32_t *lsrc = reinterpret_cast<const uint32_t *>(sc.lights);
@@ -126,6 +146,7 @@
     }
     if (WithTris) {
         sc.tris = reinterpret_cast<const Tri *>(at[7]); sc.tri_vn = reinterpret_cast<const float *>(at[8]); sc.tri_uv = reinterpret_cast<const float *>(at[9]);
+        if constexpr (BuildFrames) { sc.tri_frames = frames_at; sc.emit_face_n = face_n_at; }
     }
 }
 
diff --git a/mitsuba2_amd/csrc/miw/path.h b/mitsuba2_amd/csrc/miw/path.h
--- a/mitsuba2_amd/csrc/miw/path.h
+++ b/mitsuba2_amd/csrc/miw/path.h
@@ -234,7 +234,7 @@
 MIW_HD constexpr bool mats_full(int mats) { return mats == MATS_ALL || mats == MATS_NESTED || mats == MATS_LIGHTS; }
 MIW_HD constexpr bool mats_nested(int mats) { return mats == MATS_NESTED || mats == MATS_LIGHTS; }
 MIW_HD constexpr bool mats_lights(int mats) { return mats == MATS_LIGHTS; }
-template <int Mats = MATS_ALL, bool Analytic = true, typename PrevO, typename Cnt>
+template <int Mats = MATS_ALL, bool Analytic = true, bool Frames = false, typename PrevO, typename Cnt>
 MIW_HD int path_step(const RenderParams &P, const SceneView &sc, LaneRegs &L, F4 h, PrevO prev_o,
                      ShadowOut &sh, Cnt *cnt_local) {
     sh.has = false;
@@ -246,7 +246,7 @@
     SurfaceInteraction si;
     uint32_t bsdf_index = 0;
     int32_t emitter = -1;
-    if (valid) hit_surface_interaction<Analytic, mats_full(Mats)>(sc, tri_idx, h.x, h.y, h.z, prev_o, ray_d, si, bsdf_index, emitter);
+    if (valid) hit_surface_interaction<Analytic, mats_full(Mats), Frames>(sc, tri_idx, h.x, h.y, h.z, prev_o, ray_d, si, bsdf_index, emitter);
     else emitter = miss_emitter<mats_lights(Mats)>(sc);
     if (depth == 1 && valid) L.flags |= LF_VALID_RAY;
     MIW_SECTION(7);
@@ -298,7 +298,7 @@
 
     if (bflags & BSDF_Smooth) {
         DirectionSample ds;
-        Spec emitter_val = sample_emitter_direction<Analytic, mats_lights(Mats)>(sc, si.p, next_2d(L.rng), ds, L.wl);
+        Spec emitter_val = sample_emitter_direction<Analytic, mats_lights(Mats), Frames>(sc, si.p, next_2d(L.rng), ds, L.wl);
         if (ds.pdf != 0.f) {
             V3 wo = to_local(si.sh, ds.d);
             Spec bsdf_val = Mats == MATS_DIFFUSE ? diffuse_eval(*bsdf.b, si.wi, wo, tc) : bsdf_side_eval<Ext, Trio, Nested>(bsdf, si.wi, wo, tc);
@@ -383,7 +383,7 @@
 }
 #endif
 
-template <int Mats = MATS_ALL, bool Analytic = true, typename Work, typename Trace2, typename Cnt>
+template <int Mats = MATS_ALL, bool Analytic = true, bool Frames = false, typename Work, typename Trace2, typename Cnt>
 MIW_HD void pixel_stream_render(const RenderParams &P, const SceneView &sc, uint32_t sample_end, Work &work,
                                 Trace2 trace2, Cnt *cnt_local) {
     LaneRegs L;
@@ -417,7 +417,7 @@
         sh.has = false;
         int r = STEP_FINISHED;
         if (!dead_pending) {
-            r = path_step<Mats, Analytic>(P, sc, L, h, [o]() { return o; }, sh, cnt_local);
+            r = path_step<Mats, Analytic, Frames>(P, sc, L, h, [o]() { return o; }, sh, cnt_local);
             MIW_SECTION(4);
             if (r == STEP_DEAD_PENDING) { dead_pending = true; continue; }
             if (r == STEP_CONTINUE) continue;
diff --git a/mitsuba2_amd/csrc/miw/scene.h b/mitsuba2_amd/csrc/miw/scene.h
--- a/mitsuba2_amd/csrc/miw/scene.h
+++ b/mitsuba2_amd/csrc/miw/scene.h
@@ -58,6 +58,8 @@
     const struct Bvh4Node *nodes4;
     const struct Bvh8Node *nodes8;
     const float *env_top; uint32_t env_top_count, env_top_base;
+    const TriFrame *tri_frames;
+    const float *emit_face_n;
     const LightRec *lights;
     const LightRec *constant;
 };
@@ -69,7 +71,7 @@
 
 MIW_HD PrimCtx prim_ctx(const SceneView &sc) { PrimCtx c; c.rects = sc.rects; c.accept_pad = sc.accept_pad; return c; }
 
-template <bool Analytic, bool Texcoords, typename RayO>
+template <bool Analytic, bool Texcoords, bool Frames = false, typename RayO>
 MIW_HD void hit_surface_interaction(const SceneView &sc, uint32_t tri_idx, float t, float u, float v, RayO ray_o, V3 ray_d,
                                     SurfaceInteraction &si, uint32_t &bsdf_index, int32_t &emitter) {
     const Tri &tr = sc.tris[tri_idx];
@@ -81,7 +83,8 @@
     } else {
         const float *vn = (shape.flags & 1u) ? sc.tri_vn + 9 * (size_t) tri_idx : nullptr;
         const float *tc = (Texcoords && (shape.flags & SHAPE_HAS_TEXCOORDS)) ? sc.tri_uv + 6 * (size_t) tr.prim : nullptr;
-        compute_surface_interaction(ld3(tr.p0), ld3(tr.p1), ld3(tr.p2), vn, tc, t, u, v, ray_d, si);
+        if constexpr (Frames) compute_surface_interaction(ld3(tr.p0), ld3(tr.p1), ld3(tr.p2), vn, tc, sc.tri_frames[tri_idx], t, u, v, ray_d, si);
+        else compute_surface_interaction(ld3(tr.p0), ld3(tr.p1), ld3(tr.p2), vn, tc, t, u, v, ray_d, si);
     }
     si.shape = tr.shape; si.prim = tr.prim;
     emitter = shape.emitter; bsdf_index = shape.bsdf;
@@ -209,7 +212,7 @@
 MIW_HD Spec env_eval_spec(const EnvmapRec &e, V3 d, const Wavelengths &) { return env_eval(e, d); }
 #endif
 
-template <bool Analytic = true, bool Lights = false>
+template <bool Analytic = true, bool Lights = false, bool Frames = false>
 MIW_HD Spec emitter_sample_direction(const SceneView &sc, uint32_t index, V3 ref_p, V2 sample, DirectionSample &ds, const Wavelengths &wl) {
     const EmitterRec &e = sc.emitters[index];
     Spec value;
@@ -225,8 +228,10 @@
         if (Analytic && (e.flags & 2u) && sc.rects[e.tri_first].kind == ANALYTIC_SPHERE) {
             sphere_sample_direction(sc.rects[e.tri_first], ref_p, sample, ds);
         } else {
-            PositionSample ps = (Analytic && (e.flags & 2u)) ? rect_sample_position(sc.rects[e.tri_first], sample)
-                                                             : mesh_sample_position(emitter_mesh(sc, e), sample);
+            PositionSample ps;
+            if (Analytic && (e.flags & 2u)) ps = rect_sample_position(sc.rects[e.tri_first], sample);
+            else if constexpr (Frames) ps = mesh_sample_position(emitter_mesh(sc, e), sample, FaceNormalTable{ sc.emit_face_n + 4 * (size_t) e.tri_first });
+            else ps = mesh_sample_position(emitter_mesh(sc, e), sample);
             ds.p = ps.p; ds.n = ps.n; ds.pdf = ps.pdf;
             ds.d = ds.p - ref_p;
             float dist_squared = squared_norm(ds.d);
@@ -242,7 +247,7 @@
     return value;
 }
 
-template <bool Analytic = true, bool Lights = false>
+template <bool Analytic = true, bool Lights = false, bool Frames = false>
 MIW_HD Spec sample_emitter_direction(const SceneView &sc, V3 ref_p, V2 sample, DirectionSample &ds, const Wavelengths &wl) {
     if (sc.emitter_count == 0) {
         ds.p = ds.n = ds.d = v3(0.f); ds.dist = 0.f; ds.pdf = 0.f; ds.emitter = 0;
@@ -258,7 +263,7 @@
         index = i < sc.emitter_count - 1 ? i : sc.emitter_count - 1;
         sample.x = (sample.x - (float) index * emitter_pdf) * n;
     }
-    Spec value = emitter_sample_direction<Analytic, Lights>(sc, index, ref_p, sample, ds, wl);
+    Spec value = emitter_sample_direction<Analytic, Lights, Frames>(sc, index, ref_p, sample, ds, wl);
     if (sc.emitter_count > 1) {
         ds.pdf *= emitter_pdf;
         value = value * rcp(emitter_pdf);
diff --git a/mitsuba2_amd/csrc/miw/shape.h b/mitsuba2_amd/csrc/miw/shape.h
--- a/mitsuba2_amd/csrc/miw/shape.h
+++ b/mitsuba2_amd/csrc/miw/shape.h
@@ -142,6 +142,54 @@
     uint32_t shape, prim;
 };
 
+struct TriFrame { float n[3], dp_du[3], s[3], t[3]; };
+MIW_HD void st3(float *p, V3 v) { p[0] = v.x; p[1] = v.y; p[2] = v.z; }
+MIW_HD TriFrame tri_frame(V3 p0, V3 p1, V3 p2, const float *tc) {
+    V3 dp0 = p1 - p0, dp1 = p2 - p0;
+    const V3 n = normalize(cross(dp0, dp1));
+    V3 dp_du, dp_dv;
+    coordinate_system(n, dp_du, dp_dv);
+    if (tc) {
+        const V2 uv0 = v2(tc[0], tc[1]), uv1 = v2(tc[2], tc[3]), uv2 = v2(tc[4], tc[5]);
+        const V2 duv0 = v2(uv1.x - uv0.x, uv1.y - uv0.y), duv1 = v2(uv2.x - uv0.x, uv2.y - uv0.y);
+        const float det = fmsub(duv0.x, duv1.y, duv0.y * duv1.x), inv_det = rcp(det);
+        if (det != 0.f) {
+            dp_du = fmsub3(dp0, duv1.y, dp1 * duv0.y) * inv_det;
+            dp_dv = fnmadd3(dp0, duv1.x, dp1 * duv0.x) * inv_det;
+        }
+    }
+    (void) dp_dv;
+    const V3 s = normalize(fnmadd3(n, dot(n, dp_du), dp_du));
+    const V3 t = cross(n, s);
+    TriFrame f;
+    st3(f.n, n); st3(f.dp_du, dp_du); st3(f.s, s); st3(f.t, t);
+    return f;
+}
+MIW_HD void compute_surface_interaction(V3 p0, V3 p1, V3 p2, const float *vn, const float *tc, const TriFrame &frame,
+                                        float t, float b1, float b2, V3 ray_d,
+                                        SurfaceInteraction &si) {
+    float b0 = 1.f - b1 - b2;
+    si.t = t;
+    si.p = p0 * b0 + p1 * b1 + p2 * b2;
+    si.n = ld3(frame.n);
+    si.uv = v2(b1, b2);
+    if (tc) {
+        const V2 uv0 = v2(tc[0], tc[1]), uv1 = v2(tc[2], tc[3]), uv2 = v2(tc[4], tc[5]);
+        si.uv = v2(uv0.x * b0 + uv1.x * b1 + uv2.x * b2, uv0.y * b0 + uv1.y * b1 + uv2.y * b2);
+    }
+    if (vn) {
+        V3 n0 = ld3(vn), n1 = ld3(vn + 3), n2 = ld3(vn + 6);
+        const V3 dp_du = ld3(frame.dp_du);
+        si.sh.n = normalize(n0 * b0 + n1 * b1 + n2 * b2);
+        si.sh.s = normalize(fnmadd3(si.sh.n, dot(si.sh.n, dp_du), dp_du));
+        si.sh.t = cross(si.sh.n, si.sh.s);
+    } else {
+        si.sh.n = si.n;
+        si.sh.s = ld3(frame.s);
+        si.sh.t = ld3(frame.t);
+    }
+    si.wi = to_local(si.sh, -ray_d);
+}
 MIW_HD void compute_surface_interaction(V3 p0, V3 p1, V3 p2, const float *vn, const float *tc,
                                         float t, float b1, float b2, V3 ray_d,
                                         SurfaceInteraction &si) {
@@ -242,7 +290,11 @@
     return ps;
 }
 
-MIW_HD PositionSample mesh_sample_position(const MeshSampler &m, V2 sample) {
+MIW_HD V3 face_normal(V3 p0, V3 p1, V3 p2) { return normalize(cross(p1 - p0, p2 - p0)); }
+struct FaceNormalCompute { MIW_HD V3 operator()(uint32_t, V3 e0, V3 e1) const { return normalize(cross(e0, e1)); } };
+struct FaceNormalTable { const float *n; MIW_HD V3 operator()(uint32_t idx, V3, V3) const { return ld3(n + 4 * (size_t) idx); } };
+template <typename FaceN>
+MIW_HD PositionSample mesh_sample_position(const MeshSampler &m, V2 sample, FaceN face_n) {
     uint32_t idx = distr_sample(m, sample.y);
     float pmf = m.pmf[idx] * m.normalization,
           cdf = idx > 0 ? m.cdf[idx - 1] * m.normalization : 0.f;
@@ -262,10 +314,13 @@
         V3 n0 = ld3(vn), n1 = ld3(vn + 3), n2 = ld3(vn + 6);
         ps.n = normalize(n0 * (1.f - b.x - b.y) + n1 * b.x + n2 * b.y);
     } else {
-        ps.n = normalize(cross(e0, e1));
+        ps.n = face_n(idx, e0, e1);
     }
     return ps;
 }
+MIW_HD PositionSample mesh_sample_position(const MeshSampler &m, V2 sample) {
+    return mesh_sample_position(m, sample, FaceNormalCompute{});
+}
 
 MIW_HD float face_area(V3 p0, V3 p1, V3 p2) { return 0.5f * norm(cross(p1 - p0, p2 - p0)); }
 
diff --git a/mitsuba2_amd/csrc/miwave.hip b/mitsuba2_amd/csrc/miwave.hip
--- a/mitsuba2_amd/csrc/miwave.hip
+++ b/mitsuba2_amd/csrc/miwave.hip
@@ -664,17 +664,20 @@
     return MI_OK;
 }
 
-#define MIW_LDS_PER_WORKGROUP (40u * 1024u)
+#define MIW_LDS_PER_CU (160u * 1024u)
+#define MIW_LDS_PER_WORKGROUP (MIW_LDS_PER_CU / 4u)
 #define MIW_LDS_STATIC 1024u
 #define MIW_LDS_GRANULE 512u
-static size_t lds_table_bytes(const mi_ctx *c, uint32_t words[10], bool with_tris) {
+static size_t lds_table_bytes(const mi_ctx *c, uint32_t words[12], bool with_tris) {
     words[0] = (uint32_t) (c->shapes.size() * sizeof(ShapeRec) / 4); words[1] = (uint32_t) (c->bsdfs.size() * sizeof(BsdfRec) / 4);
     words[2] = (uint32_t) (c->emitters.size() * sizeof(EmitterRec) / 4);
     words[3] = (uint32_t) c->emit_tri.size(); words[4] = (uint32_t) c->emit_vnorm.size(); words[5] = (uint32_t) c->emit_pmf.size(); words[6] = (uint32_t) c->emit_cdf.size();
     words[7] = with_tris ? (uint32_t) (c->tris_in.size() * sizeof(Tri) / 4) : 0u;
     words[8] = with_tris ? (uint32_t) c->tri_vn_in.size() : 0u; words[9] = with_tris ? (uint32_t) c->tri_uv_in.size() : 0u;
+    words[10] = with_tris ? (uint32_t) (c->tris_in.size() * sizeof(TriFrame) / 4) : 0u;
+    words[11] = with_tris ? (uint32_t) (c->emit_tri.size() / 9 * 4) : 0u;
     size_t total = 0;
-    for (int k = 0; k < 10; ++k) total += ((size_t) words[k] + 3u) / 4u * 16u;
+    for (int k = 0; k < 12; ++k) total += ((size_t) words[k] + 3u) / 4u * 16u;
     total += c->lights.size() * sizeof(LightRec);
     return total;
 }
@@ -700,7 +703,7 @@
     int max_fan = 4;
     if (const char *e = c->opt.get("MIW_BVH4_FAN")) max_fan = std::min(4, std::max(2, atoi(e)));
     double ms_bvh4 = 0.0;
-    uint32_t tab_words_[10];
+    uint32_t tab_words_[12];
     const bool tiny = c->tris_in.size() <= MIW_BRUTE_MAX_TRIS && !force_tree && c->rects.empty() &&
                       (!MIW_LDS_TABLES || lds_table_bytes(c, tab_words_, true) <= 24u * 1024u);
     if (quality == 0 && !tiny && tri_count >= 2) {
@@ -936,6 +939,7 @@
     v.lights = c->lights.empty() ? nullptr : c->d_lights.p;
     v.constant = c->constant_light >= 0 ? c->d_lights.p + c->constant_light : nullptr;
     v.env_top = nullptr; v.env_top_count = v.env_top_base = 0;
+    v.tri_frames = nullptr; v.emit_face_n = nullptr;
     v.rects = c->rects.empty() ? nullptr : c->d_rects.p; v.rect_count = (uint32_t) c->rects.size();
 
     size_t all = (size_t) node_count * sizeof(BvhNode) + (size_t) tri_count * sizeof(Tri);
@@ -1798,7 +1802,7 @@
         L.cfg.tab16 = (uint32_t) ((L.rlds + 15) / 16);
         L.table_bytes = lds_table_bytes(c, L.cfg.tab_words, c->lds_cfg.brute != 0);
         L.cfg.light_words = (uint32_t) (c->lights.size() * sizeof(LightRec) / 4);
-        L.tables_fit = (size_t) L.cfg.tab16 * 16 + L.table_bytes <= (c->lds_cfg.brute ? 64u * 1024u : lds_budget);
+        L.tables_fit = (size_t) L.cfg.tab16 * 16 + L.table_bytes <= (c->lds_cfg.brute ? 64u * 1024u - MIW_LDS_STATIC - MIW_LDS_GRANULE : lds_budget);
         L.cfg.env_top_count = L.cfg.env_top_base = L.cfg.env_top_words = 0;
         if (L.tables_fit && c->have_env && !(ropt.get("MIW_ENV_TOP") && atoi(ropt.get("MIW_ENV_TOP")) == 0)) {
             const EnvmapRec &e = c->env_host;
@@ -1842,8 +1846,14 @@
                                          pool_nw, pool_pp, layp.rlds, (size_t) pool16 * 16, 5u * NJ * 16u, layp.table_bytes, layp.cfg.env_top_words * 4u, (int) pooled_fits);
     }
     TraceLds rcfg = lay.cfg; size_t rlds = lay.rlds; const size_t rlds_plain = lay.rlds_plain, table_bytes = lay.table_bytes; const bool tables_fit = lay.tables_fit;
-    if (ropt.get("MIW_DEBUG")) fprintf(stderr, "[miwave] LDS per workgroup: %zu bytes dynamic with the scene tables (%zu without), tables %zu B of which environment warp levels %u B, budget %zu%s\n",
-                                     rlds, rlds_plain, table_bytes, rcfg.env_top_words * 4u, lds_budget4, stack8_sized ? "; stack sized for the 8-wide tree's depth" : "");
+    if (MIW_LDS_TABLES && c->lds_cfg.brute && !tables_fit) return fail(c, MI_ERR_STATE, "render: the tables of this packet scene do not fit a workgroup's LDS");
+    auto lds_workgroups = [](size_t dyn) -> uint32_t {
+        const size_t per = (dyn + MIW_LDS_STATIC + 16u + MIW_LDS_GRANULE - 1u) / MIW_LDS_GRANULE * MIW_LDS_GRANULE;
+        return (uint32_t) (MIW_LDS_PER_CU / per);
+    };
+    if (ropt.get("MIW_DEBUG")) fprintf(stderr, "[miwave] LDS per workgroup: %zu bytes dynamic with the scene tables (%zu without), tables %zu B of which environment warp levels %u B and built frame tables %u B, budget %zu%s; + %u static: %u workgroups per CU by LDS\n",
+                                     rlds, rlds_plain, table_bytes, rcfg.env_top_words * 4u, (rcfg.tab_words[10] + rcfg.tab_words[11]) * 4u, lds_budget4, stack8_sized ? "; stack sized for the 8-wide tree's depth" : "",
+                                     MIW_LDS_STATIC + 16u, lds_workgroups(rlds));
 
     mi_counters &K = c->counters;
     K.samples = K.segments = K.shadow_rays = K.iterations = 0; K.lanes = n_lanes;
@@ -1898,7 +1908,8 @@
         if (phased8) { view8.nodes8 = c->d_nodes8.p; view8.tris = c->d_tris8.p; if (view8.tri_vn) view8.tri_vn = c->d_tri_vn8.p; }
         bool packet_shard4 = !phased && tiny && c->diffuse_only && !MIW_SPECTRAL && !direct && c->view.tri_count <= 32u && MIW_PACKET_WAVES > 4 && film_mode == 1 && n_lanes <= 64u * 4u * n_simd;
         if (const char *e = ropt.get("MIW_PACKET_SHARD4")) packet_shard4 = packet_shard4 && atoi(e) != 0;
-        const uint32_t res_waves = phased ? (uint32_t) ph_waves : !tiny ? (uint32_t) MIW_TREE_WAVES : (c->diffuse_only && !MIW_SPECTRAL ? (c->view.tri_count <= 32u && !packet_shard4 ? (uint32_t) MIW_PACKET_WAVES : 4u) : (uint32_t) MIW_PACKET_WAVES_ALL);
+        const uint32_t res_waves_compiled = phased ? (uint32_t) ph_waves : !tiny ? (uint32_t) MIW_TREE_WAVES : (c->diffuse_only && !MIW_SPECTRAL ? (c->view.tri_count <= 32u && !packet_shard4 ? (uint32_t) MIW_PACKET_WAVES : 4u) : (uint32_t) MIW_PACKET_WAVES_ALL);
+        const uint32_t res_waves = tiny && film_mode == 1 ? std::max(1u, std::min(res_waves_compiled, lds_workgroups(rlds))) : res_waves_compiled;
         bool place = film_mode == 1 && !direct && (tiny || phased_placeable) && n_lanes >= 64u * n_simd / 2u && n_lanes <= 64u * res_waves * n_simd &&
                      cfg->spp >= 128u && per_launch >= cfg->spp && cfg->timeout_s <= 0.f;
         if (const char *e = ropt.get("MIW_PLACE")) place = place && atoi(e) != 0;
```

New measurement: 4649, median of 6. 1.04x the previous value.
